# uzh-rpg/rpg_ramnet

Hardware: AMD Instinct MI355X
Metric: depth samples/sec (346x260 cropped to 256x344, 5-bin grids, K=5 grids + 1 frame per sample; training step) (higher is better)
Workload: dtype f32; 1 GPU; EventScape-shaped 346x260 -> 256x344 crop, 5 event bins, K=5, batch 8/GPU, seq-len 8, 1xMI355X-per-rank train, state=convgru, SI loss on [image,events4], Adam, backward-weights co-scheduled on a side stream, decoders on a second stream; global_batch=8, seq_len=8, parallelism=dp1

## Files before the change

include/ramnet_hip.h:

```cpp
#ifndef RAMNET_HIP_H
#define RAMNET_HIP_H
#include <stddef.h>
#include <stdint.h>

#ifdef __cplusplus
extern "C" {
#endif

#define RAMNET_ABI_VERSION 27
#define RAMNET_E_BADARG 10001
#define RAMNET_E_UNSUPPORTED 10002

enum ramnet_in_mode {
    RAMNET_IN_PLAIN = 0,
    RAMNET_IN_CAT = 1,
    RAMNET_IN_CAT_MUL = 2,
    RAMNET_IN_UP2X = 3,
    RAMNET_IN_UP2X_SKIP = 4,
    RAMNET_IN_RELUMASK = 5,
    RAMNET_IN_S2D = 6,
    RAMNET_IN_PARITY4 = 7
};

enum ramnet_algo { RAMNET_ALGO_DIRECT = 0, RAMNET_ALGO_WINOGRAD = 1, RAMNET_ALGO_HEAD = 2, RAMNET_ALGO_WINOGRAD24 = 3, RAMNET_ALGO_WINOGRAD_2X4 = 4,
                   RAMNET_ALGO_WINOGRAD_2X4_SPLIT = 5, RAMNET_ALGO_DIRECT_SPLIT = 6, RAMNET_ALGO_WINOGRAD24_2X3 = 7 };

enum ramnet_epilogue {
    RAMNET_EPI_LINEAR = 0,
    RAMNET_EPI_RELU = 1,
    RAMNET_EPI_SIGMOID = 2,
    RAMNET_EPI_RES_RELU = 3,
    RAMNET_EPI_GRU_BLEND = 4,
    RAMNET_EPI_LSTM = 5,
    RAMNET_EPI_GRU_BWD = 6,
    RAMNET_EPI_SIGMOID_HR = 7
};

typedef struct ramnet_conv_desc {
    const float *x0, *x1, *xm;
    int ld0, ld1, ldm;
    int C0, C1;
    int in_mode;
    int B, Hin, Win;
    int ntaps, stride;
    int8_t dy[25], dx[25];
    uint8_t wtap[25];
    const float *w;
    const float *bias;
    int Cout;
    int Ho, Wo;
    int HoF, WoF;
    int osy, osx, ooy, oox;
    int epi;
    float beta;
    const float *e0, *e1;
    int lde0, lde1;
    float *out, *o1, *o2;
    int ldo, ldo1, ldo2;
    int algo;
    int frame;
    int out_s2d;
    int head_cin;
    int s2d_5x5;
    float *splitk_ws;
    size_t splitk_floats;
    const int *active;
} ramnet_conv_desc;

#define RAMNET_WGRAD_MAX_SEGMENTS 48
typedef struct ramnet_wgrad_seg {
    const float *x0, *x1, *xm, *dout, *gmask;
} ramnet_wgrad_seg;

typedef struct ramnet_wgrad_desc {
    const float *x0, *x1, *xm;
    int ld0, ld1, ldm, C0, C1, in_mode;
    int B, Hin, Win;
    int ntaps, stride;
    int8_t dy[25], dx[25];
    const float *dout, *gmask;
    int ldg, ldgm;
    int Cout, Ho, Wo;
    float *dw;
    float *dbias;
    int algo;
    int gsy, gsx, goy, gox;
    int HoG, WoG;
    int head_cin;
    int dw_slabs;
    int nseg;
    const ramnet_wgrad_seg *segs;
} ramnet_wgrad_desc;

int ramnet_set_option(const char *name, int value);
int ramnet_get_option(const char *name);
const char *ramnet_last_error(void);
int ramnet_abi_version(void);
const char *ramnet_last_kernel(void);
int ramnet_stream_fork(void *from, void *to);

int ramnet_gemm(const float *A, const float *B, float *C, int M, int N, int K, int lda, int ldb, int ldc, int trans_a,
                int accumulate, int batch, long stride_a, long stride_b, long stride_c, void *stream);
int ramnet_gemm2(const float *A, const float *B, float *C, int M, long stride_a, long stride_b, long stride_c, int batch, const float *A2,
                 const float *B2, float *C2, int M2, long stride_a2, long stride_b2, long stride_c2, int batch2, int N, int K, int K2, int lda,
                 int ldb, int ldc, int trans_a, int accumulate, void *stream);

int ramnet_nchw_to_nhwc_pad(const float *src, float *dst, int B, int C, int H, int W, int Cpad, void *stream);
int ramnet_reflect_pad(const float *src, float *dst, int B, int C, int H, int W, int Cpad, int top, int left, int Hc, int Wc, int nhwc,
                       void *stream);
int ramnet_wgrad_wino_slabs(int Cin, int Cout);
int ramnet_wgrad_wino2x4_slabs(int Cin, int Cout);
int ramnet_wgrad_dsplit_slabs(int Cin, int Cout);
size_t ramnet_wgrad_dsplit_ws_floats(int Cin, int Cout);
int ramnet_unpack_wgrad_dsplit(const float *ws, float *grad, int Cout, int Cin, int CinWs, int CoutWs, int n_off, void *stream);
size_t ramnet_wgrad_wino2x4_ws_floats(int Cin, int Cout);
int ramnet_reduce_slabs(float *ws, int slabs, size_t n, void *stream);
size_t ramnet_packed_weight_elems(int Cout, int Cin, int KH, int KW, int transposed, int gates);
size_t ramnet_packed_weight_elems_wino(int Cout, int Cin, int transposed, int gates);
int ramnet_pack_weight_wino(const float *w_oihw, float *wp, int Cout, int Cin, int transposed, int gates, void *stream);
size_t ramnet_packed_weight_elems_wino2x4(int Cout, int Cin, int transposed);
int ramnet_pack_weight_wino2x4(const float *w_oihw, float *wp, int Cout, int Cin, int transposed, void *stream);
size_t ramnet_packed_weight_elems_wino2x4_gates(int Cout, int Cin, int transposed, int gates);
int ramnet_pack_weight_wino2x4_gates(const float *w_oihw, float *wp, int Cout, int Cin, int transposed, int gates, void *stream);
int ramnet_conv_wino_variant(const ramnet_conv_desc *d, int force);
int ramnet_conv_wino_split_ok(const ramnet_conv_desc *d, int force);
size_t ramnet_packed_weight_elems_wino2x4_split(int Cout, int Cin, int transposed);
int ramnet_pack_weight_wino2x4_split(const float *w_oihw, float *wp, int Cout, int Cin, int transposed, void *stream);
size_t ramnet_conv_splitk_floats(const ramnet_conv_desc *d);
int ramnet_wino2x4_config(int min_wgs);
int ramnet_fold_wino_supported(int Cout, int Cin);
size_t ramnet_packed_weight_elems_fold_wino(int Cout, int Cin);
int ramnet_pack_weight_fold_wino(const float *w_oihw, float *wp, int Cout, int Cin, void *stream);
int ramnet_pack_weight_fold_wino_dgrad(const float *w_oihw, float *wp, int Cout, int Cin, void *stream);
int ramnet_pack_border_weights(const float *w_oihw, float *rows, float *cols, float *rows_t, float *cols_t, int Cout, int Cin, void *stream);
int ramnet_fold_wino_variant(const ramnet_conv_desc *d, int force);
size_t ramnet_packed_weight_elems_fold_wino2x3(int Cout, int Cin);
int ramnet_pack_weight_fold_wino2x3(const float *w_oihw, float *wp, int Cout, int Cin, void *stream);
int ramnet_pack_weight_fold_wino2x3_dgrad(const float *w_oihw, float *wp, int Cout, int Cin, void *stream);
int ramnet_fold_unpack_wgrad(float *w4, float *dU, float *wr, float *wc, float *grad, int Cout, int Cin, int CinWs, void *stream);
size_t ramnet_packed_weight_elems_head(int Cin);
int ramnet_head_supported(int Cin, int Cout);
int ramnet_pack_weight_head(const float *w_oihw, float *wp, int Cout, int Cin, void *stream);
int ramnet_pack_weight(const float *w_oihw, float *wp, int Cout, int Cin, int KH, int KW,
                       int transposed, int gates, void *stream);
int ramnet_unpack_wgrad(const float *ws, float *grad_oihw, int Cout, int Cin, int CinWs, int CoutWs, int n_off,
                        int KH, int KW, void *stream);

int ramnet_unpack_wgrad_wino(const float *ws, float *grad_oihw, int Cout, int Cin, int CinWs, int CoutWs, int n_off,
                             void *stream);
int ramnet_unpack_wgrad_wino2x4(const float *ws, float *grad_oihw, int Cout, int Cin, int CinWs, int CoutWs, int n_off,
                                void *stream);

int ramnet_conv_launch(const ramnet_conv_desc *d, void *stream);
int ramnet_conv_launch_multi(const ramnet_conv_desc *descs, int n, void *stream);
int ramnet_wgrad_launch(const ramnet_wgrad_desc *d, void *stream);

int ramnet_pred_sigmoid_fwd(const float *x, int ldx, int C, const float *w, const float *b, float *y,
                            size_t npix, void *stream);
int ramnet_pred_sigmoid_bwd(const float *x, int ldx, int C, const float *w, const float *y, const float *dy,
                            float *dx, int lddx, float *dw, float *db, size_t npix, void *stream);
#define RAMNET_PRED_SI_MAX_SEGMENTS 8
size_t ramnet_pred_si_scratch_doubles(size_t seg_pix, int nseg);
int ramnet_pred_sigmoid_si_fwd(const float *x, int ldx, int C, const float *w, const float *b, float *y, size_t seg_pix, int nseg,
                               const float *const *targets, float weight, float lambda, double *scratch, double *stats, float *loss,
                               void *stream);
int ramnet_pred_sigmoid_si_bwd(const float *x, int ldx, int C, const float *w, const float *y, const float *dy, size_t seg_pix, int nseg,
                               const float *const *targets, const double *stats, const float *gscale, float weight, float lambda,
                               float *dx, int lddx, float *dw, float *db, double *scratch, int mask_x, void *stream);
int ramnet_pred_linear_fwd(const float *x, int ldx, int C, const float *w, const float *b, float *z, size_t npix, void *stream);
int ramnet_pred_linear_bwd(const float *x, int ldx, int C, const float *w, const float *dz, float *dx, int lddx, float *dw, float *db,
                           size_t npix, void *stream);
int ramnet_relu_bwd(const float *dy, const float *y, float *dx, size_t n, void *stream);
int ramnet_pad2_sum(const float *x, const float *skip, float *out, int B, int H, int W, int C, void *stream);
int ramnet_up2x_border_im2col(const float *x, const float *skip, float *rows, float *cols, int B, int H, int W, int C, void *stream);
int ramnet_pad2_sum_im2col(const float *x, const float *skip, float *out, float *rows, float *cols, int B, int H, int W, int C, void *stream);
int ramnet_unpad2_fold(const float *dxpad, float *dx, int B, int H, int W, int C, void *stream);
int ramnet_up2x_border_col2im(const float *rows, const float *cols, float *dx, int B, int H, int W, int C, void *stream);
int ramnet_frame_gather(const float *dy, const float *mask, float *rows, float *cols, int B, int H2, int W2, int C, void *stream);
int ramnet_space_to_depth2(const float *x, float *out, int B, int H, int W, int C, int inverse, void *stream);
int ramnet_upsample2x_bwd(const float *dup, float *dx, int B, int H, int W, int C, void *stream);
int ramnet_gru_bwd_a(const float *dhn, const float *ur, const float *o, const float *h, float *dpo,
                     float *dpur, float *dh, size_t npix, int C, int ld_dhn ,
                     void *stream);
int ramnet_gru_bwd_a2(const float *dhn, const float *ur, const float *o, const float *h, float *dpo,
                      float *dpur, float *dh, size_t npix, int C, int ld_dhn, int ld_dh ,
                      void *stream);
int ramnet_gru_bwd_b(const float *dxhr, const float *ur, const float *h, float *dpur, float *dh,
                     size_t npix, int C, void *stream);
int ramnet_lstm_bwd(const float *gates, const float *cprev, const float *cnew, const float *dhn,
                    const float *dcn, float *dpre, float *dcprev, size_t npix, int C, void *stream);
int ramnet_lstm_bwd_masked(const float *gates, const float *cprev, const float *cnew, const float *dhn, const float *dcn,
                           const int *active, float *dpre, float *dcprev, float *dxh, size_t npix, int hw, int C, void *stream);
int ramnet_bias_grad(const float *dy, const float *mask, float *db, size_t npix, int C, void *stream);
int ramnet_norm_slabs(int groups, long npix, int C);
int ramnet_norm_partial(const float *a, int lda, const float *y, int ldy, int act, const float *b, int ldb, int groups, long npix,
                        int C, int nslab, double *part, void *stream);
int ramnet_norm_finalize(const double *part, int groups, int nslab, int C, long npix, double eps, const float *gamma, const float *beta,
                         float *running_mean, float *running_var, double momentum, int update_running, int use_running,
                         long long *num_batches_tracked, double *mean, double *rstd, float *scale, float *shift, void *stream);
int ramnet_norm_finalize_bwd(const double *part, int groups, int nslab, int C, long npix, const double *mean, const double *rstd,
                             const float *gamma, int batch_stats, float *c1, float *c2, float *c3, float *dgamma, float *dbeta, void *stream);
int ramnet_norm_apply(const float *x, int ldx, const float *scale, const float *shift, const float *res, int ldr, int act, float *out,
                      int ldo, int groups, long npix, int C, void *stream);
int ramnet_norm_bwd(const float *dy, int lddy, const float *y, int ldy, int act, const float *x, int ldx, const float *c1, const float *c2,
                    const float *c3, float *dx, int lddx, float *dres, int lddres, int groups, long npix, int C, void *stream);
int ramnet_add(const float *a, const float *b, float *y, size_t n, void *stream);
int ramnet_concat2(const float *a, int lda, int Ca, const float *b, int ldb, int Cb, float *y, size_t npix, void *stream);
int ramnet_cat_batch_add(const float *const *parts, int n, size_t npix, int C, int ld, const float *base, float *out, void *stream);
int ramnet_cat_batch_add_masked(const float *const *parts, int n, size_t npix, int C, int ld, const float *base, const float *mask, float *out,
                                void *stream);
int ramnet_split2(const float *y, int ldy, int Ca, int Cb, float *a, float *b, size_t npix, void *stream);

int ramnet_si_loss_fwd(const float *pred, const float *target, size_t n, float weight, float lambda,
                       double *stats, float *loss, void *stream);
int ramnet_si_loss_from_stats(const double *stats, float weight, float lambda, float *loss, void *stream);
int ramnet_si_loss_bwd(const float *pred, const float *target, size_t n, float weight, float lambda,
                       const double *stats, const float *gscale, float *dpred, void *stream);

int ramnet_si_log_loss_fwd(const float *pred, const float *target, size_t n, float lambda, double *stats, float *loss, void *stream);
int ramnet_si_log_loss_bwd(const float *pred, const float *target, size_t n, float lambda, const double *stats, const float *gscale,
                           float *dpred, void *stream);
int ramnet_mse_loss_fwd(const float *pred, const float *target, int B, int H, int W, int half, double *stats, float *loss, void *stream);
int ramnet_mse_loss_bwd(const float *pred, const float *target, int B, int H, int W, int half, const double *stats, const float *gscale,
                        float *dpred, void *stream);

int ramnet_depth_metrics(const float *pred, const float *target, size_t n, float clip_distance, float reg_factor,
                         float cutoff, double *out11, void *stream);

size_t ramnet_msg_workspace_elems(int B, int H, int W, int num_scales);
int ramnet_msg_loss_fwd(const float *pred, const float *target, int B, int H, int W, int num_scales, float *ws,
                        double *stats, float *loss, void *stream);
int ramnet_msg_loss_bwd(const float *ws, const double *stats, const float *gscale, int B, int H, int W, int num_scales,
                        float *dws, float *dpred, void *stream);

int ramnet_voxelize(const double *events, size_t n_events, int bins, int W, int H, float *grid, void *stream);
int ramnet_voxel_indices(const double *events, size_t n_events, int bins, int W, int H,
                         long long *idx_left, long long *idx_right, void *stream);
int ramnet_normalize_nonzero(float *grid, size_t n, double *scratch, void *stream);
int ramnet_voxelize_batch(const double *events, const long long *offsets, int n_grids, size_t max_events, int bins, int W, int H,
                          float *grids, void *stream);
int ramnet_normalize_nonzero_batch(float *grids, int n_grids, size_t n, double *scratch, void *stream);
int ramnet_nonzero_stats_batch(const float *grids, int n_grids, size_t n, double *stats, void *stream);

int ramnet_augment_batch(const float *const *src, float *const *dst, const int *pidx, const float *theta, const int *win,
                         const int *win_host, const double *stats, const float *bx, const float *by, int G, int n_params, int C,
                         int H, int W, int th, int tw, int Cpad, int nhwc, void *stream);

#define RAMNET_BATCH_METRICS_TICKET_BYTES 262144
size_t ramnet_batch_metrics_workspace(int G, int N, size_t npix);
int ramnet_batch_metrics(const float *const *pred, const float *const *target, int G, int N, size_t npix, void *workspace,
                         double *out, void *stream);

int ramnet_fill_pointer_table(const void **table, const void *const *host_ptrs, int n, void *stream);
size_t ramnet_grad_loss_workspace(int G, int B, int H, int W);
int ramnet_grad_loss_stats(const float *const *pred, const float *const *target, int G, int B, int H, int W, int num_scales,
                           void *workspace, double *stats, const float *weights, float *loss, float *wsum, void *stream);
int ramnet_grad_loss_from_stats(const double *stats, int G, int num_scales, double Bg, const double *Bg_dev, const float *weights,
                                float *loss, float *wsum, void *stream);
int ramnet_grad_loss_bwd(const float *const *pred, const float *const *target, int G, int B, int H, int W, int num_scales,
                         const double *stats, double Bg, const double *Bg_dev, double gain, const float *weights, const float *up,
                         const float *up_sum, float *dpred, void *stream);

#ifdef __cplusplus
}
#endif
#endif
```

rpg_ramnet_amd/_hip.py:

```python
import ctypes as C
import os

_PKG = os.path.dirname(os.path.abspath(__file__))
LIB_PATH = os.environ.get("RAMNET_HIP_LIB") or os.path.join(_PKG, "librpg_ramnet_hip.so")

IN_PLAIN, IN_CAT, IN_CAT_MUL, IN_UP2X, IN_UP2X_SKIP, IN_RELUMASK, IN_S2D, IN_PARITY4 = range(8)
ALGO_DIRECT, ALGO_WINOGRAD, ALGO_HEAD, ALGO_WINOGRAD24, ALGO_WINOGRAD_2X4, ALGO_WINOGRAD_2X4_SPLIT, ALGO_DIRECT_SPLIT = 0, 1, 2, 3, 4, 5, 6
ALGO_WINOGRAD24_2X3 = 7
EPI_LINEAR, EPI_RELU, EPI_SIGMOID, EPI_RES_RELU, EPI_GRU_BLEND, EPI_LSTM, EPI_GRU_BWD, EPI_SIGMOID_HR = range(8)

_fp = C.c_void_p


class ConvDesc(C.Structure):
    _fields_ = [
        ("x0", _fp), ("x1", _fp), ("xm", _fp),
        ("ld0", C.c_int), ("ld1", C.c_int), ("ldm", C.c_int),
        ("C0", C.c_int), ("C1", C.c_int), ("in_mode", C.c_int),
        ("B", C.c_int), ("Hin", C.c_int), ("Win", C.c_int),
        ("ntaps", C.c_int), ("stride", C.c_int),
        ("dy", C.c_int8 * 25), ("dx", C.c_int8 * 25), ("wtap", C.c_uint8 * 25),
        ("w", _fp), ("bias", _fp),
        ("Cout", C.c_int), ("Ho", C.c_int), ("Wo", C.c_int), ("HoF", C.c_int), ("WoF", C.c_int),
        ("osy", C.c_int), ("osx", C.c_int), ("ooy", C.c_int), ("oox", C.c_int),
        ("epi", C.c_int), ("beta", C.c_float),
        ("e0", _fp), ("e1", _fp), ("lde0", C.c_int), ("lde1", C.c_int),
        ("out", _fp), ("o1", _fp), ("o2", _fp),
        ("ldo", C.c_int), ("ldo1", C.c_int), ("ldo2", C.c_int),
        ("algo", C.c_int),
        ("frame", C.c_int),
        ("out_s2d", C.c_int),
        ("head_cin", C.c_int),
        ("s2d_5x5", C.c_int),
        ("splitk_ws", C.c_void_p), ("splitk_floats", C.c_size_t),
        ("active", _fp),
    ]


class WgradSeg(C.Structure):
    _fields_ = [("x0", _fp), ("x1", _fp), ("xm", _fp), ("dout", _fp), ("gmask", _fp)]


WGRAD_MAX_SEGMENTS = 48


class WgradDesc(C.Structure):
    _fields_ = [
        ("x0", _fp), ("x1", _fp), ("xm", _fp),
        ("ld0", C.c_int), ("ld1", C.c_int), ("ldm", C.c_int),
        ("C0", C.c_int), ("C1", C.c_int), ("in_mode", C.c_int),
        ("B", C.c_int), ("Hin", C.c_int), ("Win", C.c_int),
        ("ntaps", C.c_int), ("stride", C.c_int),
        ("dy", C.c_int8 * 25), ("dx", C.c_int8 * 25),
        ("dout", _fp), ("gmask", _fp), ("ldg", C.c_int), ("ldgm", C.c_int),
        ("Cout", C.c_int), ("Ho", C.c_int), ("Wo", C.c_int),
        ("dw", _fp), ("dbias", _fp),
        ("algo", C.c_int),
        ("gsy", C.c_int), ("gsx", C.c_int), ("goy", C.c_int), ("gox", C.c_int), ("HoG", C.c_int), ("WoG", C.c_int),
        ("head_cin", C.c_int),
        ("dw_slabs", C.c_int),
        ("nseg", C.c_int), ("segs", C.POINTER(WgradSeg)),
    ]


_SIGS = {
    "ramnet_abi_version": (C.c_int, []),
    "ramnet_last_error": (C.c_char_p, []),
    "ramnet_set_option": (C.c_int, [C.c_char_p, C.c_int]),
    "ramnet_get_option": (C.c_int, [C.c_char_p]),
    "ramnet_last_kernel": (C.c_char_p, []),
    "ramnet_stream_fork": (C.c_int, [_fp, _fp]),
    "ramnet_gemm": (C.c_int, [_fp, _fp, _fp] + [C.c_int] * 9 + [C.c_long] * 3 + [_fp]),
    "ramnet_gemm2": (C.c_int, [_fp, _fp, _fp, C.c_int, C.c_long, C.c_long, C.c_long, C.c_int, _fp, _fp, _fp, C.c_int, C.c_long, C.c_long, C.c_long,
                               C.c_int, C.c_int, C.c_int, C.c_int, C.c_int, C.c_int, C.c_int, C.c_int, C.c_int, _fp]),
    "ramnet_nchw_to_nhwc_pad": (C.c_int, [_fp, _fp, C.c_int, C.c_int, C.c_int, C.c_int, C.c_int, _fp]),
    "ramnet_reflect_pad": (C.c_int, [_fp, _fp] + [C.c_int] * 10 + [_fp]),
    "ramnet_wgrad_wino_slabs": (C.c_int, [C.c_int, C.c_int]),
    "ramnet_wgrad_wino2x4_slabs": (C.c_int, [C.c_int, C.c_int]),
    "ramnet_wgrad_dsplit_slabs": (C.c_int, [C.c_int, C.c_int]),
    "ramnet_wgrad_dsplit_ws_floats": (C.c_size_t, [C.c_int, C.c_int]),
    "ramnet_unpack_wgrad_dsplit": (C.c_int, [_fp, _fp, C.c_int, C.c_int, C.c_int, C.c_int, C.c_int, _fp]),
    "ramnet_wgrad_wino2x4_ws_floats": (C.c_size_t, [C.c_int, C.c_int]),
    "ramnet_reduce_slabs": (C.c_int, [_fp, C.c_int, C.c_size_t, _fp]),
    "ramnet_packed_weight_elems": (C.c_size_t, [C.c_int] * 6),
    "ramnet_pack_weight": (C.c_int, [_fp, _fp, C.c_int, C.c_int, C.c_int, C.c_int, C.c_int, C.c_int, _fp]),
    "ramnet_packed_weight_elems_wino": (C.c_size_t, [C.c_int] * 4),
    "ramnet_pack_weight_wino": (C.c_int, [_fp, _fp, C.c_int, C.c_int, C.c_int, C.c_int, _fp]),
    "ramnet_packed_weight_elems_wino2x4": (C.c_size_t, [C.c_int] * 3),
    "ramnet_pack_weight_wino2x4": (C.c_int, [_fp, _fp, C.c_int, C.c_int, C.c_int, _fp]),
    "ramnet_packed_weight_elems_wino2x4_gates": (C.c_size_t, [C.c_int] * 4),
    "ramnet_pack_weight_wino2x4_gates": (C.c_int, [_fp, _fp, C.c_int, C.c_int, C.c_int, C.c_int, _fp]),
    "ramnet_wino2x4_config": (C.c_int, [C.c_int]),
    "ramnet_conv_wino_variant": (C.c_int, [C.POINTER(ConvDesc), C.c_int]),
    "ramnet_conv_wino_split_ok": (C.c_int, [C.POINTER(ConvDesc), C.c_int]),
    "ramnet_packed_weight_elems_wino2x4_split": (C.c_size_t, [C.c_int] * 3),
    "ramnet_pack_weight_wino2x4_split": (C.c_int, [_fp, _fp, C.c_int, C.c_int, C.c_int, _fp]),
    "ramnet_conv_splitk_floats": (C.c_size_t, [C.POINTER(ConvDesc)]),
    "ramnet_packed_weight_elems_head": (C.c_size_t, [C.c_int]),
    "ramnet_head_supported": (C.c_int, [C.c_int, C.c_int]),
    "ramnet_pack_weight_head": (C.c_int, [_fp, _fp, C.c_int, C.c_int, _fp]),
    "ramnet_fold_wino_supported": (C.c_int, [C.c_int, C.c_int]),
    "ramnet_packed_weight_elems_fold_wino": (C.c_size_t, [C.c_int, C.c_int]),
    "ramnet_pack_weight_fold_wino": (C.c_int, [_fp, _fp, C.c_int, C.c_int, _fp]),
    "ramnet_pack_weight_fold_wino_dgrad": (C.c_int, [_fp, _fp, C.c_int, C.c_int, _fp]),
    "ramnet_fold_wino_variant": (C.c_int, [C.POINTER(ConvDesc), C.c_int]),
    "ramnet_packed_weight_elems_fold_wino2x3": (C.c_size_t, [C.c_int, C.c_int]),
    "ramnet_pack_weight_fold_wino2x3": (C.c_int, [_fp, _fp, C.c_int, C.c_int, _fp]),
    "ramnet_pack_weight_fold_wino2x3_dgrad": (C.c_int, [_fp, _fp, C.c_int, C.c_int, _fp]),
    "ramnet_pack_border_weights": (C.c_int, [_fp] * 5 + [C.c_int, C.c_int, _fp]),
    "ramnet_fold_unpack_wgrad": (C.c_int, [_fp] * 5 + [C.c_int, C.c_int, C.c_int, _fp]),
    "ramnet_unpad2_fold": (C.c_int, [_fp, _fp, C.c_int, C.c_int, C.c_int, C.c_int, _fp]),
    "ramnet_up2x_border_col2im": (C.c_int, [_fp, _fp, _fp, C.c_int, C.c_int, C.c_int, C.c_int, _fp]),
    "ramnet_pad2_sum": (C.c_int, [_fp, _fp, _fp, C.c_int, C.c_int, C.c_int, C.c_int, _fp]),
    "ramnet_up2x_border_im2col": (C.c_int, [_fp, _fp, _fp, _fp, C.c_int, C.c_int, C.c_int, C.c_int, _fp]),
    "ramnet_pad2_sum_im2col": (C.c_int, [_fp, _fp, _fp, _fp, _fp, C.c_int, C.c_int, C.c_int, C.c_int, _fp]),
    "ramnet_space_to_depth2": (C.c_int, [_fp, _fp, C.c_int, C.c_int, C.c_int, C.c_int, C.c_int, _fp]),
    "ramnet_frame_gather": (C.c_int, [_fp, _fp, _fp, _fp, C.c_int, C.c_int, C.c_int, C.c_int, _fp]),
    "ramnet_unpack_wgrad": (C.c_int, [_fp, _fp] + [C.c_int] * 7 + [_fp]),
    "ramnet_unpack_wgrad_wino": (C.c_int, [_fp, _fp] + [C.c_int] * 5 + [_fp]),
    "ramnet_unpack_wgrad_wino2x4": (C.c_int, [_fp, _fp] + [C.c_int] * 5 + [_fp]),
    "ramnet_conv_launch": (C.c_int, [C.POINTER(ConvDesc), _fp]),
    "ramnet_conv_launch_multi": (C.c_int, [C.POINTER(ConvDesc), C.c_int, _fp]),
    "ramnet_wgrad_launch": (C.c_int, [C.POINTER(WgradDesc), _fp]),
    "ramnet_pred_sigmoid_fwd": (C.c_int, [_fp, C.c_int, C.c_int, _fp, _fp, _fp, C.c_size_t, _fp]),
    "ramnet_pred_sigmoid_bwd": (C.c_int, [_fp, C.c_int, C.c_int, _fp, _fp, _fp, _fp, C.c_int, _fp, _fp, C.c_size_t, _fp]),
    "ramnet_pred_si_scratch_doubles": (C.c_size_t, [C.c_size_t, C.c_int]),
    "ramnet_pred_sigmoid_si_fwd": (C.c_int, [_fp, C.c_int, C.c_int, _fp, _fp, _fp, C.c_size_t, C.c_int, C.POINTER(C.c_void_p), C.c_float, C.c_float,
                                             _fp, _fp, _fp, _fp]),
    "ramnet_pred_sigmoid_si_bwd": (C.c_int, [_fp, C.c_int, C.c_int, _fp, _fp, _fp, C.c_size_t, C.c_int, C.POINTER(C.c_void_p), _fp, _fp, C.c_float,
                                             C.c_float, _fp, C.c_int, _fp, _fp, _fp, C.c_int, _fp]),
    "ramnet_pred_linear_fwd": (C.c_int, [_fp, C.c_int, C.c_int, _fp, _fp, _fp, C.c_size_t, _fp]),
    "ramnet_pred_linear_bwd": (C.c_int, [_fp, C.c_int, C.c_int, _fp, _fp, _fp, C.c_int, _fp, _fp, C.c_size_t, _fp]),
    "ramnet_cat_batch_add": (C.c_int, [_fp, C.c_int, C.c_size_t, C.c_int, C.c_int, _fp, _fp, _fp]),
    "ramnet_cat_batch_add_masked": (C.c_int, [_fp, C.c_int, C.c_size_t, C.c_int, C.c_int, _fp, _fp, _fp, _fp]),
    "ramnet_relu_bwd": (C.c_int, [_fp, _fp, _fp, C.c_size_t, _fp]),
    "ramnet_upsample2x_bwd": (C.c_int, [_fp, _fp, C.c_int, C.c_int, C.c_int, C.c_int, _fp]),
    "ramnet_gru_bwd_a": (C.c_int, [_fp] * 7 + [C.c_size_t, C.c_int, C.c_int, _fp]),
    "ramnet_gru_bwd_a2": (C.c_int, [_fp] * 7 + [C.c_size_t, C.c_int, C.c_int, C.c_int, _fp]),
    "ramnet_gru_bwd_b": (C.c_int, [_fp] * 5 + [C.c_size_t, C.c_int, _fp]),
    "ramnet_lstm_bwd": (C.c_int, [_fp] * 7 + [C.c_size_t, C.c_int, _fp]),
    "ramnet_lstm_bwd_masked": (C.c_int, [_fp, _fp, _fp, _fp, _fp, _fp, _fp, _fp, _fp, C.c_size_t, C.c_int, C.c_int, _fp]),
    "ramnet_norm_slabs": (C.c_int, [C.c_int, C.c_long, C.c_int]),
    "ramnet_norm_partial": (C.c_int, [_fp, C.c_int, _fp, C.c_int, C.c_int, _fp, C.c_int, C.c_int, C.c_long, C.c_int, C.c_int, _fp, _fp]),
    "ramnet_norm_finalize": (C.c_int, [_fp, C.c_int, C.c_int, C.c_int, C.c_long, C.c_double, _fp, _fp, _fp, _fp, C.c_double, C.c_int, C.c_int,
                                       _fp, _fp, _fp, _fp, _fp, _fp]),
    "ramnet_norm_finalize_bwd": (C.c_int, [_fp, C.c_int, C.c_int, C.c_int, C.c_long, _fp, _fp, _fp, C.c_int, _fp, _fp, _fp, _fp, _fp, _fp]),
    "ramnet_norm_apply": (C.c_int, [_fp, C.c_int, _fp, _fp, _fp, C.c_int, C.c_int, _fp, C.c_int, C.c_int, C.c_long, C.c_int, _fp]),
    "ramnet_norm_bwd": (C.c_int, [_fp, C.c_int, _fp, C.c_int, C.c_int, _fp, C.c_int, _fp, _fp, _fp, _fp, C.c_int, _fp, C.c_int,
                                  C.c_int, C.c_long, C.c_int, _fp]),
    "ramnet_add": (C.c_int, [_fp, _fp, _fp, C.c_size_t, _fp]),
    "ramnet_split2": (C.c_int, [_fp, C.c_int, C.c_int, C.c_int, _fp, _fp, C.c_size_t, _fp]),
    "ramnet_concat2": (C.c_int, [_fp, C.c_int, C.c_int, _fp, C.c_int, C.c_int, _fp, C.c_size_t, _fp]),
    "ramnet_bias_grad": (C.c_int, [_fp, _fp, _fp, C.c_size_t, C.c_int, _fp]),
    "ramnet_si_loss_fwd": (C.c_int, [_fp, _fp, C.c_size_t, C.c_float, C.c_float, _fp, _fp, _fp]),
    "ramnet_si_loss_from_stats": (C.c_int, [_fp, C.c_float, C.c_float, _fp, _fp]),
    "ramnet_si_loss_bwd": (C.c_int, [_fp, _fp, C.c_size_t, C.c_float, C.c_float, _fp, _fp, _fp, _fp]),
    "ramnet_si_log_loss_fwd": (C.c_int, [_fp, _fp, C.c_size_t, C.c_float, _fp, _fp, _fp]),
    "ramnet_si_log_loss_bwd": (C.c_int, [_fp, _fp, C.c_size_t, C.c_float, _fp, _fp, _fp, _fp]),
    "ramnet_mse_loss_fwd": (C.c_int, [_fp, _fp, C.c_int, C.c_int, C.c_int, C.c_int, _fp, _fp, _fp]),
    "ramnet_mse_loss_bwd": (C.c_int, [_fp, _fp, C.c_int, C.c_int, C.c_int, C.c_int, _fp, _fp, _fp, _fp]),
    "ramnet_depth_metrics": (C.c_int, [_fp, _fp, C.c_size_t, C.c_float, C.c_float, C.c_float, _fp, _fp]),
    "ramnet_msg_workspace_elems": (C.c_size_t, [C.c_int] * 4),
    "ramnet_msg_loss_fwd": (C.c_int, [_fp, _fp, C.c_int, C.c_int, C.c_int, C.c_int, _fp, _fp, _fp, _fp]),
    "ramnet_msg_loss_bwd": (C.c_int, [_fp, _fp, _fp, C.c_int, C.c_int, C.c_int, C.c_int, _fp, _fp, _fp]),
    "ramnet_voxelize": (C.c_int, [_fp, C.c_size_t, C.c_int, C.c_int, C.c_int, _fp, _fp]),
    "ramnet_voxel_indices": (C.c_int, [_fp, C.c_size_t, C.c_int, C.c_int, C.c_int, _fp, _fp, _fp]),
    "ramnet_normalize_nonzero": (C.c_int, [_fp, C.c_size_t, _fp, _fp]),
    "ramnet_voxelize_batch": (C.c_int, [_fp, _fp, C.c_int, C.c_size_t, C.c_int, C.c_int, C.c_int, _fp, _fp]),
    "ramnet_normalize_nonzero_batch": (C.c_int, [_fp, C.c_int, C.c_size_t, _fp, _fp]),
    "ramnet_nonzero_stats_batch": (C.c_int, [_fp, C.c_int, C.c_size_t, _fp, _fp]),
    "ramnet_augment_batch": (C.c_int, [_fp] * 9 + [C.c_int] * 9 + [_fp]),
    "ramnet_batch_metrics_workspace": (C.c_size_t, [C.c_int, C.c_int, C.c_size_t]),
    "ramnet_batch_metrics": (C.c_int, [_fp, _fp, C.c_int, C.c_int, C.c_size_t, _fp, _fp, _fp]),
    "ramnet_fill_pointer_table": (C.c_int, [_fp, C.POINTER(C.c_void_p), C.c_int, _fp]),
    "ramnet_grad_loss_workspace": (C.c_size_t, [C.c_int] * 4),
    "ramnet_grad_loss_stats": (C.c_int, [_fp, _fp] + [C.c_int] * 5 + [_fp] * 6),
    "ramnet_grad_loss_from_stats": (C.c_int, [_fp, C.c_int, C.c_int, C.c_double, _fp, _fp, _fp, _fp, _fp]),
    "ramnet_grad_loss_bwd": (C.c_int, [_fp, _fp] + [C.c_int] * 5 + [_fp, C.c_double, _fp, C.c_double, _fp, _fp, _fp, _fp, _fp]),
}
EXPORTS = tuple(_SIGS)

_lib = None
_tracer = None


class _Traced:
    def __init__(self, l):
        self._l = l

    def __getattr__(self, name):
        fn = getattr(self._l, name)
        tr = _tracer
        if tr is None:
            return fn
        return lambda *a: tr(name, fn, a)


def set_tracer(fn):
    global _tracer
    _tracer = fn


class HipLibraryMissing(RuntimeError):
    pass


def lib():
    global _lib
    if _lib is None:
        if not os.path.exists(LIB_PATH):
            raise HipLibraryMissing(
                "%s not found: build it with `python -c 'import __graft_entry__ as g; g.build()'` "
                "(hipcc --offload-arch=gfx950). rpg_ramnet_amd has no CPU fallback." % LIB_PATH)
        import torch
        rt = os.path.join(os.path.dirname(torch.__file__), "lib", "libamdhip64.so")
        if os.path.exists(rt):
            C.CDLL(rt, mode=C.RTLD_GLOBAL)
        l = C.CDLL(LIB_PATH)
        for name, (res, args) in _SIGS.items():
            fn = getattr(l, name)
            fn.restype, fn.argtypes = res, args
        if l.ramnet_abi_version() != 27:
            raise RuntimeError("ABI version mismatch in %s" % LIB_PATH)
        _lib = l
    return _lib if _tracer is None else _Traced(_lib)


def check(code, what):
    if code != 0:
        msg = lib().ramnet_last_error()
        raise RuntimeError("%s failed (code %d): %s" % (what, code, msg.decode() if msg else "?"))
```

rpg_ramnet_amd/csrc/common.hpp:

```cpp
#pragma once
#include <hip/hip_runtime.h>
#include <stdint.h>
#include <stdio.h>
#include "../../include/ramnet_hip.h"

typedef float f32x16 __attribute__((ext_vector_type(16)));

namespace ramnet {

constexpr int CK = 16;
constexpr int LDP = CK + 4;
constexpr int TWID = 16;
constexpr int WCK = 32;

extern int g_opt_voxel_sorted, g_opt_fold_pair, g_opt_wgrad_blocks, g_opt_wgrad_wino_blocks, g_opt_wino_ksplit, g_opt_wgrad_wino_nf, g_opt_pred_si_cap, g_opt_pred_si_bwd_cap;
void set_error(const char *fmt, ...);
void note_kernel(const char *fmt, ...);
int launch_wino(const ramnet_conv_desc &d, hipStream_t st);
size_t wino24_splitk_floats(const ramnet_conv_desc &d);
int launch_wino6(const ramnet_conv_desc &d, hipStream_t st);
int launch_wino6s(const ramnet_conv_desc &d, hipStream_t st);
int launch_head(const ramnet_conv_desc &d, hipStream_t st);
int launch_wino24(const ramnet_conv_desc &d, hipStream_t st);
int launch_wgrad_wino24(const ramnet_wgrad_desc &d, hipStream_t st);
int launch_head_wgrad(const ramnet_wgrad_desc &d, hipStream_t st);
int launch_wgrad_wino(const ramnet_wgrad_desc &d, hipStream_t st);
int launch_wgrad_wino6(const ramnet_wgrad_desc &d, hipStream_t st);
int launch_wgrad_dsplit(const ramnet_wgrad_desc &d, hipStream_t st);

#define RAMNET_CHECK_ARG(cond)                                                        \
    do {                                                                              \
        if (!(cond)) {                                                                \
            ramnet::set_error("%s:%d: bad argument: %s", __FILE__, __LINE__, #cond);  \
            return RAMNET_E_BADARG;                                                   \
        }                                                                             \
    } while (0)

#define RAMNET_HIP(call)                                                                        \
    do {                                                                                        \
        hipError_t e_ = (call);                                                                 \
        if (e_ != hipSuccess) {                                                                 \
            ramnet::set_error("%s:%d: %s -> %s", __FILE__, __LINE__, #call, hipGetErrorString(e_)); \
            return (int)e_;                                                                     \
        }                                                                                       \
    } while (0)

#define RAMNET_LAUNCH_CHECK() RAMNET_HIP(hipGetLastError())

hipError_t allow_full_lds(const void *kernel);
#define RAMNET_FULL_LDS(kern) RAMNET_HIP(ramnet::allow_full_lds(reinterpret_cast<const void *>(kern)))

__device__ __forceinline__ float4 ld4(const float *p) { return *reinterpret_cast<const float4 *>(p); }
__device__ __forceinline__ void st4(float *p, float4 v) { *reinterpret_cast<float4 *>(p) = v; }
__device__ __forceinline__ float4 f4zero() { return make_float4(0.f, 0.f, 0.f, 0.f); }
__device__ __forceinline__ float4 f4add(float4 a, float4 b) { return make_float4(a.x + b.x, a.y + b.y, a.z + b.z, a.w + b.w); }
__device__ __forceinline__ float4 f4mul(float4 a, float4 b) { return make_float4(a.x * b.x, a.y * b.y, a.z * b.z, a.w * b.w); }
__device__ __forceinline__ float4 f4scale(float4 a, float s) { return make_float4(a.x * s, a.y * s, a.z * s, a.w * s); }
__device__ __forceinline__ float sigmoidf_(float x) { return __builtin_amdgcn_rcpf(1.0f + __expf(-x)); }
__device__ __forceinline__ float tanhf_(float x) { return 1.0f - 2.0f * __builtin_amdgcn_rcpf(1.0f + __expf(2.0f * x)); }

__device__ __forceinline__ auto wino_rsrc(const void *p, unsigned bytes) {
    const unsigned long long a = (unsigned long long)p;
    const unsigned lo = __builtin_amdgcn_readfirstlane((unsigned)a), hi = __builtin_amdgcn_readfirstlane((unsigned)(a >> 32));
    return __builtin_amdgcn_make_buffer_rsrc((void *)(((unsigned long long)hi << 32) | lo), (short)0, (int)bytes, 0x00020000);
}
constexpr unsigned WOOB = 0x7fffff00u;

struct InSrc {
    const float *x0, *x1, *xm;
    int ld0, ld1, ldm, C0, Cin, mode, Hin, Win;
};

__device__ __forceinline__ void up2x_coord(int d, int n_src, int &i0, int &i1, float &l1) {
    float s = fmaxf(0.5f * (float)d - 0.25f, 0.0f);
    i0 = (int)s;
    i1 = i0 + (i0 < n_src - 1 ? 1 : 0);
    l1 = s - (float)i0;
}

__device__ __forceinline__ float4 load_in4(const InSrc &s, int b, int iy, int ix, int c) {
    if ((unsigned)iy >= (unsigned)s.Hin || (unsigned)ix >= (unsigned)s.Win || c >= s.Cin) return f4zero();
    if (s.mode == RAMNET_IN_UP2X || s.mode == RAMNET_IN_UP2X_SKIP) {
        const int Hs = s.Hin >> 1, Ws = s.Win >> 1;
        int y0, y1, x0, x1;
        float ly, lx;
        up2x_coord(iy, Hs, y0, y1, ly);
        up2x_coord(ix, Ws, x0, x1, lx);
        const float hy = 1.0f - ly, hx = 1.0f - lx;
        const size_t r0 = ((size_t)b * Hs + y0) * Ws, r1 = ((size_t)b * Hs + y1) * Ws;
        float4 v00 = ld4(s.x0 + (r0 + x0) * s.ld0 + c), v01 = ld4(s.x0 + (r0 + x1) * s.ld0 + c);
        float4 v10 = ld4(s.x0 + (r1 + x0) * s.ld0 + c), v11 = ld4(s.x0 + (r1 + x1) * s.ld0 + c);
        if (s.mode == RAMNET_IN_UP2X_SKIP) {
            v00 = f4add(v00, ld4(s.x1 + (r0 + x0) * s.ld1 + c));
            v01 = f4add(v01, ld4(s.x1 + (r0 + x1) * s.ld1 + c));
            v10 = f4add(v10, ld4(s.x1 + (r1 + x0) * s.ld1 + c));
            v11 = f4add(v11, ld4(s.x1 + (r1 + x1) * s.ld1 + c));
        }
        float4 top = f4add(f4scale(v00, hx), f4scale(v01, lx));
        float4 bot = f4add(f4scale(v10, hx), f4scale(v11, lx));
        return f4add(f4scale(top, hy), f4scale(bot, ly));
    }
    const size_t pix = ((size_t)b * s.Hin + iy) * s.Win + ix;
    if (s.mode == RAMNET_IN_PLAIN) return ld4(s.x0 + pix * s.ld0 + c);
    if (s.mode == RAMNET_IN_RELUMASK) {
        float4 v = ld4(s.x0 + pix * s.ld0 + c), m = ld4(s.xm + pix * s.ldm + c);
        return make_float4(m.x > 0.f ? v.x : 0.f, m.y > 0.f ? v.y : 0.f, m.z > 0.f ? v.z : 0.f, m.w > 0.f ? v.w : 0.f);
    }
    if (c < s.C0) return ld4(s.x0 + pix * s.ld0 + c);
    float4 v = ld4(s.x1 + pix * s.ld1 + (c - s.C0));
    if (s.mode == RAMNET_IN_CAT_MUL) v = f4mul(v, ld4(s.xm + pix * s.ldm + (c - s.C0)));
    return v;
}

template <int QPP, int LDX, int NB, int NT>
__device__ __forceinline__ void stage_patch(float *__restrict__ patch, const InSrc &s, int b, int iy0, int ix0, int c0,
                                            int PH, int PW, int tid) {
    constexpr int PXS = LDX, QS = 4;
    const int nslots = PH * PW * QPP;
    if (s.mode == RAMNET_IN_UP2X || s.mode == RAMNET_IN_UP2X_SKIP) {
        for (int sl = tid; sl < nslots; sl += NT) {
            const int pix = sl / QPP, qd = sl - pix * QPP;
            const int py = pix / PW, px = pix - py * PW;
            st4(patch + pix * PXS + qd * QS, load_in4(s, b, iy0 + py, ix0 + px, c0 + qd * 4));
        }
        return;
    }
    const bool two = s.mode == RAMNET_IN_CAT_MUL || s.mode == RAMNET_IN_RELUMASK;
    for (int base = tid; base < nslots; base += NB * NT) {
        float4 v[NB], m[NB];
        int dst[NB];
        bool ok[NB], hasm[NB];
#pragma unroll
        for (int i = 0; i < NB; ++i) {
            const int sl = base + i * NT;
            const int pix = sl / QPP, qd = sl - pix * QPP;
            const int py = pix / PW, px = pix - py * PW;
            const int iy = iy0 + py, ix = ix0 + px, c = c0 + qd * 4;
            ok[i] = sl < nslots && (unsigned)iy < (unsigned)s.Hin && (unsigned)ix < (unsigned)s.Win && c < s.Cin;
            dst[i] = sl < nslots ? pix * PXS + qd * QS : -1;
            const size_t gp = ((size_t)b * s.Hin + iy) * s.Win + ix;
            const bool second = s.mode != RAMNET_IN_PLAIN && s.mode != RAMNET_IN_RELUMASK && c >= s.C0;
            const float *p0 = second ? s.x1 + gp * s.ld1 + (c - s.C0) : s.x0 + gp * s.ld0 + c;
            hasm[i] = two && (s.mode == RAMNET_IN_RELUMASK || second);
            const float *p1 = s.mode == RAMNET_IN_RELUMASK ? s.xm + gp * s.ldm + c : s.xm + gp * s.ldm + (c - s.C0);
            v[i] = ld4(ok[i] ? p0 : s.x0);
            if (two) m[i] = ld4(ok[i] && hasm[i] ? p1 : s.x0);
        }
#pragma unroll
        for (int i = 0; i < NB; ++i) {
            float4 r = v[i];
            if (two && hasm[i]) {
                if (s.mode == RAMNET_IN_RELUMASK)
                    r = make_float4(m[i].x > 0.f ? r.x : 0.f, m[i].y > 0.f ? r.y : 0.f, m[i].z > 0.f ? r.z : 0.f, m[i].w > 0.f ? r.w : 0.f);
                else
                    r = f4mul(r, m[i]);
            }
            if (!ok[i]) r = f4zero();
            if (dst[i] >= 0) st4(patch + dst[i], r);
        }
    }
}

template <int QPP, int NB, int NT>
struct PatchRegs {
    float4 v[NB], m[NB];
    unsigned okmask, mmask;

    __device__ __forceinline__ void load(const InSrc &s, int b, int iy0, int ix0, int c0, int PH, int PW, int tid) {
        const int nslots = PH * PW * QPP;
        const bool two = s.mode == RAMNET_IN_CAT_MUL || s.mode == RAMNET_IN_RELUMASK;
        okmask = 0, mmask = 0;
#pragma unroll
        for (int i = 0; i < NB; ++i) {
            const int sl = tid + i * NT;
            const int pix = sl / QPP, qd = sl - pix * QPP;
            const int py = pix / PW, px = pix - py * PW;
            const int iy = iy0 + py, ix = ix0 + px, c = c0 + qd * 4;
            const bool ok = sl < nslots && (unsigned)iy < (unsigned)s.Hin && (unsigned)ix < (unsigned)s.Win && c < s.Cin;
            const size_t gp = ((size_t)b * s.Hin + iy) * s.Win + ix;
            const bool second = s.mode != RAMNET_IN_PLAIN && s.mode != RAMNET_IN_RELUMASK && c >= s.C0;
            const float *p0 = second ? s.x1 + gp * s.ld1 + (c - s.C0) : s.x0 + gp * s.ld0 + c;
            const bool hm = two && (s.mode == RAMNET_IN_RELUMASK || second);
            const float *p1 = s.mode == RAMNET_IN_RELUMASK ? s.xm + gp * s.ldm + c : s.xm + gp * s.ldm + (c - s.C0);
            v[i] = ld4(ok ? p0 : s.x0);
            m[i] = two ? ld4(ok && hm ? p1 : s.x0) : f4zero();
            okmask |= (ok ? 1u : 0u) << i;
            mmask |= (hm ? 1u : 0u) << i;
        }
    }

    __device__ __forceinline__ float4 value(const InSrc &s, int i) const {
        float4 r = v[i];
        if ((mmask >> i) & 1u) {
            if (s.mode == RAMNET_IN_RELUMASK)
                r = make_float4(m[i].x > 0.f ? r.x : 0.f, m[i].y > 0.f ? r.y : 0.f, m[i].z > 0.f ? r.z : 0.f, m[i].w > 0.f ? r.w : 0.f);
            else
                r = f4mul(r, m[i]);
        }
        if (!((okmask >> i) & 1u)) r = f4zero();
        return r;
    }

    template <int ROWF, int PS>
    __device__ __forceinline__ void store_planes(float *__restrict__ patch, const InSrc &s, int PH, int PW, int tid) const {
        const int nslots = PH * PW * QPP;
#pragma unroll
        for (int i = 0; i < NB; ++i) {
            const int sl = tid + i * NT;
            const float4 r = value(s, i);
            const int pix = sl / QPP, qd = sl - pix * QPP;
            const int py = pix / PW, px = pix - py * PW;
            if (sl < nslots) {
                float *d = patch + (2 * qd) * PS + py * ROWF + px * 2;
                *reinterpret_cast<float2 *>(d) = make_float2(r.x, r.y);
                *reinterpret_cast<float2 *>(d + PS) = make_float2(r.z, r.w);
            }
        }
    }

    template <int LDX>
    __device__ __forceinline__ void store(float *__restrict__ patch, const InSrc &s, int PH, int PW, int tid) const {
        const int nslots = PH * PW * QPP;
#pragma unroll
        for (int i = 0; i < NB; ++i) {
            const int sl = tid + i * NT;
            float4 r = v[i];
            if ((mmask >> i) & 1u) {
                if (s.mode == RAMNET_IN_RELUMASK)
                    r = make_float4(m[i].x > 0.f ? r.x : 0.f, m[i].y > 0.f ? r.y : 0.f, m[i].z > 0.f ? r.z : 0.f, m[i].w > 0.f ? r.w : 0.f);
                else
                    r = f4mul(r, m[i]);
            }
            if (!((okmask >> i) & 1u)) r = f4zero();
            if (sl < nslots) st4(patch + (sl / QPP) * LDX + (sl % QPP) * 4, r);
        }
    }
};

inline int cdiv(int a, int b) { return (a + b - 1) / b; }
inline int roundup(int a, int b) { return cdiv(a, b) * b; }

}
```

rpg_ramnet_amd/csrc/conv_igemm.hip:

```cpp
#include <stdlib.h>
#include "common.hpp"
#include "conv_epilogue.hpp"

namespace ramnet {

struct ConvCommon {
    InSrc src;
    int nchunks, CoutPad;
    int patch_floats;
    int nclass;
    int xcd_swizzle;
};

struct ConvClass {
    int ntaps, Ho, Wo, ooy, oox;
    int PH, PW, dymin, dxmin;
    int tiles_x, tiles_y;
    int toff[25];
    unsigned woff[25];
};
struct ConvClasses { ConvClass c[4]; };

template <int BM, int BN, int WM, int WN, bool MASK = false>
__global__ void __launch_bounds__(256) conv_igemm_kernel(const ramnet_conv_desc p, const ConvCommon qc, const ConvClasses qk) {
    int flat = blockIdx.x + gridDim.x * (blockIdx.y + gridDim.y * blockIdx.z);
    if (qc.xcd_swizzle) {
        const int nwg = gridDim.x * gridDim.y * gridDim.z, xcd = flat & 7, qq = nwg >> 3, rr = nwg & 7;
        flat = (xcd < rr ? xcd * (qq + 1) : rr * (qq + 1) + (xcd - rr) * qq) + (flat >> 3);
    }
    int bid = flat % gridDim.x;
    const int by = (flat / gridDim.x) % gridDim.y, bz = flat / (gridDim.x * gridDim.y);
    const ConvClass &q = qk.c[bz];
    constexpr int TM = BM / WM / 32, TN = BN / WN / 32;
    constexpr int TH = BM / TWID;
    constexpr int CKC = CK;
    static_assert(WM * WN == 4 && TM >= 1 && TN >= 1, "4 waves per workgroup");
    extern __shared__ __attribute__((aligned(16))) float smem[];
    float *patch = smem;
    float *wsm = smem + qc.patch_floats;

    const int tid = threadIdx.x, lane = tid & 63;
    const int wave = __builtin_amdgcn_readfirstlane(tid >> 6);
    const int wm = wave / WN, wn = wave % WN;
    const int l31 = lane & 31, kk = lane >> 5;

    if (bid >= q.tiles_x * q.tiles_y * p.B) return;
    const int tx_i = bid % q.tiles_x;
    bid /= q.tiles_x;
    const int ty_i = bid % q.tiles_y;
    const int b = bid / q.tiles_y;
    const int n0 = by * BN;
    const int oy0 = ty_i * TH, ox0 = tx_i * TWID;
    const int iy0 = oy0 * p.stride + q.dymin, ix0 = ox0 * p.stride + q.dxmin;

    int aBase[TM], bBase[TN];
#pragma unroll
    for (int ms = 0; ms < TM; ++ms) {
        const int m = (wm * TM + ms) * 32 + l31;
        aBase[ms] = (((m >> 4) * p.stride) * q.PW + (m & 15) * p.stride) * LDP + 4 * kk;
    }
#pragma unroll
    for (int ns = 0; ns < TN; ++ns) bBase[ns] = ((wn * TN + ns) * 32 + l31) * LDP + 4 * kk;

    f32x16 acc[TM][TN];
#pragma unroll
    for (int ms = 0; ms < TM; ++ms)
#pragma unroll
        for (int ns = 0; ns < TN; ++ns)
#pragma unroll
            for (int r = 0; r < 16; ++r) acc[ms][ns][r] = 0.f;

    constexpr int WF4 = BN * 4;
    constexpr int WPT = (WF4 + 255) / 256;
    float4 wreg[WPT];
    const int ntaps = q.ntaps;
    auto load_w = [&](int chunk, int t) {
        const float *src = p.w + ((size_t)q.woff[t] + ((size_t)chunk * qc.CoutPad + n0)) * 16;
#pragma unroll
        for (int i = 0; i < WPT; ++i) {
            const int f = tid + i * 256;
            if (WF4 % 256 == 0 || f < WF4) wreg[i] = ld4(src + (size_t)f * 4);
        }
    };
    auto store_w = [&](int buf) {
        float *dst = wsm + buf * (BN * LDP);
#pragma unroll
        for (int i = 0; i < WPT; ++i) {
            const int f = tid + i * 256;
            if (WF4 % 256 == 0 || f < WF4) st4(dst + (f >> 2) * LDP + (f & 3) * 4, wreg[i]);
        }
    };

    load_w(0, 0);
    int buf = 0;
    for (int chunk = 0; chunk < qc.nchunks; ++chunk) {
        __syncthreads();
        stage_patch<CKC / 4, LDP, 4, 256>(patch, qc.src, b, iy0, ix0, chunk * CKC, q.PH, q.PW, tid);
        for (int t = 0; t < ntaps; ++t) {
            store_w(buf);
            __syncthreads();
            if (t + 1 < ntaps) load_w(chunk, t + 1);
            else if (chunk + 1 < qc.nchunks) load_w(chunk + 1, 0);
            const float *pa = patch + q.toff[t];
            const float *wb = wsm + buf * (BN * LDP);
#pragma unroll
            for (int k8 = 0; k8 < 2; ++k8) {
                float4 a[TM], bb[TN];
#pragma unroll
                for (int ms = 0; ms < TM; ++ms) a[ms] = ld4(pa + aBase[ms] + k8 * 8);
#pragma unroll
                for (int ns = 0; ns < TN; ++ns) bb[ns] = ld4(wb + bBase[ns] + k8 * 8);
#pragma unroll
                for (int ms = 0; ms < TM; ++ms)
#pragma unroll
                    for (int ns = 0; ns < TN; ++ns) {
                        acc[ms][ns] = __builtin_amdgcn_mfma_f32_32x32x2f32(a[ms].x, bb[ns].x, acc[ms][ns], 0, 0, 0);
                        acc[ms][ns] = __builtin_amdgcn_mfma_f32_32x32x2f32(a[ms].y, bb[ns].y, acc[ms][ns], 0, 0, 0);
                        acc[ms][ns] = __builtin_amdgcn_mfma_f32_32x32x2f32(a[ms].z, bb[ns].z, acc[ms][ns], 0, 0, 0);
                        acc[ms][ns] = __builtin_amdgcn_mfma_f32_32x32x2f32(a[ms].w, bb[ns].w, acc[ms][ns], 0, 0, 0);
                    }
            }
            buf ^= 1;
        }
    }

    const int epi = p.epi;
    const bool act = !MASK || sample_active(p, b);
#pragma unroll
    for (int ms = 0; ms < TM; ++ms) {
#pragma unroll
        for (int r = 0; r < 16; ++r) {
            const int m = (wm * TM + ms) * 32 + (r & 3) + 8 * (r >> 2) + 4 * kk;
            const int oy = oy0 + (m >> 4), ox = ox0 + (m & 15);
            if (oy >= q.Ho || ox >= q.Wo) continue;
            const size_t pix = ((size_t)b * p.HoF + (oy * p.osy + q.ooy)) * p.WoF + (ox * p.osx + q.oox);
            const bool addold = epilogue_addold(p, oy * p.osy + q.ooy, ox * p.osx + q.oox);
            if (epi == RAMNET_EPI_LSTM) {
                if constexpr (TN == 4) {
                    const int C = p.Cout, ch = by * 32 + l31;
                    if (MASK && !act) {
                        if (ch < C) epilogue_inactive(p, epi, pix, ch);
                    } else if (ch < C) {
                        const float gi = sigmoidf_(acc[ms][0][r] + p.bias[ch]);
                        const float gf = sigmoidf_(acc[ms][1][r] + p.bias[C + ch]);
                        const float go = sigmoidf_(acc[ms][2][r] + p.bias[2 * C + ch]);
                        const float gc = tanhf_(acc[ms][3][r] + p.bias[3 * C + ch]);
                        const float cp = p.e1 ? p.e1[pix * p.lde1 + ch] : 0.f;
                        const float cn = gf * cp + gi * gc;
                        p.out[pix * p.ldo + ch] = go * tanhf_(cn);
                        p.o1[pix * p.ldo1 + ch] = cn;
                        if (p.o2) {
                            float *g = p.o2 + pix * p.ldo2 + ch;
                            g[0] = gi, g[C] = gf, g[2 * C] = go, g[3 * C] = gc;
                        }
                    }
                }
                continue;
            }
#pragma unroll
            for (int ns = 0; ns < TN; ++ns) {
                const int n = n0 + (wn * TN + ns) * 32 + l31;
                if (n >= p.Cout) continue;
                if (MASK && !act) {
                    epilogue_inactive(p, epi, pix, n);
                    continue;
                }
                epilogue_store(p, epi, pix, n, acc[ms][ns][r] + epilogue_side(p, epi, b, oy * p.osy + q.ooy, ox * p.osx + q.oox, n), addold);
            }
        }
    }
}

template <int BM, int BN, int WM, int WN>
static int launch_cfg(const ramnet_conv_desc &d, const ConvCommon &qc, const ConvClasses &qk, int max_tiles, hipStream_t st) {
    auto kern = d.active ? conv_igemm_kernel<BM, BN, WM, WN, true> : conv_igemm_kernel<BM, BN, WM, WN>;
    const size_t lds = ((size_t)qc.patch_floats + 2 * BN * LDP) * sizeof(float);
    static size_t lds_set[2] = {0, 0};
    if (lds > lds_set[d.active != nullptr]) {
        RAMNET_FULL_LDS((kern));
        lds_set[d.active != nullptr] = 160 * 1024;
    }
    if (lds > 160 * 1024) {
        set_error("conv patch does not fit LDS (%zu bytes)", lds);
        return RAMNET_E_UNSUPPORTED;
    }
    dim3 grid(max_tiles * d.B, qc.CoutPad / BN, qc.nclass);
    note_kernel(d.active ? "conv_igemm_kernel<%d,%d,%d,%d,masked>" : "conv_igemm_kernel<%d,%d,%d,%d>", BM, BN, WM, WN);
    hipLaunchKernelGGL(kern, grid, dim3(256), lds, st, d, qc, qk);
    RAMNET_LAUNCH_CHECK();
    return 0;
}

static int check_desc(const ramnet_conv_desc &d) {
    RAMNET_CHECK_ARG(d.x0 && d.w && d.out);
    RAMNET_CHECK_ARG(d.ntaps >= 1 && d.ntaps <= 25 && (d.stride == 1 || d.stride == 2));
    RAMNET_CHECK_ARG(d.B > 0 && d.Ho > 0 && d.Wo > 0 && d.Hin > 0 && d.Win > 0 && d.Cout > 0);
    RAMNET_CHECK_ARG(d.C0 > 0 && d.C0 % 4 == 0 && d.ld0 % 4 == 0 && d.ldo > 0);
    RAMNET_CHECK_ARG(d.osy >= 1 && d.osx >= 1);
    const bool cat = d.in_mode == RAMNET_IN_CAT || d.in_mode == RAMNET_IN_CAT_MUL;
    if (cat) RAMNET_CHECK_ARG(d.x1 && d.C1 > 0 && d.C1 % 4 == 0 && d.ld1 % 4 == 0);
    if (d.in_mode == RAMNET_IN_CAT_MUL || d.in_mode == RAMNET_IN_RELUMASK) RAMNET_CHECK_ARG(d.xm && d.ldm % 4 == 0);
    if (d.in_mode == RAMNET_IN_UP2X_SKIP) RAMNET_CHECK_ARG(d.x1 && d.ld1 % 4 == 0);
    if (d.in_mode == RAMNET_IN_UP2X || d.in_mode == RAMNET_IN_UP2X_SKIP) RAMNET_CHECK_ARG(d.Hin % 2 == 0 && d.Win % 2 == 0);
    if (d.epi == RAMNET_EPI_RES_RELU) RAMNET_CHECK_ARG(d.e0);
    if (d.epi == RAMNET_EPI_GRU_BLEND) RAMNET_CHECK_ARG(d.e0);
    if (d.epi == RAMNET_EPI_LSTM) RAMNET_CHECK_ARG(d.o1 && d.bias);
    if (d.epi == RAMNET_EPI_GRU_BWD) RAMNET_CHECK_ARG(d.e0 && d.o1 && d.Cout % 8 == 0 && !d.bias && d.beta == 0.f && d.frame == 0 && d.out_s2d == 0);
    if (d.epi == RAMNET_EPI_SIGMOID_HR) RAMNET_CHECK_ARG(d.e1 && d.o1 && d.Cout % 8 == 0 && d.beta == 0.f && d.frame == 0 && d.out_s2d == 0 &&
                                                         d.algo != RAMNET_ALGO_WINOGRAD24 && d.algo != RAMNET_ALGO_WINOGRAD24_2X3 && d.algo != RAMNET_ALGO_HEAD);
    {
        unsigned long long ld = (unsigned long long)d.ld0;
        if (cat || d.in_mode == RAMNET_IN_UP2X_SKIP) ld = ld > (unsigned long long)d.ld1 ? ld : (unsigned long long)d.ld1;
        if (d.xm) ld = ld > (unsigned long long)d.ldm ? ld : (unsigned long long)d.ldm;
        const unsigned long long px = (unsigned long long)d.B * d.Hin * d.Win * (d.in_mode == RAMNET_IN_S2D ? 4 : 1);
        RAMNET_CHECK_ARG(px * ld < (1ull << 32));
    }
    RAMNET_CHECK_ARG(d.frame >= 0);
    if (d.active) RAMNET_CHECK_ARG((d.epi == RAMNET_EPI_SIGMOID || d.epi == RAMNET_EPI_SIGMOID_HR || d.epi == RAMNET_EPI_GRU_BLEND ||
                                    (d.epi == RAMNET_EPI_LSTM && d.e0)) && d.frame == 0 && d.out_s2d == 0 &&
                                   (d.algo == RAMNET_ALGO_DIRECT || d.algo == RAMNET_ALGO_WINOGRAD || d.algo == RAMNET_ALGO_WINOGRAD_2X4 ||
                                    d.algo == RAMNET_ALGO_WINOGRAD_2X4_SPLIT));
    if (d.frame > 0) RAMNET_CHECK_ARG(d.e0 && d.e1 && (d.epi == RAMNET_EPI_RELU || d.epi == RAMNET_EPI_LINEAR));
    return 0;
}

static int launch_classes(const ramnet_conv_desc *ds, int n, hipStream_t st) {
    const ramnet_conv_desc &d = ds[0];
    for (int i = 0; i < n; ++i) {
        const int rc = check_desc(ds[i]);
        if (rc) return rc;
        RAMNET_CHECK_ARG(ds[i].x0 == d.x0 && ds[i].w == d.w && ds[i].out == d.out && ds[i].stride == d.stride &&
                         ds[i].Cout == d.Cout && ds[i].epi == d.epi && ds[i].osy == d.osy && ds[i].osx == d.osx &&
                         ds[i].B == d.B && ds[i].in_mode == d.in_mode && ds[i].active == d.active);
    }
    const bool cat = d.in_mode == RAMNET_IN_CAT || d.in_mode == RAMNET_IN_CAT_MUL;
    ConvCommon qc;
    ConvClasses qk;
    qc.src.x0 = d.x0, qc.src.x1 = d.x1, qc.src.xm = d.xm;
    qc.src.ld0 = d.ld0, qc.src.ld1 = d.ld1, qc.src.ldm = d.ldm;
    qc.src.C0 = d.C0, qc.src.Cin = d.C0 + (cat ? d.C1 : 0);
    qc.src.mode = d.in_mode, qc.src.Hin = d.Hin, qc.src.Win = d.Win;
    qc.nchunks = cdiv(qc.src.Cin, CK);
    qc.CoutPad = d.epi == RAMNET_EPI_LSTM ? 4 * roundup(d.Cout, 32) : roundup(d.Cout, 32);
    qc.nclass = n;
    qc.xcd_swizzle = 0;
    const int lstm = d.epi == RAMNET_EPI_LSTM;
    int BM = 128, BN = lstm ? 128 : (qc.CoutPad % 128 == 0 ? 128 : qc.CoutPad % 64 == 0 ? 64 : 32);
    auto blocks = [&](int bm, int bn) {
        long t = 0;
        for (int i = 0; i < n; ++i) t += (long)cdiv(ds[i].Wo, TWID) * cdiv(ds[i].Ho, bm / TWID);
        return t * d.B * (qc.CoutPad / bn);
    };
    if (!lstm && BN >= 64) {
        const long want = 768;
        if (blocks(BM, BN) < want) BM = 64;
        if (blocks(BM, BN) < want && BN == 128) BN = 64;
    }
    if (!lstm && BN == 32 && blocks(256, 32) >= 1024)
        BM = 256;
    const int TH = BM / TWID;
    int max_tiles = 0;
    qc.patch_floats = 0;
    for (int i = 0; i < n; ++i) {
        const ramnet_conv_desc &e = ds[i];
        ConvClass &q = qk.c[i];
        int dymin = 127, dymax = -127, dxmin = 127, dxmax = -127;
        for (int t = 0; t < e.ntaps; ++t) {
            dymin = e.dy[t] < dymin ? e.dy[t] : dymin, dymax = e.dy[t] > dymax ? e.dy[t] : dymax;
            dxmin = e.dx[t] < dxmin ? e.dx[t] : dxmin, dxmax = e.dx[t] > dxmax ? e.dx[t] : dxmax;
        }
        q.ntaps = e.ntaps, q.Ho = e.Ho, q.Wo = e.Wo, q.ooy = e.ooy, q.oox = e.oox;
        q.dymin = dymin, q.dxmin = dxmin;
        q.PH = (TH - 1) * e.stride + (dymax - dymin) + 1;
        q.PW = (TWID - 1) * e.stride + (dxmax - dxmin) + 1;
        q.tiles_x = cdiv(e.Wo, TWID), q.tiles_y = cdiv(e.Ho, TH);
        for (int t = 0; t < e.ntaps; ++t) {
            q.toff[t] = ((e.dy[t] - dymin) * q.PW + (e.dx[t] - dxmin)) * LDP;
            q.woff[t] = (unsigned)e.wtap[t] * (unsigned)qc.nchunks * (unsigned)qc.CoutPad;
        }
        if (q.PH * q.PW * LDP > qc.patch_floats) qc.patch_floats = q.PH * q.PW * LDP;
        if (q.tiles_x * q.tiles_y > max_tiles) max_tiles = q.tiles_x * q.tiles_y;
    }
    if (lstm) return launch_cfg<128, 128, 4, 1>(d, qc, qk, max_tiles, st);
    if (BM == 128 && BN == 128) return launch_cfg<128, 128, 2, 2>(d, qc, qk, max_tiles, st);
    if (BM == 128 && BN == 64) return launch_cfg<128, 64, 2, 2>(d, qc, qk, max_tiles, st);
    if (BM == 64 && BN == 128) return launch_cfg<64, 128, 2, 2>(d, qc, qk, max_tiles, st);
    if (BM == 64 && BN == 64) return launch_cfg<64, 64, 2, 2>(d, qc, qk, max_tiles, st);
    if (BM == 256) return launch_cfg<256, 32, 4, 1>(d, qc, qk, max_tiles, st);
    return launch_cfg<128, 32, 4, 1>(d, qc, qk, max_tiles, st);
}

}

using namespace ramnet;

extern "C" int ramnet_conv_launch(const ramnet_conv_desc *dp, void *stream) {
    RAMNET_CHECK_ARG(dp != nullptr);
    if (dp->algo == RAMNET_ALGO_WINOGRAD) {
        const int rc = check_desc(*dp);
        return rc ? rc : launch_wino(*dp, (hipStream_t)stream);
    }
    if (dp->algo == RAMNET_ALGO_WINOGRAD_2X4) {
        const int rc = check_desc(*dp);
        return rc ? rc : launch_wino6(*dp, (hipStream_t)stream);
    }
    if (dp->algo == RAMNET_ALGO_WINOGRAD_2X4_SPLIT) {
        const int rc = check_desc(*dp);
        return rc ? rc : launch_wino6s(*dp, (hipStream_t)stream);
    }
    if (dp->algo == RAMNET_ALGO_WINOGRAD24 || dp->algo == RAMNET_ALGO_WINOGRAD24_2X3) {
        const int rc = check_desc(*dp);
        return rc ? rc : launch_wino24(*dp, (hipStream_t)stream);
    }
    if (dp->algo == RAMNET_ALGO_HEAD) {
        const int rc = check_desc(*dp);
        return rc ? rc : launch_head(*dp, (hipStream_t)stream);
    }
    RAMNET_CHECK_ARG(dp->algo == RAMNET_ALGO_DIRECT && dp->in_mode != RAMNET_IN_S2D && dp->out_s2d == 0);
    return launch_classes(dp, 1, (hipStream_t)stream);
}

extern "C" int ramnet_conv_launch_multi(const ramnet_conv_desc *descs, int n, void *stream) {
    RAMNET_CHECK_ARG(descs != nullptr && n >= 1 && n <= 4);
    for (int i = 0; i < n; ++i) RAMNET_CHECK_ARG(descs[i].in_mode != RAMNET_IN_S2D && descs[i].out_s2d == 0);
    return launch_classes(descs, n, (hipStream_t)stream);
}
```

rpg_ramnet_amd/csrc/conv_plan.hpp:

```cpp
#pragma once
#include "conv_wino_common.hpp"

namespace ramnet {

#define RAMNET_PLAN_CHECK(cond)                                                                       \
    do {                                                                                              \
        if (!(cond)) {                                                                                \
            if (!quiet) ramnet::set_error("%s:%d: bad argument: %s", __FILE__, __LINE__, #cond);      \
            return RAMNET_E_BADARG;                                                                   \
        }                                                                                             \
    } while (0)

constexpr int WKS = 16;
constexpr int W6_BN = 64;
constexpr int W6_U_FLOATS = 24 * W6_BN * WK;
constexpr int W6S_POS_BYTES = 2 * 3 * 1024;
constexpr int W6S_BLK_BYTES = 4 * 6 * W6S_POS_BYTES;

inline int log2_exact(int v) {
    int sh = 0;
    while ((1 << sh) < v) ++sh;
    return (1 << sh) == v ? sh : -1;
}

inline bool al16(const void *ptr) { return ptr == nullptr || ((uintptr_t)ptr & 15) == 0; }

template <class Desc>
inline void fill_in_src(const Desc &d, InSrc &s) {
    const bool cat = d.in_mode == RAMNET_IN_CAT || d.in_mode == RAMNET_IN_CAT_MUL;
    s.x0 = d.x0, s.x1 = d.x1, s.xm = d.xm;
    s.ld0 = d.ld0, s.ld1 = d.ld1, s.ldm = d.ldm;
    s.C0 = d.C0, s.Cin = d.C0 + (cat ? d.C1 : 0);
    s.mode = d.in_mode, s.Hin = d.Hin, s.Win = d.Win;
    if (d.in_mode == RAMNET_IN_S2D) s.Cin = 4 * d.C0, s.ld1 = log2_exact(d.C0);
}

inline bool taps_3x3(const int8_t *dy, const int8_t *dx, bool forward_order, int &dy0, int &dx0) {
    dy0 = 127, dx0 = 127;
    for (int t = 0; t < 9; ++t) {
        dy0 = dy[t] < dy0 ? dy[t] : dy0;
        dx0 = dx[t] < dx0 ? dx[t] : dx0;
    }
    unsigned seen = 0;
    for (int t = 0; t < 9; ++t) {
        const int a = dy[t] - dy0, c = dx[t] - dx0;
        if (a < 0 || a >= 3 || c < 0 || c >= 3 || (forward_order && a * 3 + c != t)) return false;
        seen |= 1u << (a * 3 + c);
    }
    return seen == 0x1ffu;
}

inline bool conv_vec4(const ramnet_conv_desc &d, bool with_o2) {
    return d.Cout % 4 == 0 && d.ldo % 4 == 0 && al16(d.out) && al16(d.bias) && (!d.o1 || (d.ldo1 % 4 == 0 && al16(d.o1))) &&
           (!d.e0 || (d.lde0 % 4 == 0 && al16(d.e0))) && (!d.e1 || (d.lde1 % 4 == 0 && al16(d.e1))) &&
           (!with_o2 || !d.o2 || (d.ldo2 % 4 == 0 && al16(d.o2)));
}

inline bool out_s2d_ok(const ramnet_conv_desc &d) {
    return d.out_s2d >= 8 && log2_exact(d.out_s2d) > 0 && d.Cout == 4 * d.out_s2d && d.epi == RAMNET_EPI_LINEAR && !d.bias && d.beta == 0.f &&
           d.HoF == 2 * d.Ho && d.WoF == 2 * d.Wo;
}

inline int xcd_groups(size_t wbytes, int nblk) {
    int xg = wbytes > (12u << 20) ? 2 : wbytes > (3u << 20) ? 1 : 0;
    while (xg > 0 && (nblk % (1 << xg)) != 0) --xg;
    return xg;
}

inline int check_offsets32(const ramnet_conv_desc &d, bool with_o2, bool quiet) {
    const unsigned long long px = (unsigned long long)d.Hin * d.Win * (d.in_mode == RAMNET_IN_S2D ? 4 : 1);
    int ldmax = d.ld0 > d.ld1 ? d.ld0 : d.ld1;
    ldmax = ldmax > d.ldm ? ldmax : d.ldm;
    RAMNET_PLAN_CHECK(px * ldmax * 4ull < (unsigned long long)WOOB);
    int lo = d.ldo > d.ldo1 ? d.ldo : d.ldo1;
    lo = lo > d.lde0 ? lo : d.lde0;
    lo = lo > d.lde1 ? lo : d.lde1;
    if (with_o2) lo = lo > d.ldo2 ? lo : d.ldo2;
    RAMNET_PLAN_CHECK((unsigned long long)d.HoF * d.WoF * lo * 4ull < (unsigned long long)WOOB);
    return 0;
}

inline long wino6_tile(int Ho, int Wo, int &txg) {
    const int shapes[3] = {4, 2, 8};
    long best = -1;
    for (int s = 0; s < 3; ++s) {
        const int t = shapes[s], th = 2 * (32 / t), tw = 4 * t;
        const long a = (long)cdiv(Ho, th) * th * cdiv(Wo, tw) * tw;
        if (best < 0 || a < best) best = a, txg = t;
    }
    return best;
}

inline bool wino6_lstm_ok(const ramnet_conv_desc &d) {
    return d.in_mode == RAMNET_IN_CAT && d.C0 % WK == 0 && d.Cout > 0 && d.Cout % 16 == 0 && d.o1 && d.bias && !d.out_s2d && !d.frame &&
           d.osy == 1 && d.osx == 1 && d.ooy == 0 && d.oox == 0 &&
           (!d.o2 || (d.ldo2 % 4 == 0 && d.ldo2 >= 4 * d.Cout && ((uintptr_t)d.o2 & 15) == 0));
}

struct Wino6Plan {
    WinoParams q;
    int txg;
    unsigned grid;
    size_t exchange;
};

inline int wino6_plan(const ramnet_conv_desc &d, int chunk, Wino6Plan &out, bool quiet = false) {
    const bool split = chunk == WKS;
    RAMNET_PLAN_CHECK(d.ntaps == 9 && d.stride == 1 && !d.frame);
    const bool lstm = d.epi == RAMNET_EPI_LSTM;
    if (lstm) RAMNET_PLAN_CHECK(!split && wino6_lstm_ok(d) && (!d.active || d.e0));
    const int ncol = lstm ? 4 * d.Cout : d.Cout;
    RAMNET_PLAN_CHECK(ncol % W6_BN == 0);
    RAMNET_PLAN_CHECK(d.in_mode == RAMNET_IN_PLAIN || d.in_mode == RAMNET_IN_CAT || d.in_mode == RAMNET_IN_CAT_MUL || d.in_mode == RAMNET_IN_RELUMASK ||
                      d.in_mode == RAMNET_IN_S2D);
    if (d.in_mode == RAMNET_IN_S2D) RAMNET_PLAN_CHECK(d.C0 >= chunk && log2_exact(d.C0) > 0);
    if (d.in_mode == RAMNET_IN_CAT || d.in_mode == RAMNET_IN_CAT_MUL) RAMNET_PLAN_CHECK(d.C0 % chunk == 0);
    RAMNET_PLAN_CHECK(conv_vec4(d, false) && d.osy == 1 && d.osx == 1 && d.ooy == 0 && d.oox == 0);
    if (d.out_s2d) RAMNET_PLAN_CHECK(out_s2d_ok(d));
    if (d.epi == RAMNET_EPI_GRU_BWD) RAMNET_PLAN_CHECK(d.Cout % 128 == 0);
    int dy0, dx0;
    RAMNET_PLAN_CHECK(taps_3x3(d.dy, d.dx, false, dy0, dx0));
    if (int rc = check_offsets32(d, lstm && d.o2, quiet)) return rc;
    WinoParams &q = out.q;
    q = WinoParams{};
    fill_in_src(d, q.src);
    q.nchunks = cdiv(q.src.Cin, chunk), q.nblk = cdiv(ncol, W6_BN);
    wino6_tile(d.Ho, d.Wo, out.txg);
    q.tiles_x = cdiv(d.Wo, 4 * out.txg), q.tiles_y = cdiv(d.Ho, 2 * (32 / out.txg));
    q.dy0 = dy0, q.dx0 = dx0;
    q.vec4 = 1, q.s2d_shift = d.out_s2d ? log2_exact(d.out_s2d) : 0, q.ksplit = 1;
    q.xg = xcd_groups((size_t)q.nchunks * q.nblk * (split ? (size_t)W6S_BLK_BYTES : W6_U_FLOATS * sizeof(float)), q.nblk);
    const int wgcols = split ? 64 : 32;
    const int nbl = (q.nblk * (W6_BN / wgcols)) >> q.xg;
    q.inv_nbl = 1.0f / (float)nbl, q.inv_tx = 1.0f / (float)q.tiles_x, q.inv_ty = 1.0f / (float)q.tiles_y;
    out.grid = (unsigned)(cdiv(q.tiles_x * q.tiles_y * d.B, 8 >> q.xg) * 8 * nbl);
    out.exchange = (size_t)4 * 4 * 32 * (wgcols + 4) * sizeof(float);
    return 0;
}

#undef RAMNET_PLAN_CHECK

template <int BLOCK = 256, class K, class... A>
inline int launch_1d(K kernel, size_t total, void *stream, A... args) {
    size_t blocks = (total + BLOCK - 1) / BLOCK;
    if (blocks > 65535) blocks = 65535;
    hipLaunchKernelGGL(kernel, dim3((unsigned)blocks), dim3(BLOCK), 0, (hipStream_t)stream, args...);
    RAMNET_LAUNCH_CHECK();
    return 0;
}

}
```

rpg_ramnet_amd/csrc/conv_wino6.hip:

```cpp
#include <stdlib.h>
#include <type_traits>
#include "common.hpp"
#include "conv_epilogue.hpp"
#include "conv_plan.hpp"

typedef float f32x4 __attribute__((ext_vector_type(4)));
typedef unsigned u32x4 __attribute__((ext_vector_type(4)));

namespace ramnet {

#ifdef RAMNET_PROBE
__device__ unsigned long long g_probe6[16384 * 16];
#define RAMNET_STAMP(k) do { if (threadIdx.x == 0 && blockIdx.x < 16384) g_probe6[blockIdx.x * 16 + (k)] = __builtin_readcyclecounter(); } while (0)
#else
#define RAMNET_STAMP(k) do { } while (0)
#endif

template <int TXG> struct R6Geom {
    static constexpr int TYG = 32 / TXG, TH = 2 * TYG, TW = 4 * TXG, PH = TH + 2, PW = TW + 2, PWS = PW + 3;
    static constexpr int PSLOTS = PH * PWS + ((4 - (PH * PWS) % 8) + 8) % 8;
    static constexpr int PLANE = PSLOTS * 4;
    static constexpr int PFLOATS = 2 * PLANE;
    static_assert(PH * PW * 2 <= 768, "three patch slots per thread");
};

template <int TXG, int MODE, bool MASK = false, bool LSTM = false>
__global__ void __launch_bounds__(256, 2) conv_wino_r6_kernel(const ramnet_conv_desc p, const WinoParams q) {
    constexpr int NF = 1;
    constexpr int RO_LD = NF * 32 + 4;
    using G = R6Geom<TXG>;
    constexpr int RP_PLANE = G::PLANE, RP_FLOATS = G::PFLOATS, RPW = G::PWS, RTW = G::TW;
    extern __shared__ __attribute__((aligned(16))) float smem[];
    float *patch = smem;

    const int tid = threadIdx.x, lane = tid & 63;
    const int wave = __builtin_amdgcn_readfirstlane(tid >> 6);
    const int l31 = lane & 31, hq = lane >> 5;
    RAMNET_STAMP(0);
#ifdef RAMNET_PROBE
    if (threadIdx.x == 0 && blockIdx.x < 16384) {
        g_probe6[blockIdx.x * 16 + 7] = __builtin_amdgcn_s_memrealtime();
        g_probe6[blockIdx.x * 16 + 8] = __builtin_amdgcn_s_getreg((31 << 11) | 4);
        g_probe6[blockIdx.x * 16 + 9] = __builtin_amdgcn_s_getreg((31 << 11) | 20);
    }
#endif

    auto fdiv = [](int n, int d, float inv) {
        int qv = (int)((float)n * inv);
        const int r = n - qv * d;
        qv += (r >= d ? 1 : 0) - (r < 0 ? 1 : 0);
        return qv;
    };
    const int xslot = blockIdx.x >> 3, xcd = blockIdx.x & 7;
    const int nbl = (q.nblk * (2 / NF)) >> q.xg;
    const int xq = fdiv(xslot, nbl, q.inv_nbl);
    const int nblk_v = ((xslot - xq * nbl) << q.xg) + (xcd & ((1 << q.xg) - 1));
    const int nblk_i = NF == 1 ? nblk_v >> 1 : nblk_v, fh = NF == 1 ? nblk_v & 1 : 0;
    int bid = xq * (8 >> q.xg) + (xcd >> q.xg);
    if (bid >= q.tiles_x * q.tiles_y * p.B) return;
    const int bq = fdiv(bid, q.tiles_x, q.inv_tx);
    const int tx_i = bid - bq * q.tiles_x;
    const int b = fdiv(bq, q.tiles_y, q.inv_ty);
    const int ty_i = bq - b * q.tiles_y;
    const int n0 = nblk_i * W6_BN + fh * 32;
    const int oy0 = ty_i * G::TH, ox0 = tx_i * G::TW;
    const int iy0 = oy0 + q.dy0, ix0 = ox0 + q.dx0;

    const int tty = l31 / TXG, ttx = l31 % TXG;
    const int ra = wave == 0 ? 0 : (wave == 2 ? 2 : 1);
    const int rb = wave == 0 ? 2 : (wave == 1 ? 2 : (wave == 2 ? 1 : 3));
    const float sb = wave == 1 ? 1.f : -1.f;
    const int pra = hq * RP_PLANE + ((2 * tty + ra) * RPW + 4 * ttx + (((2 * tty + ra) >> 1) & 3)) * 4;
    const int prb = hq * RP_PLANE + ((2 * tty + rb) * RPW + 4 * ttx + (((2 * tty + rb) >> 1) & 3)) * 4;

    f32x16 acc[6][NF];
#pragma unroll
    for (int i = 0; i < 6; ++i)
#pragma unroll
        for (int f = 0; f < NF; ++f)
#pragma unroll
            for (int r = 0; r < 16; ++r) acc[i][f][r] = 0.f;

    const int nch = q.nchunks;
    const int clast = (nch - 1) * WK;
    WinoPatch<MODE, 3> pr;
    pr.template init<G::PH, G::PW, G::PWS, G::PLANE, true>(q.src, b, iy0, ix0, tid, clast, 2 * RP_FLOATS);
    const auto wrs = wino_rsrc(p.w, (unsigned)((size_t)nch * q.nblk * W6_U_FLOATS * sizeof(float)));
    const unsigned wvo = (unsigned)((wave * 3072 + fh * 256 + lane * 4) * 4);
    const int wblk = nblk_i * W6_U_FLOATS * 4, wchunk = q.nblk * W6_U_FLOATS * 4;
    auto wload = [&](int chunk, int i) {
        return __builtin_bit_cast(float4, __builtin_amdgcn_raw_buffer_load_b128(wrs, (int)wvo, chunk * wchunk + wblk + i * 1024, 0));
    };
    float4 breg[6][NF];
    float tA[6][4], tB[6][4];
    constexpr int LD = 2;
    float vb[4][4];
    float4 qa[6], qb[6];
    float sa[4], sd[4];
    auto colop = [&](int qp, int vi, int i, const float (&t)[6][4]) {
        float(&v)[4] = vb[vi];
        if (qp == 0) {
            if (i < 4) v[i] = fmaf(-5.f, t[2][i], t[4][i]);
            else v[i - 4] = fmaf(4.f, t[0][i - 4], v[i - 4]);
        } else if (qp == 1) {
            if (i < 2) sa[2 * i] = fmaf(-4.f, t[2][2 * i], t[4][2 * i]), sa[2 * i + 1] = fmaf(-4.f, t[2][2 * i + 1], t[4][2 * i + 1]);
            else if (i < 4) sd[2 * i - 4] = fmaf(-4.f, t[1][2 * i - 4], t[3][2 * i - 4]), sd[2 * i - 3] = fmaf(-4.f, t[1][2 * i - 3], t[3][2 * i - 3]);
            else v[i - 4] = sa[i - 4] + sd[i - 4];
        } else if (qp == 2) {
            if (i >= 4) v[i - 4] = sa[i - 4] - sd[i - 4];
        } else if (qp == 3) {
            if (i < 2) sa[2 * i] = t[4][2 * i] - t[2][2 * i], sa[2 * i + 1] = t[4][2 * i + 1] - t[2][2 * i + 1];
            else if (i < 4) sd[2 * i - 4] = t[3][2 * i - 4] - t[1][2 * i - 4], sd[2 * i - 3] = t[3][2 * i - 3] - t[1][2 * i - 3];
            else v[i - 4] = fmaf(2.f, sd[i - 4], sa[i - 4]);
        } else if (qp == 4) {
            if (i >= 4) v[i - 4] = fmaf(-2.f, sd[i - 4], sa[i - 4]);
        } else {
            if (i < 4) v[i] = fmaf(-5.f, t[3][i], t[5][i]);
            else v[i - 4] = fmaf(4.f, t[1][i - 4], v[i - 4]);
        }
    };

    RAMNET_STAMP(1);
    pr.load(q.src, 0, clast);
#pragma unroll
    for (int i = 0; i < 12; ++i)
        if (!(i & 1)) breg[i >> 1][0] = wload(0, i);
    pr.store(patch, q.src, 0);
    pr.load(q.src, min(WK, clast), clast);
    __syncthreads();
    RAMNET_STAMP(2);
#pragma unroll
    for (int c = 0; c < 6; ++c) {
        const float4 x = ld4(patch + pra + c * 4), y = ld4(patch + prb + c * 4);
        tA[c][0] = x.x + sb * y.x, tA[c][1] = x.y + sb * y.y, tA[c][2] = x.z + sb * y.z, tA[c][3] = x.w + sb * y.w;
    }
#pragma unroll
    for (int qp = 0; qp < LD; ++qp)
#pragma unroll
        for (int i = 0; i < 8; ++i) colop(qp, qp, i, tA);
    pr.store(patch + RP_FLOATS, q.src, min(WK, clast));
    pr.load(q.src, min(2 * WK, clast), clast);
    __syncthreads();
    RAMNET_STAMP(3);
    auto body = [&](auto par, int chunk, const float (&tc)[6][4], float (&tn)[6][4]) {
        constexpr int PAR = decltype(par)::value;
        const float *pnext = patch + ((chunk + 1) & 1) * RP_FLOATS;
        float *pfree = patch + (chunk & 1) * RP_FLOATS;
        const int cw = min(chunk + 1, nch - 1);
        const int c2 = min((chunk + 2) * WK, clast), c3 = min((chunk + 3) * WK, clast);
        auto slot = [&](int s) {
            const int g = s >> 3, i = s & 7;
            if (s < 12) {
                if (!(s & 1)) qa[s >> 1] = ld4(pnext + pra + (s >> 1) * 4);
                else qb[s >> 1] = ld4(pnext + prb + (s >> 1) * 4);
            }
            if (s >= 4 && s < 28) {
                const int j = (s - 4) >> 2, c = (s - 4) & 3;
                const float x = c == 0 ? qa[j].x : c == 1 ? qa[j].y : c == 2 ? qa[j].z : qa[j].w;
                const float y = c == 0 ? qb[j].x : c == 1 ? qb[j].y : c == 2 ? qb[j].z : qb[j].w;
                tn[j][c] = fmaf(sb, y, x);
                asm volatile("" : "+v"(tn[j][c]));
            }
            if (g + LD < 6) colop(g + LD, (g + LD + 2 * PAR) & 3, i, tc);
            else colop(g + LD - 6, (g + LD - 6 + 2 * (PAR ^ 1)) & 3, i, tn);
            if (s >= 28 && s < 31) pr.store_slot(pfree, q.src, c2, s - 28);
            if (s == 33 || s == 35 || s == 37) pr.load_slot(q.src, c3, (s - 33) >> 1, clast);
            if ((s & 15) == 15) breg[g - 1][0] = wload(cw, (g - 1) * 2), breg[g][0] = wload(cw, g * 2);
        };
#pragma unroll
        for (int gp = 0; gp < 3; ++gp) {
            const int p0 = 2 * gp, p1 = 2 * gp + 1;
            const float b0[4] = {breg[p0][0].x, breg[p0][0].y, breg[p0][0].z, breg[p0][0].w};
            const float b1[4] = {breg[p1][0].x, breg[p1][0].y, breg[p1][0].z, breg[p1][0].w};
#pragma unroll
            for (int j = 0; j < 4; ++j) {
                __builtin_amdgcn_sched_barrier(0);
                acc[p0][0] = __builtin_amdgcn_mfma_f32_32x32x2f32(b0[j], vb[(p0 + 2 * PAR) & 3][j], acc[p0][0], 0, 0, 0);
                __builtin_amdgcn_sched_barrier(0);
                slot(gp * 16 + j * 4), slot(gp * 16 + j * 4 + 1);
                __builtin_amdgcn_sched_barrier(0);
                acc[p1][0] = __builtin_amdgcn_mfma_f32_32x32x2f32(b1[j], vb[(p1 + 2 * PAR) & 3][j], acc[p1][0], 0, 0, 0);
                __builtin_amdgcn_sched_barrier(0);
                slot(gp * 16 + j * 4 + 2), slot(gp * 16 + j * 4 + 3);
            }
        }
        __builtin_amdgcn_sched_barrier(0);
        __syncthreads();
    };
    int chunk = 0;
    do {
        body(std::integral_constant<int, 0>{}, chunk, tA, tB);
        if (chunk + 1 < nch) body(std::integral_constant<int, 1>{}, chunk + 1, tB, tA);
        chunk += 2;
    } while (chunk < nch);
    RAMNET_STAMP(4);

    const int qd = tid & 7, nq = n0 + qd * 4;
    const bool nok = nq < p.Cout;
    const float4 bias4 = p.bias ? ld4(p.bias + (nok ? nq : 0)) : f4zero();
    const int lchn = nblk_i * 16 + fh * 8 + (tid & 1) * 4;
    float4 lbias[4];
    if constexpr (LSTM) {
#pragma unroll
        for (int g = 0; g < 4; ++g) lbias[g] = ld4(p.bias + g * p.Cout + lchn);
    }
    float *P = smem;
#pragma unroll
    for (int f = 0; f < NF; ++f)
#pragma unroll
        for (int g = 0; g < 4; ++g) {
            float c0[4], c1[4], c2[4], c3[4];
#pragma unroll
            for (int e = 0; e < 4; ++e) {
                const int r = 4 * g + e;
                const float m0 = acc[0][f][r], m1 = acc[1][f][r], m2 = acc[2][f][r], m3 = acc[3][f][r], m4 = acc[4][f][r], m5 = acc[5][f][r];
                const float a12 = m1 + m2, d12 = m1 - m2, a34 = m3 + m4, d34 = m3 - m4;
                c0[e] = m0 + a12 + a34, c1[e] = d12 + 2.f * d34, c2[e] = a12 + 4.f * a34, c3[e] = d12 + 8.f * d34 + m5;
            }
            float *dst = P + ((wave * 4) * 32 + l31) * RO_LD + f * 32 + 8 * g + 4 * hq;
            st4(dst + 0 * 32 * RO_LD, make_float4(c0[0], c0[1], c0[2], c0[3]));
            st4(dst + 1 * 32 * RO_LD, make_float4(c1[0], c1[1], c1[2], c1[3]));
            st4(dst + 2 * 32 * RO_LD, make_float4(c2[0], c2[1], c2[2], c2[3]));
            st4(dst + 3 * 32 * RO_LD, make_float4(c3[0], c3[1], c3[2], c3[3]));
        }
    __syncthreads();
    RAMNET_STAMP(5);
    const int epi = p.epi;
    const bool act = !MASK || sample_active(p, b);
    constexpr int NI = 4, RSTEP = 32 / RTW;
    const int px0 = (tid >> 3) % RTW, py0 = (tid >> 3) / RTW;
    const bool colok = nok && ox0 + px0 < p.Wo;
    const unsigned pix0 = (unsigned)((oy0 + py0) * p.WoF + ox0 + px0);
    const size_t img = (size_t)b * p.HoF * p.WoF;
    const float *lbase = P + ((px0 & 3) * 32 + (px0 >> 2)) * RO_LD + qd * 4;
    auto rsrc_of = [&](const float *ptr, int ld) { return wino_rsrc(ptr ? ptr + img * ld : nullptr, WOOB); };
    auto bld = [](decltype(wino_rsrc(nullptr, 0u)) r, unsigned off) { return __builtin_bit_cast(float4, __builtin_amdgcn_raw_buffer_load_b128(r, (int)off, 0, 0)); };
    auto bst = [](decltype(wino_rsrc(nullptr, 0u)) r, unsigned off, float4 v) { __builtin_amdgcn_raw_buffer_store_b128(__builtin_bit_cast(u32x4, v), r, (int)off, 0, 0); };
    unsigned bad[2 * NI];
#pragma unroll
    for (int j = 0; j < 2 * NI; ++j) bad[j] = (colok && oy0 + py0 + j * RSTEP < p.Ho) ? 0u : WOOB;
    auto off0_of = [&](int ld, bool have, int dn = 0) { return have ? (pix0 * (unsigned)ld + (unsigned)(nq + dn)) * 4u : WOOB; };
    auto step_of = [&](int ld) { return (unsigned)(RSTEP * p.WoF * ld * 4); };
    const auto r_out = rsrc_of(p.out, p.ldo);
    if constexpr (LSTM) {
        constexpr int LSTEP = 128 / RTW;
        const int C = p.Cout, lpx = (tid >> 1) % RTW, lpy = (tid >> 1) / RTW;
        const unsigned lpix = (unsigned)((oy0 + lpy) * p.WoF + ox0 + lpx);
        const float *lb0 = P + ((lpx & 3) * 32 + (lpx >> 2)) * RO_LD + (tid & 1) * 4;
        const auto r_c = rsrc_of(p.e1, p.lde1), r_h = MASK ? rsrc_of(p.e0, p.lde0) : r_out;
        const auto r_cn = rsrc_of(p.o1, p.ldo1), r_g = rsrc_of(p.o2, p.ldo2);
        const bool lact = !MASK || sample_active(p, b);
        auto lsel = [&](float4 v, float4 w) { return make_float4(lact ? v.x : w.x, lact ? v.y : w.y, lact ? v.z : w.z, lact ? v.w : w.w); };
        unsigned lbad[2];
#pragma unroll
        for (int i = 0; i < 2; ++i) lbad[i] = (ox0 + lpx < p.Wo && oy0 + lpy + i * LSTEP < p.Ho) ? 0u : WOOB;
        auto loff = [&](int ld, bool have, int i) {
            return have ? ((lpix * (unsigned)ld + (unsigned)lchn) * 4u + (unsigned)(i * LSTEP * p.WoF * ld * 4)) | lbad[i] : WOOB;
        };
        float4 cp[2], hp[2];
#pragma unroll
        for (int i = 0; i < 2; ++i) {
            cp[i] = bld(r_c, loff(p.lde1, p.e1 != nullptr, i));
            if (MASK) hp[i] = bld(r_h, loff(p.lde0, true, i));
        }
#pragma unroll
        for (int i = 0; i < 2; ++i) {
            const int py = lpy + i * LSTEP;
            const float *bb = lb0 + ((py >> 1) * TXG + (py & 1) * 128) * RO_LD;
            const float sg = (py & 1) ? -1.f : 1.f;
            float4 t0[4], t1[4], t2[4], a[4];
#pragma unroll
            for (int g = 0; g < 4; ++g) t0[g] = ld4(bb + 8 * g), t1[g] = ld4(bb + 128 * RO_LD + 8 * g), t2[g] = ld4(bb + 256 * RO_LD + 8 * g);
#pragma unroll
            for (int g = 0; g < 4; ++g)
                a[g] = f4add(make_float4(fmaf(sg, t2[g].x, fmaf(sg, t1[g].x, t0[g].x)), fmaf(sg, t2[g].y, fmaf(sg, t1[g].y, t0[g].y)),
                                         fmaf(sg, t2[g].z, fmaf(sg, t1[g].z, t0[g].z)), fmaf(sg, t2[g].w, fmaf(sg, t1[g].w, t0[g].w))), lbias[g]);
            float4 gi = make_float4(sigmoidf_(a[0].x), sigmoidf_(a[0].y), sigmoidf_(a[0].z), sigmoidf_(a[0].w));
            float4 gf = make_float4(sigmoidf_(a[1].x), sigmoidf_(a[1].y), sigmoidf_(a[1].z), sigmoidf_(a[1].w));
            float4 go = make_float4(sigmoidf_(a[2].x), sigmoidf_(a[2].y), sigmoidf_(a[2].z), sigmoidf_(a[2].w));
            float4 gc = make_float4(tanhf_(a[3].x), tanhf_(a[3].y), tanhf_(a[3].z), tanhf_(a[3].w));
            const float4 c = cp[i];
            float4 cn = make_float4(gf.x * c.x + gi.x * gc.x, gf.y * c.y + gi.y * gc.y, gf.z * c.z + gi.z * gc.z, gf.w * c.w + gi.w * gc.w);
            float4 hn = make_float4(go.x * tanhf_(cn.x), go.y * tanhf_(cn.y), go.z * tanhf_(cn.z), go.w * tanhf_(cn.w));
            if (MASK) hn = lsel(hn, hp[i]), cn = lsel(cn, c), gi = lsel(gi, f4zero()), gf = lsel(gf, f4zero()), go = lsel(go, f4zero()), gc = lsel(gc, f4zero());
            bst(r_out, loff(p.ldo, true, i), hn);
            bst(r_cn, loff(p.ldo1, true, i), cn);
            const unsigned og = loff(p.ldo2, p.o2 != nullptr, i);
            bst(r_g, og, gi), bst(r_g, og + (unsigned)C * 4u, gf), bst(r_g, og + (unsigned)C * 8u, go), bst(r_g, og + (unsigned)C * 12u, gc);
        }
        return;
    }
    auto run = [&](auto kind) {
        constexpr int K = decltype(kind)::value;
        const bool addold = K == 0 && p.beta != 0.f && (epi == RAMNET_EPI_RELU || epi == RAMNET_EPI_LINEAR);
        const bool relu = epi == RAMNET_EPI_RELU;
        const auto r_e0 = (K >= 1 && K <= 3) ? rsrc_of(p.e0, p.lde0) : r_out;
        const auto r_e1 = (K == 2 || K == 3 || K == 5) ? rsrc_of(p.e1, p.lde1) : r_out;
        const auto r_o1 = (K == 2 || K == 3 || K == 5) ? rsrc_of(p.o1, p.ldo1) : r_out;
        const unsigned o_out = off0_of(p.ldo, true), s_out = step_of(p.ldo);
        const unsigned o_e0 = off0_of(p.lde0, K >= 1 && K <= 3), s_e0 = step_of(p.lde0);
        const unsigned o_e1 = off0_of(p.lde1, ((K == 2 || K == 3) && p.e1 != nullptr) || (K == 5 && nq >= p.Cout / 2), (K == 3 || K == 5) ? -(p.Cout / 2) : 0), s_e1 = step_of(p.lde1);
        const unsigned o_o1 = off0_of(p.ldo1, ((K == 2 || K == 3) && p.o1 != nullptr) || (K == 5 && nq >= p.Cout / 2), K == 5 ? -(p.Cout / 2) : 0), s_o1 = step_of(p.ldo1);
#pragma unroll
        for (int half = 0; half < 2; ++half) {
            unsigned oo[NI];
            float4 ea[NI], eb[NI], ec[NI], t0[NI], t1[NI], t2[NI];
#pragma unroll
            for (int i = 0; i < NI; ++i) {
                const int j = half * NI + i;
                oo[i] = (o_out + j * s_out) | bad[j];
                if (K == 0) ea[i] = addold ? bld(r_out, oo[i]) : f4zero();
                if (K >= 1 && K <= 3) ea[i] = bld(r_e0, (o_e0 + j * s_e0) | bad[j]);
                if (K == 2 || K == 3 || K == 5) eb[i] = bld(r_e1, (o_e1 + j * s_e1) | bad[j]);
                if (K == 3) ec[i] = bld(r_out, oo[i]);
            }
            RAMNET_STAMP(11 + 2 * half);
#pragma unroll
            for (int i = 0; i < NI; ++i) {
                const int py = py0 + (half * NI + i) * RSTEP;
                const float *bb = lbase + ((py >> 1) * TXG + (py & 1) * 128) * RO_LD;
                t0[i] = ld4(bb), t1[i] = ld4(bb + 128 * RO_LD), t2[i] = ld4(bb + 256 * RO_LD);
            }
#pragma unroll
            for (int i = 0; i < NI; ++i) {
                const float sg = ((py0 + (half * NI + i) * RSTEP) & 1) ? -1.f : 1.f;
                float4 v = make_float4(fmaf(sg, t2[i].x, fmaf(sg, t1[i].x, t0[i].x)), fmaf(sg, t2[i].y, fmaf(sg, t1[i].y, t0[i].y)),
                                       fmaf(sg, t2[i].z, fmaf(sg, t1[i].z, t0[i].z)), fmaf(sg, t2[i].w, fmaf(sg, t1[i].w, t0[i].w)));
                v = f4add(v, bias4);
                if (K == 0) {
                    if (addold) v = make_float4(v.x + p.beta * ea[i].x, v.y + p.beta * ea[i].y, v.z + p.beta * ea[i].z, v.w + p.beta * ea[i].w);
                    if (relu) v = make_float4(fmaxf(v.x, 0.f), fmaxf(v.y, 0.f), fmaxf(v.z, 0.f), fmaxf(v.w, 0.f));
                } else if (K == 4) {
                    v = make_float4(sigmoidf_(v.x), sigmoidf_(v.y), sigmoidf_(v.z), sigmoidf_(v.w));
                    if (MASK && !act) v = f4zero();
                } else if (K == 5) {
                    v = make_float4(sigmoidf_(v.x), sigmoidf_(v.y), sigmoidf_(v.z), sigmoidf_(v.w));
                    if (MASK && !act) v = f4zero();
                    const float4 h = (MASK && !act) ? f4zero() : eb[i];
                    bst(r_o1, (o_o1 + (half * NI + i) * s_o1) | bad[half * NI + i], make_float4(h.x * v.x, h.y * v.y, h.z * v.z, h.w * v.w));
                } else if (K == 1) {
                    v = make_float4(fmaxf(v.x + ea[i].x, 0.f), fmaxf(v.y + ea[i].y, 0.f), fmaxf(v.z + ea[i].z, 0.f), fmaxf(v.w + ea[i].w, 0.f));
                } else if (K == 3) {
                    const float4 g = v, r = ea[i], h = eb[i], old = ec[i];
                    bst(r_o1, (o_o1 + (half * NI + i) * s_o1) | bad[half * NI + i], make_float4(g.x * h.x * r.x * (1.0f - r.x), g.y * h.y * r.y * (1.0f - r.y),
                                                                                g.z * h.z * r.z * (1.0f - r.z), g.w * h.w * r.w * (1.0f - r.w)));
                    v = make_float4(old.x + g.x * r.x, old.y + g.y * r.y, old.z + g.z * r.z, old.w + g.w * r.w);
                } else {
                    const float4 o = make_float4(tanhf_(v.x), tanhf_(v.y), tanhf_(v.z), tanhf_(v.w)), u = ea[i], h = eb[i];
                    if (MASK && !act) {
                        bst(r_o1, (o_o1 + (half * NI + i) * s_o1) | bad[half * NI + i], f4zero());
                        v = h;
                    } else {
                        bst(r_o1, (o_o1 + (half * NI + i) * s_o1) | bad[half * NI + i], o);
                        v = make_float4(h.x * (1.0f - u.x) + o.x * u.x, h.y * (1.0f - u.y) + o.y * u.y, h.z * (1.0f - u.z) + o.z * u.z,
                                        h.w * (1.0f - u.w) + o.w * u.w);
                    }
                }
                bst(r_out, oo[i], v);
            }
            RAMNET_STAMP(12 + 2 * half);
        }
    };
    if (q.s2d_shift) {
        const int g = nq >> q.s2d_shift;
        const unsigned fp0 = (unsigned)((2 * (oy0 + py0) + (g >> 1)) * p.WoF + 2 * (ox0 + px0) + (g & 1));
#pragma unroll
        for (int half = 0; half < 2; ++half) {
            float4 t0[NI], t1[NI], t2[NI];
#pragma unroll
            for (int i = 0; i < NI; ++i) {
                const int py = py0 + (half * NI + i) * RSTEP;
                const float *bb = lbase + ((py >> 1) * TXG + (py & 1) * 128) * RO_LD;
                t0[i] = ld4(bb), t1[i] = ld4(bb + 128 * RO_LD), t2[i] = ld4(bb + 256 * RO_LD);
            }
#pragma unroll
            for (int i = 0; i < NI; ++i) {
                const int j = half * NI + i;
                const float sg = ((py0 + j * RSTEP) & 1) ? -1.f : 1.f;
                const unsigned off = ((fp0 * (unsigned)p.ldo + (unsigned)(nq - (g << q.s2d_shift))) * 4u + j * 2 * step_of(p.ldo)) | bad[j];
                bst(r_out, off, make_float4(fmaf(sg, t2[i].x, fmaf(sg, t1[i].x, t0[i].x)), fmaf(sg, t2[i].y, fmaf(sg, t1[i].y, t0[i].y)),
                                            fmaf(sg, t2[i].z, fmaf(sg, t1[i].z, t0[i].z)), fmaf(sg, t2[i].w, fmaf(sg, t1[i].w, t0[i].w))));
            }
        }
        return;
    }
    if (epi == RAMNET_EPI_GRU_BLEND) run(std::integral_constant<int, 2>{});
    else if (epi == RAMNET_EPI_RES_RELU) run(std::integral_constant<int, 1>{});
    else if (epi == RAMNET_EPI_GRU_BWD && n0 >= p.Cout / 2) run(std::integral_constant<int, 3>{});
    else if (epi == RAMNET_EPI_SIGMOID) run(std::integral_constant<int, 4>{});
    else if (epi == RAMNET_EPI_SIGMOID_HR) run(std::integral_constant<int, 5>{});
    else run(std::integral_constant<int, 0>{});
#ifdef RAMNET_PROBE
    __builtin_amdgcn_s_waitcnt(0);
    RAMNET_STAMP(6);
    if (threadIdx.x == 0 && blockIdx.x < 16384) g_probe6[blockIdx.x * 16 + 10] = __builtin_amdgcn_s_memrealtime();
#endif
}

__global__ void pack_weight_wino_r6_kernel(const float *__restrict__ w, float *__restrict__ wp, int Cout, int Cin, int transposed,
                                           int gates, int R, int N, int nchunks, int nblk, size_t total) {
    for (size_t i = blockIdx.x * (size_t)blockDim.x + threadIdx.x; i < total; i += (size_t)gridDim.x * blockDim.x) {
        const int j = (int)(i & 3), lane = (int)((i >> 2) & 63), f = (int)((i >> 8) & 1);
        size_t jj = i >> 9;
        const int pl = (int)(jj % 6);
        jj /= 6;
        const int wv = (int)(jj & 3);
        jj >>= 2;
        const int nb = (int)(jj % nblk), chunk = (int)(jj / nblk);
        const int n = f * 32 + (lane & 31);
        const int r = chunk * WK + 4 * (lane >> 5) + j;
        int no = nb * W6_BN + n;
        if (gates > 1) no = ((lane & 31) >> 3) * (N / gates) + nb * 16 + f * 8 + (lane & 7);
        float v = 0.f;
        if (r < R && no < N) {
            double g[3][3];
            for (int a = 0; a < 3; ++a)
                for (int bb = 0; bb < 3; ++bb)
                    g[a][bb] = transposed ? (double)w[((size_t)r * Cin + no) * 9 + (2 - a) * 3 + (2 - bb)]
                                          : (double)w[((size_t)no * Cin + r) * 9 + a * 3 + bb];
            const double G2[4][3] = {{1, 0, 0}, {0.5, 0.5, 0.5}, {0.5, -0.5, 0.5}, {0, 0, 1}};
            const double G4[6][3] = {{1.0 / 4, 0, 0},           {-1.0 / 6, -1.0 / 6, -1.0 / 6}, {-1.0 / 6, 1.0 / 6, -1.0 / 6},
                                     {1.0 / 24, 1.0 / 12, 1.0 / 6}, {1.0 / 24, -1.0 / 12, 1.0 / 6}, {0, 0, 1}};
            double s = 0;
            for (int a = 0; a < 3; ++a)
                for (int bb = 0; bb < 3; ++bb) s += G2[wv][a] * g[a][bb] * G4[pl][bb];
            v = (float)s;
        }
        wp[i] = v;
    }
}

static void wino6_geometry(int Cout, int Cin, int transposed, int &R, int &N, int &nchunks, int &nblk) {
    R = transposed ? Cout : Cin;
    N = transposed ? Cin : Cout;
    nchunks = cdiv(R, WK);
    nblk = cdiv(N, W6_BN);
}

static int g_w6_min_wgs = 150;

int wino6_eligible(const ramnet_conv_desc &d, int chunk, int force) {
    Wino6Plan pl;
    if (wino6_plan(d, chunk, pl, true) != 0) return 0;
    if (d.out_s2d && d.in_mode != RAMNET_IN_PLAIN && d.in_mode != RAMNET_IN_RELUMASK) return 0;
    if (force) return 1;
    int txg;
    const long a6 = wino6_tile(d.Ho, d.Wo, txg);
    const long a4t = (long)cdiv(d.Wo, 4) * 4 * cdiv(d.Ho, 32) * 32, a4w = (long)cdiv(d.Wo, 16) * 16 * cdiv(d.Ho, 8) * 8;
    const long a4 = a4t < a4w ? a4t : a4w;
    if (3 * a6 > 4 * a4 * 0.9) return 0;
    const long wgs = a6 / 256 * d.B * pl.q.nblk;
    return wgs >= g_w6_min_wgs ? 1 : 0;
}

int launch_wino6(const ramnet_conv_desc &d, hipStream_t st) {
    Wino6Plan pl;
    if (int rc = wino6_plan(d, WK, pl)) return rc;
    const bool lstm = d.epi == RAMNET_EPI_LSTM;
    if (lstm) note_kernel(d.active ? "conv_wino_r6_kernel<%d,%d,masked,lstm>" : "conv_wino_r6_kernel<%d,%d,lstm>", pl.txg, d.in_mode);
    else note_kernel(d.active ? "conv_wino_r6_kernel<%d,%d,masked>" : "conv_wino_r6_kernel<%d,%d>", pl.txg, d.in_mode);
    size_t probe_pad = 0;
#ifdef RAMNET_PROBE
    if (const char *e = getenv("RAMNET_PROBE_LDS_KB")) probe_pad = (size_t)atoi(e) * 1024;
#endif
#define RAMNET_GO6K(KEYv, TXv, ...)                                                                                 \
    case (KEYv) + (TXv) * 100: {                                                                                    \
        const size_t pf = (size_t)(2 * R6Geom<TXv>::PFLOATS + 256 * 4) * sizeof(float);                             \
        RAMNET_FULL_LDS((conv_wino_r6_kernel<TXv, __VA_ARGS__>));                                                   \
        hipLaunchKernelGGL((conv_wino_r6_kernel<TXv, __VA_ARGS__>), dim3(pl.grid), dim3(256), (pl.exchange > pf ? pl.exchange : pf) + probe_pad, st, d, pl.q); \
    } break;
#define RAMNET_GO6(TXv, MDv) RAMNET_GO6K(MDv, TXv, MDv)
#define RAMNET_GO6M(TXv, MDv) RAMNET_GO6K(100000 + (MDv), TXv, MDv, true)
#define RAMNET_GO6L(TXv, MSKv) RAMNET_GO6K(200000 + (MSKv) * 100000 + RAMNET_IN_CAT, TXv, RAMNET_IN_CAT, MSKv, true)
#define RAMNET_GO6_TX(TXv)                                                                                          \
    RAMNET_GO6L(TXv, false) RAMNET_GO6L(TXv, true)                                                                  \
    RAMNET_GO6M(TXv, RAMNET_IN_CAT) RAMNET_GO6M(TXv, RAMNET_IN_CAT_MUL)                                             \
    RAMNET_GO6(TXv, RAMNET_IN_PLAIN) RAMNET_GO6(TXv, RAMNET_IN_CAT) RAMNET_GO6(TXv, RAMNET_IN_CAT_MUL) RAMNET_GO6(TXv, RAMNET_IN_RELUMASK) \
    RAMNET_GO6(TXv, RAMNET_IN_S2D)
    switch (pl.txg * 100 + d.in_mode + (d.active ? 100000 : 0) + (lstm ? 200000 : 0)) {
        RAMNET_GO6_TX(4)
        RAMNET_GO6_TX(2)
        RAMNET_GO6_TX(8)
    default:
        RAMNET_CHECK_ARG(!"conv_wino_r6: unsupported (tile, input mode) combination");
    }
#undef RAMNET_GO6_TX
#undef RAMNET_GO6L
#undef RAMNET_GO6M
#undef RAMNET_GO6
#undef RAMNET_GO6K
    RAMNET_LAUNCH_CHECK();
    return 0;
}

}

using namespace ramnet;

#ifdef RAMNET_PROBE
extern "C" int ramnet_probe6_read(unsigned long long *dst, size_t n) {
    return hipMemcpyFromSymbol(dst, HIP_SYMBOL(ramnet::g_probe6), n * sizeof(unsigned long long)) == hipSuccess ? 0 : 1;
}
#endif

extern "C" int ramnet_wino2x4_config(int min_wgs) {
    if (min_wgs >= 0) g_w6_min_wgs = min_wgs;
    return 0;
}

extern "C" int ramnet_conv_wino_variant(const ramnet_conv_desc *d, int force) { return d ? wino6_eligible(*d, WK, force) : 0; }

extern "C" size_t ramnet_packed_weight_elems_wino2x4_gates(int Cout, int Cin, int transposed, int gates) {
    int R, N, nchunks, nblk;
    (void)gates;
    wino6_geometry(Cout, Cin, transposed, R, N, nchunks, nblk);
    return (size_t)nchunks * nblk * W6_U_FLOATS;
}

extern "C" size_t ramnet_packed_weight_elems_wino2x4(int Cout, int Cin, int transposed) {
    return ramnet_packed_weight_elems_wino2x4_gates(Cout, Cin, transposed, 1);
}

extern "C" int ramnet_pack_weight_wino2x4_gates(const float *w, float *wp, int Cout, int Cin, int transposed, int gates, void *stream) {
    RAMNET_CHECK_ARG(w && wp && Cout > 0 && Cin > 0);
    RAMNET_CHECK_ARG(gates == 1 || (gates == 4 && !transposed && Cout % 64 == 0));
    int R, N, nchunks, nblk;
    wino6_geometry(Cout, Cin, transposed, R, N, nchunks, nblk);
    const size_t total = (size_t)nchunks * nblk * W6_U_FLOATS;
    return launch_1d(pack_weight_wino_r6_kernel, total, stream, w, wp, Cout, Cin, transposed, gates, R, N, nchunks, nblk, total);
}

extern "C" int ramnet_pack_weight_wino2x4(const float *w, float *wp, int Cout, int Cin, int transposed, void *stream) {
    return ramnet_pack_weight_wino2x4_gates(w, wp, Cout, Cin, transposed, 1, stream);
}
```

rpg_ramnet_amd/csrc/conv_wino_common.hpp:

```cpp
#pragma once
#include "common.hpp"

namespace ramnet {

constexpr int WK = 8;

struct WinoParams {
    InSrc src;
    int nchunks, nblk;
    int tiles_x, tiles_y;
    int dy0, dx0;
    int vec4;
    int s2d_shift;
    int xg;
    int sparse;
    int ksplit;
    float *ws;
    int *cnt;
    float inv_nbl, inv_tx, inv_ty;
};

template <int MODE, int NS = 2, int QPP = 2>
struct WinoPatch {
    static_assert(QPP == 2 || QPP == 4, "quads per pixel");
    static constexpr bool CAT = MODE == RAMNET_IN_CAT || MODE == RAMNET_IN_CAT_MUL;
    float4 v[NS], m[NS];
    unsigned vo0[NS], vo1[NS], vom[NS];
    unsigned bad[NS];
    int ldst[NS];
    decltype(wino_rsrc(nullptr, 0u)) r0, r1, rm;

    template <int PH, int PW, int PWS = PW, int PLANE = PH * PW * 4, bool SKEW = false>
    __device__ __forceinline__ void init(const InSrc &s, int b, int iy0, int ix0, int tid, int clast, int scratch) {
        const bool s2d = MODE == RAMNET_IN_S2D;
        const size_t img = (size_t)(s2d ? 4 : 1) * s.Hin * s.Win;
        r0 = wino_rsrc(s.x0 + (size_t)b * img * s.ld0, (unsigned)(img * s.ld0 * 4));
        r1 = r0, rm = r0;
        if (CAT) r1 = wino_rsrc(s.x1 + (size_t)b * img * s.ld1, (unsigned)(img * s.ld1 * 4));
        if (MODE == RAMNET_IN_CAT_MUL || MODE == RAMNET_IN_RELUMASK) rm = wino_rsrc(s.xm + (size_t)b * img * s.ldm, (unsigned)(img * s.ldm * 4));
#pragma unroll
        for (int i = 0; i < NS; ++i) {
            const int sl = tid + i * 256;
            const int pix = sl / QPP, qd = sl % QPP;
            const int py = pix / PW, px = pix - py * PW;
            const int iy = iy0 + py, ix = ix0 + px;
            const bool slot = sl < PH * PW * QPP;
            const bool in = slot && (unsigned)iy < (unsigned)s.Hin && (unsigned)ix < (unsigned)s.Win;
            const unsigned gp = s2d ? (unsigned)((2 * iy) * 2 * s.Win + 2 * ix) : (unsigned)(iy * s.Win + ix);
            vo0[i] = in ? (gp * s.ld0 + qd * 4) * 4u : WOOB;
            vo1[i] = in ? (gp * s.ld1 + qd * 4) * 4u : WOOB;
            vom[i] = in ? (gp * s.ldm + qd * 4) * 4u : WOOB;
            bad[i] = clast + qd * 4 < s.Cin ? 0u : WOOB;
            ldst[i] = slot ? qd * PLANE + (py * PWS + px + (SKEW ? ((py >> 1) & 3) : 0)) * 4 : scratch + tid * 4;
        }
    }
    static __device__ __forceinline__ float4 bload(decltype(wino_rsrc(nullptr, 0u)) r, unsigned vo, int so) {
        return __builtin_bit_cast(float4, __builtin_amdgcn_raw_buffer_load_b128(r, (int)vo, so, 0));
    }
    __device__ __forceinline__ void load_slot_to(float4 &vo, float4 &mo, const InSrc &s, int c0, int i, int clast) {
        const unsigned last = c0 == clast ? 0xffffffffu : 0u;
        if (MODE == RAMNET_IN_S2D) {
            const int g = c0 >> s.ld1;
            vo = bload(r0, vo0[i] | (bad[i] & last), (((g >> 1) * 2 * s.Win + (g & 1)) * s.ld0 + (c0 - (g << s.ld1))) * 4);
        } else if (CAT) {
            const bool second = c0 >= s.C0;
            vo = bload(second ? r1 : r0, second ? (vo1[i] | (bad[i] & last)) : vo0[i], (second ? c0 - s.C0 : c0) * 4);
            if (MODE == RAMNET_IN_CAT_MUL) mo = bload(rm, second ? (vom[i] | (bad[i] & last)) : WOOB, (second ? c0 - s.C0 : 0) * 4);
        } else {
            vo = bload(r0, vo0[i] | (bad[i] & last), c0 * 4);
            if (MODE == RAMNET_IN_RELUMASK) mo = bload(rm, vom[i] | (bad[i] & last), c0 * 4);
        }
    }
    __device__ __forceinline__ void load_slot(const InSrc &s, int c0, int i, int clast) { load_slot_to(v[i], m[i], s, c0, i, clast); }
    __device__ __forceinline__ void load(const InSrc &s, int c0, int clast) {
#pragma unroll
        for (int i = 0; i < NS; ++i) load_slot(s, c0, i, clast);
    }
    __device__ __forceinline__ void store_regs(float *__restrict__ patch, const InSrc &s, int c0, int i, float4 r, float4 mk) const {
        if (MODE == RAMNET_IN_RELUMASK)
            r = make_float4(mk.x > 0.f ? r.x : 0.f, mk.y > 0.f ? r.y : 0.f, mk.z > 0.f ? r.z : 0.f, mk.w > 0.f ? r.w : 0.f);
        if (MODE == RAMNET_IN_CAT_MUL) {
            const float one = c0 >= s.C0 ? 0.f : 1.f;
            r = make_float4(r.x * (mk.x + one), r.y * (mk.y + one), r.z * (mk.z + one), r.w * (mk.w + one));
        }
        st4(patch + ldst[i], r);
    }
    __device__ __forceinline__ void store_slot(float *__restrict__ patch, const InSrc &s, int c0, int i) const { store_regs(patch, s, c0, i, v[i], m[i]); }
    __device__ __forceinline__ void store(float *__restrict__ patch, const InSrc &s, int c0) const {
#pragma unroll
        for (int i = 0; i < NS; ++i) store_slot(patch, s, c0, i);
    }
};

}
```

rpg_ramnet_amd/ops.py:

```python
import contextlib
import ctypes as C
import os as _os

import torch
from torch.autograd import Function

from . import _hip as H

_NULL = None
_ABL_SKIP_WGRAD = _os.environ.get("RAMNET_ABL_SKIP_WGRAD") == "1"
if _ABL_SKIP_WGRAD:
    import warnings as _warnings
    _warnings.warn("RAMNET_ABL_SKIP_WGRAD=1: backward-weights launches are SKIPPED — every weight gradient of this process is zero "
                   "(tuning runs only; unset the variable for anything else)", RuntimeWarning)

_WINOGRAD = True
_WINO_MIN_CIN = 32


def set_winograd(on):
    global _WINOGRAD
    _WINOGRAD = bool(on)


_WINO_2X4 = "auto"
_WGRAD_SLABS = True
_WGRAD_2X4 = "auto"


def set_wgrad_slabs(on):
    global _WGRAD_SLABS
    _WGRAD_SLABS = bool(on)



def set_winograd_2x4(mode, min_wgs=None):
    global _WINO_2X4
    assert mode in ("auto", "off", "force")
    _WINO_2X4 = mode
    if min_wgs is not None:
        H.check(H.lib().ramnet_wino2x4_config(int(min_wgs)), "wino2x4_config")
        invalidate_descs()


def get_winograd():
    return _WINOGRAD


_FOLD_UP = True


_FOLD_WINO = True
_FOLD_WINO_MIN_COUT = 32
_FOLD_WINO_WGRAD = True
_SAVE_XPAD = False


def set_fold_winograd_wgrad(on):
    global _FOLD_WINO_WGRAD
    _FOLD_WINO_WGRAD = bool(on)


def set_fold_pair(on):
    H.check(H.lib().ramnet_set_option(b"fold_pair", int(bool(on))), "set_option")
    invalidate_packs()
    invalidate_descs()


_GRU_BWD_FUSED = True


def set_gru_bwd_fused(on):
    global _GRU_BWD_FUSED
    _GRU_BWD_FUSED = bool(on)


_GRU_HR = _os.environ.get("RAMNET_GRU_HR", "1") != "0"


def set_gru_materialize_hr(on):
    global _GRU_HR
    _GRU_HR = bool(on)


_SPLIT_OPERANDS = False


def set_split_operands(on):
    global _SPLIT_OPERANDS
    _SPLIT_OPERANDS = bool(on)
    invalidate_descs()


def get_split_operands():
    return _SPLIT_OPERANDS


_SPLIT_WGRAD = _os.environ.get("RAMNET_SPLIT_WGRAD", "0") == "1"


def set_split_wgrad(on):
    global _SPLIT_WGRAD
    _SPLIT_WGRAD = bool(on)


def get_split_wgrad():
    return _SPLIT_WGRAD


def set_wgrad_winograd_2x4(mode):
    global _WGRAD_2X4
    assert mode in ("auto", "off", "force")
    _WGRAD_2X4 = mode


def set_winograd_split(on):
    H.check(H.lib().ramnet_set_option(b"wino_ksplit", int(on)), "set_option")
    invalidate_descs()


def _fold_pair(Cout, Cin):
    return Cout == 32 and Cin % 32 == 0 and bool(H.lib().ramnet_get_option(b"fold_pair"))


def _fold_wino_ok(Cin, Cout):
    kc = 16 if ((Cout % 64 == 0 and Cin % 16 == 0) or _fold_pair(Cout, Cin)) else 8
    return Cout % 32 == 0 and Cout >= _FOLD_WINO_MIN_COUT and Cin % (2 * kc) == 0


def set_fold_winograd(on):
    global _FOLD_WINO
    _FOLD_WINO = bool(on)


_FOLD_2X3 = "auto"


def set_fold_winograd_2x3(mode):
    global _FOLD_2X3
    assert mode in ("auto", "off", "force")
    _FOLD_2X3 = mode


def set_fold_upsample(on):
    global _FOLD_UP
    _FOLD_UP = bool(on)


def get_fold_upsample():
    return _FOLD_UP


_RAW_STREAM = getattr(torch._C, "_cuda_getCurrentRawStream", None)
_RAW_DEVICE = getattr(torch._C, "_cuda_getDevice", None)


def _st():
    if _RAW_STREAM is not None and _RAW_DEVICE is not None:
        return C.c_void_p(_RAW_STREAM(_RAW_DEVICE()))
    return C.c_void_p(torch.cuda.current_stream().cuda_stream)


def _p(t, off=0):
    return None if t is None else C.c_void_p(t.data_ptr() + 4 * off)


def dense(t):
    if t is None:
        return None
    B, Hh, W, Cc = t.shape
    s = t.stride()
    ok = (s[3] == 1 or Cc == 1) and s[2] % 4 == 0 and s[1] == W * s[2] and s[0] == Hh * s[1] and t.data_ptr() % 16 == 0
    if ok and t.dtype == torch.float32:
        return t
    return t.contiguous().float()


def ld(t):
    return t.stride(2)


class Taps:
    _cache = {}

    def __init__(self, triples):
        self.n = len(triples)
        assert 1 <= self.n <= 25
        self.dy = (C.c_int8 * 25)(*[t[0] for t in triples])
        self.dx = (C.c_int8 * 25)(*[t[1] for t in triples])
        self.wt = (C.c_uint8 * 25)(*[t[2] for t in triples])
        self.wino = False
        self.head = False
        self.flop_taps = self.n

    @classmethod
    def get(cls, kind, k, pad, py=0, px=0):
        key = (kind, k, pad, py, px)
        if key not in cls._cache:
            if kind in ("conv", "conv_s2d"):
                tr = [(kh - pad, kw - pad, kh * k + kw) for kh in range(k) for kw in range(k)]
            elif kind in ("dgrad1", "dgrad1_s2d"):
                tr = [(pad - kh, pad - kw, kh * k + kw) for kh in range(k) for kw in range(k)]
            elif kind == "dgrad2":
                tr = [((py + pad - kh) // 2, (px + pad - kw) // 2, kh * k + kw)
                      for kh in range(k) for kw in range(k)
                      if (py + pad - kh) % 2 == 0 and (px + pad - kw) % 2 == 0]
            elif kind == "fold":
                tr = [(py + ty, px + tx, (py * 2 + px) * 16 + ty * 4 + tx) for ty in range(4) for tx in range(4)]
            else:
                raise KeyError(kind)
            cls._cache[key] = cls(tr)
            cls._cache[key].wino = kind in ("conv", "dgrad1", "conv_s2d", "dgrad1_s2d") and k == 3 and pad == 1
            cls._cache[key].head = kind == "conv" and k == 5 and pad == 2
            if kind.endswith("_s2d"):
                cls._cache[key].flop_taps = 25.0 / 4.0
            if kind == "fold":
                cls._cache[key].flop_taps = 25
        return cls._cache[key]


def conv_launch(x0, taps, w, out, Cout, active=None, **kw):
    d = _conv_desc(x0, taps, w, out, Cout, **kw)
    if active is not None:
        d.active = _p(active)
    H.check(H.lib().ramnet_conv_launch(C.byref(d), _st()), "ramnet_conv_launch")


def conv_launch_multi(x0, w, out, Cout, classes, **kw):
    arr = (H.ConvDesc * len(classes))()
    if isinstance(w, PackRef):
        w = w.cp.pack(w.transposed, False)
    for i, (taps, Ho, Wo, os_) in enumerate(classes):
        arr[i] = _conv_desc(x0, taps, w, out, Cout, Ho=Ho, Wo=Wo, os=os_, **kw)
    H.check(H.lib().ramnet_conv_launch_multi(arr, len(classes), _st()), "ramnet_conv_launch_multi")


def uses_winograd(taps, w, stride, epi, in_mode, C0, C1):
    return bool(isinstance(w, PackRef) and _WINOGRAD and taps.wino and stride == 1
                and (w.cp.gates == 1 or w.transposed or (epi == H.EPI_LSTM and w.cp.Cout % 16 == 0))
                and (epi != H.EPI_LSTM or w.cp.gates == 4) and in_mode not in (H.IN_UP2X, H.IN_UP2X_SKIP)
                and C0 + C1 >= _WINO_MIN_CIN and (C1 == 0 or C0 % 8 == 0))


_HEAD = True


def set_head_kernel(on):
    global _HEAD
    _HEAD = bool(on)


def get_head_kernel():
    return _HEAD


def uses_head(taps, w, stride, epi, in_mode):
    return bool(isinstance(w, PackRef) and _HEAD and taps.head and stride == 1 and not w.transposed
                and w.cp.gates == 1 and len(w.cp.weights) == 1 and in_mode == H.IN_PLAIN and epi in (H.EPI_LINEAR, H.EPI_RELU)
                and H.lib().ramnet_head_supported(w.cp.Cin, w.cp.Cout))


_DESC_CACHE = {}
_DESC_EPOCH = 0
_DESC_CACHE_ON = _os.environ.get("RAMNET_DESC_CACHE", "1") != "0"


def invalidate_descs():
    global _DESC_EPOCH
    _DESC_EPOCH += 1
    _DESC_CACHE.clear()
    _WDESC_CACHE.clear()


def _sd(t):
    return -1 if t is None else t.stride(2)


def _conv_desc(x0, taps, w, out, Cout, *, stride=1, x1=None, xm=None, xm_off=0, in_mode=H.IN_PLAIN,
               C0=None, C1=0, Hin=None, Win=None, bias=None, epi=H.EPI_LINEAR, beta=0.0, e0=None, e1=None,
               o1=None, o2=None, Ho=None, Wo=None, os=(1, 1, 0, 0), out_off=0, frame=0, out_s2d=0, wino24=False, ws_owner=None):
    is_ref = isinstance(w, PackRef)
    al = out.data_ptr() | (4 * out_off)
    for t in (e0, e1, o1, o2, bias):
        if t is not None:
            al |= t.data_ptr()
    key = (id(taps), id(w.cp) if is_ref else 0, w.transposed if is_ref else -1, id(ws_owner), Cout, stride, in_mode, C0, C1, Hin, Win, epi, beta, Ho,
           Wo, os, out_off, frame, out_s2d, wino24, xm_off, tuple(x0.shape), x0.stride(2), _sd(x1), _sd(xm), out.shape[1], out.shape[2],
           out.stride(2), _sd(e0), _sd(e1), _sd(o1), _sd(o2), bias is None, al & 15, _WINOGRAD, _WINO_2X4, _SPLIT_OPERANDS, _HEAD, _S2D_SPARSE, _S2D_2X4,
           _FOLD_2X3, _DESC_EPOCH, x0.device.index)
    hit = _DESC_CACHE.get(key) if _DESC_CACHE_ON else None
    if hit is not None and (not is_ref or hit[3]() is w.cp) and (ws_owner is None or hit[4]() is ws_owner):
        tmpl, kind, nsplit = hit[0], hit[1], hit[2]
        d = H.ConvDesc.from_buffer_copy(tmpl)
        d.x0, d.x1, d.xm = _p(x0), _p(x1), _p(xm, xm_off)
        d.bias, d.e0, d.e1 = _p(bias), _p(e0), _p(e1)
        d.out, d.o1, d.o2 = _p(out, out_off), _p(o1), _p(o2)
        if kind in ("f23", "f23d"):
            d.w = _p(ws_owner.pack_fold_wino2x3_dgrad() if kind == "f23d" else ws_owner.pack_fold_wino2x3())
        else:
            d.w = _p(w) if kind is None else _p(w.cp.pack(0, "head") if kind == "head" else w.cp.pack(w.transposed, kind))
        if nsplit:
            d.splitk_ws = _p((w.cp if is_ref else ws_owner).splitk_ws(nsplit, x0.device))
        return d
    meta = []
    d = _conv_desc_build(x0, taps, w, out, Cout, meta, stride=stride, x1=x1, xm=xm, xm_off=xm_off, in_mode=in_mode, C0=C0, C1=C1, Hin=Hin, Win=Win,
                         bias=bias, epi=epi, beta=beta, e0=e0, e1=e1, o1=o1, o2=o2, Ho=Ho, Wo=Wo, os=os, out_off=out_off, frame=frame,
                         out_s2d=out_s2d, wino24=wino24, ws_owner=ws_owner)
    import weakref
    if len(_DESC_CACHE) > 4096:
        _DESC_CACHE.clear()
    _DESC_CACHE[key] = (H.ConvDesc.from_buffer_copy(d), meta[0], meta[1], weakref.ref(w.cp) if is_ref else None,
                        weakref.ref(ws_owner) if ws_owner is not None else None)
    return d


def _conv_desc_build(x0, taps, w, out, Cout, meta, *, stride=1, x1=None, xm=None, xm_off=0, in_mode=H.IN_PLAIN,
                     C0=None, C1=0, Hin=None, Win=None, bias=None, epi=H.EPI_LINEAR, beta=0.0, e0=None, e1=None,
                     o1=None, o2=None, Ho=None, Wo=None, os=(1, 1, 0, 0), out_off=0, frame=0, out_s2d=0, wino24=False, ws_owner=None):
    B = x0.shape[0]
    kind, nsplit = None, 0
    d = H.ConvDesc()
    d.x0, d.x1, d.xm = _p(x0), _p(x1), _p(xm, xm_off)
    d.ld0, d.ld1, d.ldm = ld(x0), (ld(x1) if x1 is not None else 0), (ld(xm) if xm is not None else 0)
    d.C0, d.C1, d.in_mode = (x0.shape[3] if C0 is None else C0), C1, in_mode
    d.algo = H.ALGO_DIRECT
    ref = None
    cp = w.cp if isinstance(w, PackRef) else ws_owner
    if isinstance(w, PackRef) and beta == 0.0 and frame == 0 and os == (1, 1, 0, 0) and uses_head(taps, w, stride, epi, in_mode):
        d.algo, d.head_cin = H.ALGO_HEAD, w.cp.Cin
        kind = "head"
        w = w.cp.pack(0, "head")
    elif isinstance(w, PackRef):
        wino = uses_winograd(taps, w, stride, epi, in_mode, d.C0, C1)
        d.algo = H.ALGO_WINOGRAD if wino else H.ALGO_DIRECT
        d.s2d_5x5 = int(wino and isinstance(w.cp, S2DConvParam) and _S2D_SPARSE and (in_mode == H.IN_S2D or out_s2d > 0))
        if (wino and (w.cp.gates == 1 or w.transposed or (epi == H.EPI_LSTM and w.cp.gates == 4)) and os == (1, 1, 0, 0)
                and (_S2D_2X4 or not isinstance(w.cp, S2DConvParam))):
            ref = w
        kind = bool(wino)
        w = w.cp.pack(w.transposed, wino)
    d.B, d.Hin, d.Win = B, (x0.shape[1] if Hin is None else Hin), (x0.shape[2] if Win is None else Win)
    d.ntaps, d.stride = taps.n, stride
    d.dy, d.dx, d.wtap = taps.dy, taps.dx, taps.wt
    d.w, d.bias = _p(w), _p(bias)
    d.Cout = Cout
    d.HoF, d.WoF = out.shape[1], out.shape[2]
    d.Ho, d.Wo = (d.HoF if Ho is None else Ho), (d.WoF if Wo is None else Wo)
    d.osy, d.osx, d.ooy, d.oox = os
    d.epi, d.beta, d.frame, d.out_s2d = epi, beta, frame, out_s2d
    d.e0, d.e1 = _p(e0), _p(e1)
    d.lde0, d.lde1 = (ld(e0) if e0 is not None else 0), (ld(e1) if e1 is not None else 0)
    d.out, d.o1, d.o2 = _p(out, out_off), _p(o1), _p(o2)
    d.ldo, d.ldo1, d.ldo2 = ld(out), (ld(o1) if o1 is not None else 0), (ld(o2) if o2 is not None else 0)
    if wino24:
        d.algo = H.ALGO_WINOGRAD24
    if ref is not None and _WINO_2X4 != "off" and H.lib().ramnet_conv_wino_variant(C.byref(d), int(_WINO_2X4 == "force")):
        d.algo, d.s2d_5x5 = H.ALGO_WINOGRAD_2X4, 0
        kind = "2x4g" if epi == H.EPI_LSTM else "2x4"
        if _SPLIT_OPERANDS and H.lib().ramnet_conv_wino_split_ok(C.byref(d), int(_WINO_2X4 == "force")):
            d.algo, kind = H.ALGO_WINOGRAD_2X4_SPLIT, "2x4s"
        d.w = _p(ref.cp.pack(ref.transposed, kind))
    if wino24 and cp is not None and _FOLD_2X3 != "off" and H.lib().ramnet_fold_wino_variant(C.byref(d), int(_FOLD_2X3 == "force")):
        kind = "f23d" if in_mode == H.IN_PARITY4 else "f23"
        d.algo = H.ALGO_WINOGRAD24_2X3
        d.w = _p(cp.pack_fold_wino2x3_dgrad() if kind == "f23d" else cp.pack_fold_wino2x3())
    if d.algo in (H.ALGO_WINOGRAD, H.ALGO_WINOGRAD24) and cp is not None:
        n = H.lib().ramnet_conv_splitk_floats(C.byref(d))
        if n:
            d.splitk_ws, d.splitk_floats = _p(cp.splitk_ws(n, x0.device)), n
            nsplit = n
    meta[:] = [kind, nsplit]
    return d


_WDESC_CACHE = {}


def _wgrad_desc_build(x0, taps, dout, dw, Cout, stride, x1, xm, xm_off, in_mode, C0, C1, Hin, Win, gmask, dbias, Ho, Wo, gview, dw_off, wino24):
    d = H.WgradDesc()
    d.x0, d.x1, d.xm = _p(x0), _p(x1), _p(xm, xm_off)
    d.ld0, d.ld1, d.ldm = ld(x0), (ld(x1) if x1 is not None else 0), (ld(xm) if xm is not None else 0)
    d.C0, d.C1, d.in_mode = (x0.shape[3] if C0 is None else C0), C1, in_mode
    d.B, d.Hin, d.Win = x0.shape[0], (x0.shape[1] if Hin is None else Hin), (x0.shape[2] if Win is None else Win)
    d.ntaps, d.stride = taps.n, stride
    d.dy, d.dx = taps.dy, taps.dx
    d.dout, d.gmask = _p(dout), _p(gmask)
    d.ldg, d.ldgm = ld(dout), (ld(gmask) if gmask is not None else 0)
    d.Cout, d.Ho, d.Wo = Cout, (dout.shape[1] if Ho is None else Ho), (dout.shape[2] if Wo is None else Wo)
    d.dw, d.dbias = _p(dw, dw_off), _p(dbias)
    if gview is not None:
        d.gsy, d.gsx, d.goy, d.gox, d.HoG, d.WoG = gview
    d.algo = H.ALGO_WINOGRAD if getattr(dw, "wino", False) else H.ALGO_DIRECT
    if getattr(dw, "wino6", False):
        d.algo = H.ALGO_WINOGRAD_2X4
    if getattr(dw, "wg_dsplit", False):
        d.algo = H.ALGO_DIRECT_SPLIT
    d.dw_slabs = getattr(dw, "slabs", 0) if (d.algo in (H.ALGO_WINOGRAD, H.ALGO_WINOGRAD_2X4, H.ALGO_DIRECT_SPLIT) and _WGRAD_SLABS) else 0
    if wino24:
        d.algo = H.ALGO_WINOGRAD24
    hc = getattr(dw, "head_cin", 0)
    if hc and _HEAD and taps.head and stride == 1 and in_mode == H.IN_PLAIN and gview is None and dw_off == 0:
        d.algo, d.head_cin = H.ALGO_HEAD, hc
    if d.algo in (H.ALGO_WINOGRAD, H.ALGO_WINOGRAD_2X4) and C1 and d.C0 % 32:
        raise RuntimeError("Winograd backward-weights needs the concatenation boundary at a multiple of 32 channels")
    return d


def wgrad_launch(x0, taps, dout, dw, Cout, *, stride=1, x1=None, xm=None, xm_off=0, in_mode=H.IN_PLAIN, C0=None,
                 C1=0, Hin=None, Win=None, gmask=None, dbias=None, Ho=None, Wo=None, gview=None, dw_off=0, wino24=False, segs=None, stream=None):
    key = (id(taps), id(dw), getattr(dw, "wino", False), getattr(dw, "wino6", False), getattr(dw, "wg_dsplit", False), getattr(dw, "slabs", 0), getattr(dw, "head_cin", 0), Cout, stride,
           in_mode, C0, C1, Hin, Win, Ho, Wo, gview, dw_off, wino24, xm_off, tuple(x0.shape), x0.stride(2), _sd(x1), _sd(xm), dout.shape[1],
           dout.shape[2], dout.stride(2), _sd(gmask), _WGRAD_SLABS, _HEAD, x0.device.index)
    tmpl = _WDESC_CACHE.get(key) if _DESC_CACHE_ON else None
    if tmpl is not None:
        d = H.WgradDesc.from_buffer_copy(tmpl)
        d.x0, d.x1, d.xm = _p(x0), _p(x1), _p(xm, xm_off)
        d.dout, d.gmask = _p(dout), _p(gmask)
        d.dw, d.dbias = _p(dw, dw_off), _p(dbias)
    else:
        d = _wgrad_desc_build(x0, taps, dout, dw, Cout, stride, x1, xm, xm_off, in_mode, C0, C1, Hin, Win, gmask, dbias, Ho, Wo, gview, dw_off, wino24)
        if len(_WDESC_CACHE) > 4096:
            _WDESC_CACHE.clear()
        _WDESC_CACHE[key] = H.WgradDesc.from_buffer_copy(d)
    if segs is not None:
        d.nseg, d.segs = len(segs), C.cast(segs, C.POINTER(H.WgradSeg))
    if _ABL_SKIP_WGRAD:
        return
    H.check(H.lib().ramnet_wgrad_launch(C.byref(d), _st() if stream is None else stream), "ramnet_wgrad_launch")


_SIDE = {}
_USE_SIDE = False


def set_wgrad_overlap(on):
    global _USE_SIDE
    _USE_SIDE = bool(on)
    H.check(H.lib().ramnet_set_option(b"wgrad_wino_nf", 2 if _USE_SIDE else 1), "set_option")


_DECODE = {}
_USE_DECODE = False
_DECODE_USED = set()


def set_decoder_overlap(on):
    global _USE_DECODE
    _USE_DECODE = bool(on)


def decoder_overlap():
    return _USE_DECODE


def decode_stream(dev):
    st = _DECODE.get(dev)
    if st is None:
        st = _DECODE[dev] = torch.cuda.Stream(device=dev)
    _DECODE_USED.add(dev)
    return st


_BRANCH = {}
_USE_BRANCH = False


def set_branch_overlap(on):
    global _USE_BRANCH
    _USE_BRANCH = bool(on)


def branch_overlap():
    return _USE_BRANCH


def branch_stream(dev, i):
    st = _BRANCH.get((dev, i))
    if st is None:
        st = _BRANCH[(dev, i)] = torch.cuda.Stream(device=dev)
    return st


def _side_stream(dev):
    st = _SIDE.get(dev)
    if st is None:
        st = _SIDE[dev] = torch.cuda.Stream(device=dev)
    return st


@contextlib.contextmanager
def side_work(tensors, dev):
    if not _USE_SIDE:
        yield
        return
    side = _side_stream(dev)
    side.wait_event(torch.cuda.current_stream().record_event())
    with torch.cuda.stream(side):
        yield
    for t in tensors:
        if t is not None:
            t.record_stream(side)
    _Engine.side_used = dev


def wgrad_side(tensors, *args, **kw):
    if not _USE_SIDE:
        return wgrad_launch(*args, **kw)
    dev = args[0].device
    side = _side_stream(dev)
    raw = C.c_void_p(side.cuda_stream)
    H.check(H.lib().ramnet_stream_fork(_st(), raw), "ramnet_stream_fork")
    wgrad_launch(*args, stream=raw, **kw)
    for t in tensors:
        if t is not None:
            t.record_stream(side)
    _Engine.side_used = dev


_WGRAD_DEFER = 0


def set_wgrad_defer(n):
    global _WGRAD_DEFER
    n = int(n)
    assert 0 <= n <= H.WGRAD_MAX_SEGMENTS
    _WGRAD_DEFER = n


def wgrad_defer():
    return _WGRAD_DEFER


def _wgrad_cell(cp, dw, tensors, x0, taps, dout, Cout, **kw):
    if _WGRAD_DEFER <= 1 or not getattr(dw, "wino6", False) or not _WGRAD_SLABS:
        return wgrad_side(tensors, x0, taps, dout, dw, Cout, **kw)
    x1, xm = kw.get("x1"), kw.get("xm")
    key = (id(dw), tuple(x0.shape), ld(x0), ld(x1) if x1 is not None else 0, ld(xm) if xm is not None else 0, ld(dout), Cout,
           kw.get("in_mode"), kw.get("C1"), kw.get("xm_off", 0), x0.device)
    q = cp._defer
    if q and q[0][0] != key:
        cp.flush_deferred()
    cp._defer.append((key, tensors, x0, taps, dout, dw, Cout, kw))
    if len(cp._defer) >= _WGRAD_DEFER:
        cp.flush_deferred()


_ZERO_BATCH = None


def _zero_later(t):
    if _ZERO_BATCH is None:
        t.zero_()
    else:
        _ZERO_BATCH.append(t)


class _Engine:
    dirty = []
    task = -1
    side_used = None

    @classmethod
    def enter(cls):
        tid = torch._C._current_graph_task_id()
        if tid != cls.task:
            if cls.dirty:
                cls.reset()
            cls.task = tid
            if tid != -1:
                torch.autograd.Variable._execution_engine.queue_callback(cls.flush)

    @classmethod
    def mark(cls, cp):
        cls.enter()
        if not cp._dirty:
            cp._dirty = True
            cls.dirty.append(cp)

    @classmethod
    def _join(cls):
        for dev in _DECODE_USED:
            torch.cuda.current_stream(dev).wait_stream(_DECODE[dev])
        if cls.side_used is not None:
            torch.cuda.current_stream().wait_event(_side_stream(cls.side_used).record_event())
            cls.side_used = None

    @classmethod
    def flush(cls):
        for cp in cls.dirty:
            cp.flush_deferred()
        cls._join()
        dirty, cls.dirty, cls.task = cls.dirty, [], -1
        hook = _FINALIZE_HOOK if (_FINALIZE_HOOK is not None and not (torch.cuda.is_available() and torch.cuda.is_current_stream_capturing())) else None
        if hook is not None:
            hook.begin(dirty)
        global _ZERO_BATCH
        _ZERO_BATCH = []
        try:
            for cp in dirty:
                cp.finalize()
                if hook is not None:
                    hook.finalized(cp)
        finally:
            zs, _ZERO_BATCH = _ZERO_BATCH, None
            zs = [z for z in zs if z.numel() > 0]
            if zs:
                torch._foreach_zero_(zs)
        if hook is not None and hasattr(hook, "end"):
            hook.end()

    @classmethod
    def reset(cls):
        for cp in cls.dirty:
            cp._defer = []
        cls._join()
        dirty, cls.dirty, cls.task = cls.dirty, [], -1
        for cp in dirty:
            cp.discard()


_FINALIZE_HOOK = None


def set_finalize_hook(hook):
    global _FINALIZE_HOOK
    _FINALIZE_HOOK = hook


def get_finalize_hook():
    return _FINALIZE_HOOK


def ensure_grad(p):
    if p.grad is None:
        p.grad = torch.zeros_like(p)
    return p.grad


FOLD_A = ([[.25, 0, 0, 0, 0], [.75, .75, .25, 0, 0], [0, .25, .75, .75, .25], [0, 0, 0, .25, .75]],
          [[.75, .25, 0, 0, 0], [.25, .75, .75, .25, 0], [0, 0, .25, .75, .75], [0, 0, 0, 0, .25]])


_CONSTS = {}


def _const(name, values, device, dtype):
    key = (name, str(device), dtype)
    t = _CONSTS.get(key)
    if t is None:
        t = _CONSTS[key] = torch.tensor(values, dtype=dtype, device=device)
    return t


def fold_weights(w):
    A = _const("FOLD_A", FOLD_A, w.device, torch.float64)
    return torch.einsum("ptk,qsl,oikl->oipqts", A, A, w.double())


S2D_TAP = [(-1, 0), (-1, 1), (0, 0), (0, 1), (1, 0)]


def s2d_weights(w):
    O, I = w.shape[0], w.shape[1]
    out = w.new_zeros(O, 4, I, 3, 3)
# ... 557 lines not shown
                    wgrad_launch(xpad, Taps.get("fold", 4, 0, py, px), dy, w4, cp.Cout, gmask=y, dbias=bws, Ho=Hh, Wo=W,
                                 gview=(2, 2, py, px, H2, W2), dw_off=(py * 2 + px) * 16 * cp.CinWs * cp.Cout)
        g_rows = torch.empty(2, B * W2, 2 * cp.Cout, device=dev)
        g_cols = torch.empty(2, B * H2, 2 * cp.Cout, device=dev)
        H.check(L.ramnet_frame_gather(_p(dy), _p(y), _p(g_rows), _p(g_cols), B, H2, W2, cp.Cout, _st()), "ramnet_frame_gather")
        gemm2(a_rows, g_rows, wr, a_cols, g_cols, wc, trans_a=True, accumulate=True)


_FOLD_DGRAD = True


def set_fold_dgrad(on):
    global _FOLD_DGRAD
    _FOLD_DGRAD = bool(on)


def _fold_dgrad_ok(B, H2, W2, cp):
    return bool(_FOLD_DGRAD and _FOLD_UP and cp.Cout % 16 == 0 and cp.Cin % 64 == 0
                and B * H2 * W2 * cp.Cout * 4 < 2 ** 30)


def _folded_upsample_dgrad(x, dy, y, cp):
    L = H.lib()
    B, Hh, W, Cc = x.shape
    H2, W2 = 2 * Hh, 2 * W
    dev = x.device
    g = dy
    if y is not None:
        g = torch.empty_like(dy)
        H.check(L.ramnet_relu_bwd(_p(dy), _p(y), _p(g), dy.numel(), _st()), "ramnet_relu_bwd")
    dxpad = torch.empty(B, Hh + 4, W + 4, Cc, device=dev)
    conv_launch(g, Taps.get("fold", 4, 0, 0, 0), cp.pack_fold_wino_dgrad(), dxpad, Cc, in_mode=H.IN_PARITY4, wino24=True, ws_owner=cp)
    dx = torch.empty(B, Hh, W, Cc, device=dev)
    H.check(L.ramnet_unpad2_fold(_p(dxpad), _p(dx), B, Hh, W, Cc, _st()), "ramnet_unpad2_fold")
    g_rows = torch.empty(2, B * W2, 2 * cp.Cout, device=dev)
    g_cols = torch.empty(2, B * H2, 2 * cp.Cout, device=dev)
    H.check(L.ramnet_frame_gather(_p(g), None, _p(g_rows), _p(g_cols), B, H2, W2, cp.Cout, _st()), "ramnet_frame_gather")
    wt_rows, wt_cols = cp.border_weights_t()
    d_rows = torch.empty(2, B * W2, 5 * Cc, device=dev)
    d_cols = torch.empty(2, B * H2, 5 * Cc, device=dev)
    gemm2(g_rows, wt_rows, d_rows, g_cols, wt_cols, d_cols)
    H.check(L.ramnet_up2x_border_col2im(_p(d_rows), _p(d_cols), _p(dx), B, Hh, W, Cc, _st()), "ramnet_up2x_border_col2im")
    return dx


class ConvAct(Function):

    @staticmethod
    def forward(ctx, x, skip, w, b, cp, stride, relu, up):
        x, skip = dense(x), dense(skip)
        if skip is not None and skip.shape != x.shape:
            raise RuntimeError("skip connection %s does not match the decoder feature map %s (NHWC)" % (tuple(skip.shape), tuple(x.shape)))
        if x.shape[3] != (cp.Cin + 3) // 4 * 4:
            raise RuntimeError("conv expects %d input channels, got %d" % (cp.Cin, x.shape[3]))
        B, Hh, W, _ = x.shape
        k, pad = cp.k, cp.k // 2
        Hin, Win = (2 * Hh, 2 * W) if up else (Hh, W)
        Ho, Wo = (Hin + 2 * pad - k) // stride + 1, (Win + 2 * pad - k) // stride + 1
        y = torch.empty(B, Ho, Wo, cp.Cout, device=x.device)
        mode = (H.IN_UP2X_SKIP if skip is not None else H.IN_UP2X) if up else H.IN_PLAIN
        epi = H.EPI_RELU if relu else H.EPI_LINEAR
        xpad = None
        ctx.s2d = _s2d_eligible(x, cp, k, stride, up)
        ctx.s2d_fused = ctx.s2d and _s2d_fused(x.shape[3])
        if ctx.s2d_fused:
            conv_launch(x, Taps.get("conv_s2d", 3, 1), cp.s2d().fwd(), y, cp.Cout, in_mode=H.IN_S2D, Hin=Hh // 2, Win=W // 2,
                        bias=cp.bias(), epi=epi)
        elif ctx.s2d:
            x = _space_to_depth(x)
            conv_launch(x, Taps.get("conv_s2d", 3, 1), cp.s2d().fwd(), y, cp.Cout, bias=cp.bias(), epi=epi)
        elif _fold_eligible(x, cp, k, stride, up):
            xpad = _folded_upsample_conv(x, skip, cp, y, epi)
        else:
            conv_launch(x, Taps.get("conv", k, pad), cp.fwd(), y, cp.Cout, stride=stride, x1=skip, in_mode=mode,
                        Hin=Hin, Win=Win, bias=cp.bias(), epi=epi)
        ctx.cp, ctx.stride, ctx.relu, ctx.up, ctx.mode = cp, stride, relu, up, mode
        ctx.premask_ok, ctx.premasked = bool(relu), False
        ctx.save_for_backward(x, skip, y, xpad if _SAVE_XPAD else None)
        return y

    @staticmethod
    def backward(ctx, dy):
        x, skip, y, xpad = ctx.saved_tensors
        cp, stride, relu, up, mode = ctx.cp, ctx.stride, ctx.relu, ctx.up, ctx.mode
        relu = relu and not ctx.premasked
        dy = dense(dy)
        if ctx.s2d_fused:
            sp = cp.s2d()
            ws, bws = sp.grad_ws(wino_ok=True)
            Hl, Wl = x.shape[1] // 2, x.shape[2] // 2
            wgrad_side([x, dy, y], x, Taps.get("conv_s2d", 3, 1), dy, ws, cp.Cout, in_mode=H.IN_S2D, Hin=Hl, Win=Wl,
                       gmask=y if relu else None, dbias=bws)
            dx = None
            if ctx.needs_input_grad[0]:
                dx = torch.empty_like(x)
                conv_launch(dy, Taps.get("dgrad1_s2d", 3, 1), sp.bwd(), dx, sp.Cin, xm=y if relu else None,
                            in_mode=H.IN_RELUMASK if relu else H.IN_PLAIN, Ho=Hl, Wo=Wl, out_s2d=x.shape[3])
            return dx, None, None, None, None, None, None, None
        if ctx.s2d:
            sp = cp.s2d()
            ws, bws = sp.grad_ws(wino_ok=True)
            wgrad_side([x, dy, y], x, Taps.get("conv_s2d", 3, 1), dy, ws, cp.Cout, gmask=y if relu else None, dbias=bws)
            dx = None
            if ctx.needs_input_grad[0]:
                gs = torch.empty_like(x)
                conv_launch(dy, Taps.get("dgrad1_s2d", 3, 1), sp.bwd(), gs, sp.Cin, xm=y if relu else None,
                            in_mode=H.IN_RELUMASK if relu else H.IN_PLAIN)
                dx = _space_to_depth(gs, inverse=True)
            return dx, None, None, None, None, None, None, None
        B, Hh, W, _ = x.shape
        k, pad = cp.k, cp.k // 2
        Hin, Win = (2 * Hh, 2 * W) if up else (Hh, W)
        if _fold_eligible(x, cp, k, stride, up):
            dy = dy.contiguous()
            _folded_upsample_wgrad(x, skip, dy, y if relu else None, cp, xpad)
        else:
            ws, bws = cp.grad_ws(wino_ok=(stride == 1 and k == 3 and pad == 1 and mode == H.IN_PLAIN))
            wgrad_side([x, skip, dy, y], x, Taps.get("conv", k, pad), dy, ws, cp.Cout, stride=stride, x1=skip, in_mode=mode,
                       Hin=Hin, Win=Win, gmask=y if relu else None, dbias=bws)
        dx = dskip = None
        if (ctx.needs_input_grad[0] or (skip is not None and ctx.needs_input_grad[1])) and _fold_eligible(x, cp, k, stride, up) \
                and _fold_dgrad_ok(B, Hin, Win, cp):
            dx = _folded_upsample_dgrad(x, dy, y if relu else None, cp)
            return dx, (dx if skip is not None else None), None, None, None, None, None, None
        if ctx.needs_input_grad[0] or (skip is not None and ctx.needs_input_grad[1]):
            gin = torch.empty(B, Hin, Win, cp.Cin, device=x.device)
            gmode = H.IN_RELUMASK if relu else H.IN_PLAIN
            if stride == 1:
                conv_launch(dy, Taps.get("dgrad1", k, pad), cp.bwd(), gin, cp.Cin, xm=y if relu else None, in_mode=gmode)
            else:
                conv_launch_multi(dy, cp.bwd(), gin, cp.Cin,
                                  [(Taps.get("dgrad2", k, pad, py, px), (Hin - py + 1) // 2, (Win - px + 1) // 2, (2, 2, py, px))
                                   for py in range(2) for px in range(2)], xm=y if relu else None, in_mode=gmode)
            if up:
                dx = torch.empty(B, Hh, W, cp.Cin, device=x.device)
                H.check(H.lib().ramnet_upsample2x_bwd(_p(gin), _p(dx), B, Hh, W, cp.Cin, _st()), "ramnet_upsample2x_bwd")
            else:
                dx = gin
            dskip = dx if skip is not None else None
        return dx, dskip, None, None, None, None, None, None


class TConvAct(Function):

    @staticmethod
    def forward(ctx, x, w, b, cp, relu=True):
        x = dense(x)
        B, Hh, W, _ = x.shape
        Ct = cp.Cin
        y = torch.empty(B, 2 * Hh, 2 * W, Ct, device=x.device)
        conv_launch_multi(x, cp.bwd(), y, Ct, [(Taps.get("dgrad2", 5, 2, py, px), Hh, W, (2, 2, py, px))
                                               for py in range(2) for px in range(2)], bias=cp.bias(),
                          epi=H.EPI_RELU if relu else H.EPI_LINEAR)
        ctx.cp, ctx.relu = cp, relu
        ctx.save_for_backward(x, y)
        return y

    @staticmethod
    def backward(ctx, dy):
        x, y = ctx.saved_tensors
        cp = ctx.cp
        dy = dense(dy)
        B, Hh, W, Cx = x.shape
        taps = Taps.get("conv", 5, 2)
        ws, _ = cp.grad_ws()
        mask, mode = (y, H.IN_RELUMASK) if ctx.relu else (None, H.IN_PLAIN)
        wgrad_launch(dy, taps, x, ws, Cx, stride=2, xm=mask, in_mode=mode)
        if cp.biases[0] is not None:
            dyc = dy.contiguous()
            H.check(H.lib().ramnet_bias_grad(_p(dyc), _p(mask), _p(ensure_grad(cp.biases[0])), B * 4 * Hh * W, cp.Cin, _st()), "bias_grad")
        dx = None
        if ctx.needs_input_grad[0]:
            dx = torch.empty(B, Hh, W, Cx, device=x.device)
            conv_launch(dy, taps, cp.fwd(), dx, Cx, stride=2, xm=mask, in_mode=mode)
        return dx, None, None, None, None


class ResConv(Function):

    @staticmethod
    def forward(ctx, t, res, w, b, cp):
        t, res = dense(t), dense(res)
        assert t.shape == res.shape
        y = torch.empty_like(res, memory_format=torch.contiguous_format)
        conv_launch(t, Taps.get("conv", 3, 1), cp.fwd(), y, cp.Cout, bias=cp.bias(), epi=H.EPI_RES_RELU, e0=res)
        ctx.cp = cp
        ctx.save_for_backward(t, y)
        return y

    @staticmethod
    def backward(ctx, dy):
        t, y = ctx.saved_tensors
        cp = ctx.cp
        dy = dense(dy).contiguous()
        dpre = torch.empty_like(y)
        H.check(H.lib().ramnet_relu_bwd(_p(dy), _p(y), _p(dpre), y.numel(), _st()), "ramnet_relu_bwd")
        ws, bws = cp.grad_ws(wino_ok=True)
        wgrad_side([t, dpre], t, Taps.get("conv", 3, 1), dpre, ws, cp.Cout, dbias=bws)
        dt = torch.empty_like(t, memory_format=torch.contiguous_format)
        conv_launch(dpre, Taps.get("dgrad1", 3, 1), cp.bwd(), dt, cp.Cin)
        dres = dpre
        if _USE_SIDE:
            dres = torch.empty_like(y)
            H.check(H.lib().ramnet_relu_bwd(_p(dy), _p(y), _p(dres), y.numel(), _st()), "ramnet_relu_bwd")
        return dt, dres, None, None, None


def _norm_partial(a, y, act, b, groups):
    B, Hh, W, Cc = b.shape
    npix = B * Hh * W // groups
    L = H.lib()
    nslab = L.ramnet_norm_slabs(groups, npix, Cc)
    part = torch.empty(groups, nslab, Cc, 2, device=b.device, dtype=torch.float64)
    H.check(L.ramnet_norm_partial(_p(a), Cc, _p(y), Cc, act, _p(b), Cc, groups, npix, Cc, nslab, _p(part), _st()), "ramnet_norm_partial")
    return part, nslab, npix


def norm_stats(x, groups):
    part, _, npix = _norm_partial(x, None, 0, x, groups)
    s = part.sum(1)
    mean = s[..., 0] / npix
    return mean, (s[..., 1] / npix - mean * mean).clamp_(min=0.0)


class NormAct(Function):

    @staticmethod
    def forward(ctx, x, gamma, beta, res, mean, rstd, scale, shift, batch_stats, act):
        x, res = dense(x).contiguous(), (dense(res).contiguous() if res is not None else None)
        B, Hh, W, Cc = x.shape
        groups = mean.shape[0]
        y = torch.empty_like(x)
        H.check(H.lib().ramnet_norm_apply(_p(x), Cc, _p(scale), _p(shift), _p(res), Cc, act, _p(y), Cc, groups, B * Hh * W // groups, Cc,
                                          _st()), "ramnet_norm_apply")
        ctx.batch_stats, ctx.act, ctx.has_res = batch_stats, act, res is not None
        ctx.save_for_backward(x, y, gamma, mean, rstd)
        return y

    @staticmethod
    def backward(ctx, dy):
        x, y, gamma, mean, rstd = ctx.saved_tensors
        dy = dense(dy).contiguous()
        Cc = x.shape[3]
        groups, act, L = mean.shape[0], ctx.act, H.lib()
        part, nslab, npix = _norm_partial(dy, y if act else None, act, x, groups)
        c = torch.empty(3, groups, Cc, device=x.device)
        dgb = torch.empty(2, Cc, device=x.device) if gamma is not None else None
        H.check(L.ramnet_norm_finalize_bwd(_p(part), groups, nslab, Cc, npix, _p(mean), _p(rstd), _p(gamma.detach()) if gamma is not None else None,
                                           int(ctx.batch_stats), _p(c[0]), _p(c[1]), _p(c[2]), _p(dgb[0]) if dgb is not None else None,
                                           _p(dgb[1]) if dgb is not None else None, _st()), "ramnet_norm_finalize_bwd")
        dx = torch.empty_like(x)
        dres = torch.empty_like(x) if ctx.has_res else None
        H.check(L.ramnet_norm_bwd(_p(dy), Cc, _p(y) if act else None, Cc, act, _p(x), Cc, _p(c[0]), _p(c[1]), _p(c[2]), _p(dx), Cc, _p(dres), Cc,
                                  groups, npix, Cc, _st()), "ramnet_norm_bwd")
        return dx, (dgb[0] if dgb is not None else None), (dgb[1] if dgb is not None else None), dres, None, None, None, None, None, None


_ACT_CODE = {None: 0, "relu": 1, "sigmoid": 2}


def norm_act(x, layer, act=None, res=None):
    x = dense(x).contiguous()
    B, Hh, W, Cc = x.shape
    inst = isinstance(layer, torch.nn.InstanceNorm2d)
    tracked = layer.running_mean is not None
    use_input = layer.training or not tracked
    groups = (B if inst else 1) if use_input else 1
    npix = B * Hh * W // groups
    update = bool(tracked and layer.training)
    if update and npix < 2:
        raise ValueError("Expected more than 1 value per channel when training, got input size %s" % ([B, Cc, Hh, W],))
    if update and layer.momentum is None:
        raise NotImplementedError("cumulative moving average (momentum=None): the reference builds its norm layers with momentum 0.1")
    dev = x.device
    mr = torch.empty(2, groups, Cc, device=dev, dtype=torch.float64)
    ss = torch.empty(2, groups, Cc, device=dev)
    part, nslab = None, 0
    if use_input:
        part, nslab, _ = _norm_partial(x, None, 0, x, groups)
    g, b = layer.weight, layer.bias
    H.check(H.lib().ramnet_norm_finalize(_p(part), groups, nslab, Cc, npix, float(layer.eps), _p(g.detach()) if g is not None else None,
                                         _p(b.detach()) if b is not None else None, _p(layer.running_mean), _p(layer.running_var),
                                         float(layer.momentum or 0.0), int(update), int(not use_input),
                                         _p(layer.num_batches_tracked) if (update and not inst) else None,
                                         _p(mr[0]), _p(mr[1]), _p(ss[0]), _p(ss[1]), _st()), "ramnet_norm_finalize")
    return NormAct.apply(x, g, b, res, mr[0], mr[1], ss[0], ss[1], use_input, _ACT_CODE[act])


def active_mask(active, B, device):
    if active is None:
        return None
    if not torch.is_tensor(active) or active.dim() != 1 or active.shape[0] != B:
        raise ValueError("active: a bool / integer tensor of shape [%d] expected, got %s" % (
            B, tuple(active.shape) if torch.is_tensor(active) else type(active).__name__))
    if active.dtype.is_floating_point or active.is_complex():
        raise ValueError("active: a bool / integer tensor expected, got %s" % active.dtype)
    if active.device.type == "cpu":
        return (active != 0).to(torch.int32).to(device)
    if active.device != device:
        raise ValueError("active: on %s, the cell runs on %s" % (active.device, device))
    return active if (active.dtype == torch.int32 and active.is_contiguous()) else (active != 0).to(torch.int32).contiguous()


class GRUCell(Function):

    @staticmethod
    def forward(ctx, x, h, wu, bu, wr, br, wo, bo, cp_ur, cp_o, out=None, active=None):
        x, h = dense(x), dense(h)
        act = active_mask(active, x.shape[0], x.device)
        if x.shape != h.shape:
            raise RuntimeError("Sizes of tensors must match except in dimension 1. Expected %s but got %s (input vs state; "
                               "NHWC)" % (tuple(x.shape), tuple(h.shape)))
        B, Hh, W, Cc = x.shape
        taps = Taps.get("conv", 3, 1)
        ur = torch.empty(B, Hh, W, 2 * Cc, device=x.device)
        hr = torch.empty(B, Hh, W, Cc, device=x.device) if (_GRU_HR and Cc % 4 == 0) else None
        if hr is not None:
            conv_launch(x, taps, cp_ur.fwd(), ur, 2 * Cc, x1=h, in_mode=H.IN_CAT, C1=Cc, bias=cp_ur.bias(), epi=H.EPI_SIGMOID_HR, e1=h, o1=hr,
                        active=act)
        else:
            conv_launch(x, taps, cp_ur.fwd(), ur, 2 * Cc, x1=h, in_mode=H.IN_CAT, C1=Cc, bias=cp_ur.bias(), epi=H.EPI_SIGMOID, active=act)
        hn = torch.empty(B, Hh, W, Cc, device=x.device) if out is None else out
        if out is not None:
            if tuple(out.shape) != (B, Hh, W, Cc) or not out.is_contiguous() or out.dtype != torch.float32:
                raise RuntimeError("GRUCell: `out` must be a contiguous fp32 NHWC buffer of the state's shape")
            ctx.mark_dirty(out)
        need = any(ctx.needs_input_grad)
        o = torch.empty_like(hn) if need else None
        if hr is not None:
            conv_launch(x, taps, cp_o.fwd(), hn, Cc, x1=hr, in_mode=H.IN_CAT, C1=Cc, bias=cp_o.bias(), epi=H.EPI_GRU_BLEND, e0=ur, e1=h, o1=o,
                        active=act)
        else:
            conv_launch(x, taps, cp_o.fwd(), hn, Cc, x1=h, xm=ur, xm_off=Cc, in_mode=H.IN_CAT_MUL, C1=Cc, bias=cp_o.bias(),
                        epi=H.EPI_GRU_BLEND, e0=ur, e1=h, o1=o, active=act)
        ctx.cps = (cp_ur, cp_o)
        ctx.has_hr = hr is not None
        if need:
            ctx.save_for_backward(*((x, h, ur, o, hr) if hr is not None else (x, h, ur, o)))
        return hn

    @staticmethod
    def backward(ctx, dhn):
        if ctx.has_hr:
            x, h, ur, o, hr = ctx.saved_tensors
        else:
            (x, h, ur, o), hr = ctx.saved_tensors, None
        cp_ur, cp_o = ctx.cps
        B, Hh, W, Cc = x.shape
        npix = B * Hh * W
        dhn = dense(dhn)
        L = H.lib()
        dpo = torch.empty_like(o)
        dpur = torch.empty_like(ur)
        dxh = torch.empty(B, Hh, W, 2 * Cc, device=x.device)
        taps, tapsd = Taps.get("conv", 3, 1), Taps.get("dgrad1", 3, 1)
        fused = _GRU_BWD_FUSED and Cc % 64 == 0
        if fused:
            H.check(L.ramnet_gru_bwd_a2(_p(dhn), _p(ur), _p(o), _p(h), _p(dpo), _p(dpur), _p(dxh, Cc), npix, Cc, ld(dhn), 2 * Cc, _st()), "gru_bwd_a2")
        else:
            dhd = torch.empty_like(o)
            H.check(L.ramnet_gru_bwd_a(_p(dhn), _p(ur), _p(o), _p(h), _p(dpo), _p(dpur), _p(dhd), npix, Cc, ld(dhn), _st()), "gru_bwd_a")
        ws, bws = cp_o.grad_ws(wino_ok=Cc % 32 == 0)
        if hr is not None:
            _wgrad_cell(cp_o, ws, [x, hr, dpo], x, taps, dpo, Cc, x1=hr, in_mode=H.IN_CAT, C1=Cc, dbias=bws)
        else:
            _wgrad_cell(cp_o, ws, [x, h, ur, dpo], x, taps, dpo, Cc, x1=h, xm=ur, xm_off=Cc, in_mode=H.IN_CAT_MUL, C1=Cc, dbias=bws)
        if fused:
            conv_launch(dpo, tapsd, cp_o.bwd(), dxh, 2 * Cc, epi=H.EPI_GRU_BWD, e0=ur, e1=h, o1=dpur)
        else:
            conv_launch(dpo, tapsd, cp_o.bwd(), dxh, 2 * Cc)
            H.check(L.ramnet_gru_bwd_b(_p(dxh), _p(ur), _p(h), _p(dpur), _p(dhd), npix, Cc, _st()), "gru_bwd_b")
        ws, bws = cp_ur.grad_ws(wino_ok=Cc % 32 == 0)
        _wgrad_cell(cp_ur, ws, [x, h, dpur], x, taps, dpur, 2 * Cc, x1=h, in_mode=H.IN_CAT, C1=Cc, dbias=bws)
        conv_launch(dpur, tapsd, cp_ur.bwd(), dxh, 2 * Cc, beta=1.0)
        return dxh[..., :Cc], dxh[..., Cc:], None, None, None, None, None, None, None, None, None, None


_TIME_BATCH = True


_TIME_BATCH_MAX_DECODES = 0


def set_time_batching(on, max_decodes=None):
    global _TIME_BATCH, _TIME_BATCH_MAX_DECODES
    _TIME_BATCH = bool(on)
    if max_decodes is not None:
        _TIME_BATCH_MAX_DECODES = int(max_decodes)


def time_batch_max_decodes():
    return _TIME_BATCH_MAX_DECODES


def time_batching():
    return _TIME_BATCH


_RELU_PREMASK = True


def set_relu_premask(on):
    global _RELU_PREMASK
    _RELU_PREMASK = bool(on)


def get_relu_premask():
    return _RELU_PREMASK


def premask_relu_feature(y):
    fn = getattr(y, "grad_fn", None)
    if not (_RELU_PREMASK and fn is not None and getattr(fn, "premask_ok", False)):
        return False
    fn.premasked = True
    return True


def _cat_batch_add(grads, base, shape, device, mask=None):
    n = len(grads)
    ok = (len(shape) == 4 and n <= 8 and shape[3] % 4 == 0 and all(g is not None and g.is_cuda and g.dim() == 4 and g.dtype == torch.float32 for g in grads)
          and (base is None or base.dtype == torch.float32))
    if ok:
        gs = [dense(g) for g in grads]
        ok = all(ld(g) == ld(gs[0]) and g.stride(1) == g.shape[2] * g.stride(2) and g.stride(0) == g.shape[1] * g.stride(1)
                 and tuple(g.shape) == (shape[0] // n,) + tuple(shape[1:]) for g in gs)
    if not ok:
        filled = [g if g is not None else torch.zeros((shape[0] // n,) + tuple(shape[1:]), device=device) for g in grads]
        out = torch.cat(filled, 0)
        out = out if base is None else out + base
        return out if mask is None else out * (mask > 0).to(out.dtype)
    out = torch.empty(shape, device=device)
    arr = (C.c_void_p * n)(*[g.data_ptr() for g in gs])
    b = None if base is None else base.contiguous()
    npix = shape[1] * shape[2] * (shape[0] // n)
    if mask is not None:
        assert tuple(mask.shape) == tuple(shape) and mask.is_contiguous() and mask.dtype == torch.float32
        H.check(H.lib().ramnet_cat_batch_add_masked(arr, n, npix, shape[3], ld(gs[0]), _p(b), _p(mask), _p(out), _st()), "ramnet_cat_batch_add_masked")
    else:
        H.check(H.lib().ramnet_cat_batch_add(arr, n, npix, shape[3], ld(gs[0]), _p(b), _p(out), _st()), "ramnet_cat_batch_add")
    return out


def arena_slots(n, shape, device):
    buf = torch.empty((n,) + tuple(shape), device=device, dtype=torch.float32)
    numel = buf[0].numel()
    st = buf.untyped_storage()
    slots = [torch.empty(0, device=device, dtype=torch.float32).set_(st, buf.storage_offset() + k * numel, tuple(shape)) for k in range(n)]
    return buf, slots


class TimeSplit(Function):

    @staticmethod
    def forward(ctx, x, n, premask=False):
        B = x.shape[0] // n
        ctx.meta = (n, tuple(x.shape), x.device)
        ctx.set_materialize_grads(False)
        ctx.premask = bool(premask) and x.is_contiguous()
        if ctx.premask:
            ctx.save_for_backward(x)
        return tuple(x[k * B:(k + 1) * B] for k in range(n))

    @staticmethod
    def backward(ctx, *grads):
        n, shape, dev = ctx.meta
        mask = ctx.saved_tensors[0] if ctx.premask else None
        if all(g is None for g in grads):
            return None, None, None
        return _cat_batch_add(list(grads), None, shape, dev, mask), None, None


class TimeFan(Function):

    @staticmethod
    def forward(ctx, x, n, premask=False):
        B = x.shape[0] // n
        ctx.meta = (n, tuple(x.shape), x.device)
        ctx.set_materialize_grads(False)
        ctx.premask = bool(premask) and x.is_contiguous()
        if ctx.premask:
            ctx.save_for_backward(x)
        return (x.view_as(x),) + tuple(x[k * B:(k + 1) * B] for k in range(n))

    @staticmethod
    def backward(ctx, g_all, *grads):
        n, shape, dev = ctx.meta
        mask = ctx.saved_tensors[0] if ctx.premask else None
        if all(g is None for g in grads):
            if mask is not None and g_all is not None:
                if g_all.is_cuda:
                    g_all = dense(g_all)
                    out = torch.empty_like(g_all)
                    H.check(H.lib().ramnet_relu_bwd(_p(g_all), _p(mask), _p(out), g_all.numel(), _st()), "ramnet_relu_bwd")
                    g_all = out
                else:
                    g_all = g_all * (mask > 0).to(g_all.dtype)
            return g_all, None, None
        return _cat_batch_add(list(grads), g_all, shape, dev, mask), None, None


class TimeJoin(Function):

    @staticmethod
    def forward(ctx, joined, *parts):
        B = parts[0].shape[0]
        step = parts[0].numel() * parts[0].element_size()
        for i, t in enumerate(parts):
            if t.data_ptr() != joined.data_ptr() + i * step or not t.is_contiguous():
                raise RuntimeError("TimeJoin: part %d is not slot %d of the joined buffer" % (i, i))
        ctx.meta = (len(parts), B)
        return joined.view(joined.shape)

    @staticmethod
    def backward(ctx, g):
        n, B = ctx.meta
        g = dense(g)
        return (None,) + tuple(g[i * B:(i + 1) * B] for i in range(n))


class LSTMCell(Function):

    @staticmethod
    def forward(ctx, x, h, c, w, b, cp, out_h=None, out_c=None, active=None):
        x, h, c = dense(x), dense(h), dense(c)
        act = active_mask(active, x.shape[0], x.device)
        if x.shape != h.shape or x.shape != c.shape:
            raise RuntimeError("Sizes of tensors must match except in dimension 1. Expected %s but got %s / %s (input vs "
                               "hidden / cell state; NHWC)" % (tuple(x.shape), tuple(h.shape), tuple(c.shape)))
        B, Hh, W, Cc = x.shape
        hn = torch.empty(B, Hh, W, Cc, device=x.device) if out_h is None else out_h
        cn = torch.empty_like(hn) if out_c is None else out_c
        for t in (out_h, out_c):
            if t is not None and (tuple(t.shape) != (B, Hh, W, Cc) or not t.is_contiguous() or t.dtype != torch.float32):
                raise RuntimeError("LSTMCell: `out_h` / `out_c` must be contiguous fp32 NHWC buffers of the state's shape")
        dirty = [t for t in (out_h, out_c) if t is not None]
        if dirty:
            ctx.mark_dirty(*dirty)
        need = any(ctx.needs_input_grad)
        gates = torch.empty(B, Hh, W, 4 * Cc, device=x.device) if need else None
        if act is None:
            conv_launch(x, Taps.get("conv", 3, 1), cp.fwd(), hn, Cc, x1=h, in_mode=H.IN_CAT, C1=Cc, bias=cp.bias(),
                        epi=H.EPI_LSTM, e1=c, o1=cn, o2=gates)
        else:
            conv_launch(x, Taps.get("conv", 3, 1), cp.fwd(), hn, Cc, x1=h, in_mode=H.IN_CAT, C1=Cc, bias=cp.bias(),
                        epi=H.EPI_LSTM, e0=h, e1=c, o1=cn, o2=gates, active=act)
        ctx.cp = cp
        ctx.active = act
        if need:
            ctx.save_for_backward(x, h, c, cn, gates)
        return hn, cn

    @staticmethod
    def backward(ctx, dhn, dcn):
        x, h, c, cn, gates = ctx.saved_tensors
        cp = ctx.cp
        B, Hh, W, Cc = x.shape
        npix = B * Hh * W
        dhn = None if dhn is None else dense(dhn).contiguous()
        dcn = None if dcn is None else dense(dcn).contiguous()
        dpre = torch.empty_like(gates)
        dc = torch.empty_like(cn)
        dxh = torch.empty(B, Hh, W, 2 * Cc, device=x.device)
        if ctx.active is None:
            H.check(H.lib().ramnet_lstm_bwd(_p(gates), _p(c), _p(cn), _p(dhn), _p(dcn), _p(dpre), _p(dc), npix, Cc, _st()), "lstm_bwd")
        else:
            H.check(H.lib().ramnet_lstm_bwd_masked(_p(gates), _p(c), _p(cn), _p(dhn), _p(dcn), _p(ctx.active), _p(dpre), _p(dc), _p(dxh),
                                                   npix, Hh * W, Cc, _st()), "lstm_bwd_masked")
        ws, bws = cp.grad_ws(wino_ok=x.shape[3] % 32 == 0)
        wgrad_side([x, h, dpre], x, Taps.get("conv", 3, 1), dpre, ws, 4 * Cc, x1=h, in_mode=H.IN_CAT, C1=Cc, dbias=bws)
        conv_launch(dpre, Taps.get("dgrad1", 3, 1), cp.bwd(), dxh, 2 * Cc, beta=0.0 if ctx.active is None else 1.0)
        return dxh[..., :Cc], dxh[..., Cc:], dc, None, None, None, None, None, None


class PredSigmoid(Function):

    @staticmethod
    def forward(ctx, x, w, b):
        x = dense(x)
        B, Hh, W, Cc = x.shape
        y = torch.empty(B, 1, Hh, W, device=x.device)
        H.check(H.lib().ramnet_pred_sigmoid_fwd(_p(x), ld(x), Cc, _p(w.detach()), _p(b.detach()), _p(y), B * Hh * W, _st()), "pred_fwd")
        ctx.save_for_backward(x, w, b, y)
        return y

    @staticmethod
    def backward(ctx, dy):
        x, w, b, y = ctx.saved_tensors
        B, Hh, W, Cc = x.shape
        dy = dy.contiguous()
        dx = torch.empty(B, Hh, W, Cc, device=x.device) if ctx.needs_input_grad[0] else None
        H.check(H.lib().ramnet_pred_sigmoid_bwd(_p(x), ld(x), Cc, _p(w.detach()), _p(y), _p(dy), _p(dx), Cc,
                                                _p(ensure_grad(w)), _p(ensure_grad(b)), B * Hh * W, _st()), "pred_bwd")
        return dx, None, None


_SI_FUSION = True


def set_si_fusion(on):
    global _SI_FUSION
    _SI_FUSION = bool(on)


def si_fusion():
    return _SI_FUSION


class PredSigmoidSI(Function):

    @staticmethod
    def forward(ctx, x, w, b, weight, n_lambda, mask_x, *targets):
        x = dense(x)
        B, Hh, W, Cc = x.shape
        n = len(targets)
        assert 1 <= n <= 8 and B % n == 0
        seg_pix = (B // n) * Hh * W
        tg = [t.contiguous() for t in targets]
        for t in tg:
            assert t.is_cuda and t.dtype == torch.float32 and t.numel() == seg_pix, "PredSigmoidSI: one [B/n, 1, H, W] fp32 target per segment"
        L = H.lib()
        y = torch.empty(B, 1, Hh, W, device=x.device)
        scratch = torch.zeros(L.ramnet_pred_si_scratch_doubles(seg_pix, n), device=x.device, dtype=torch.float64)
        stats = torch.empty(n, 4, device=x.device, dtype=torch.float64)
        loss = torch.empty(n, device=x.device)
        arr = (C.c_void_p * n)(*[t.data_ptr() for t in tg])
        H.check(L.ramnet_pred_sigmoid_si_fwd(_p(x), ld(x), Cc, _p(w.detach()), _p(b.detach()), _p(y), seg_pix, n, arr, weight, n_lambda,
                                             _p(scratch), _p(stats), _p(loss), _st()), "pred_si_fwd")
        ctx.save_for_backward(x, w, b, y, stats, scratch, *tg)
        ctx.meta = (weight, n_lambda, n, seg_pix, bool(mask_x))
        ctx.set_materialize_grads(False)
        return (y,) + tuple(loss[i] for i in range(n))

    @staticmethod
    def backward(ctx, dy, *dloss):
        x, w, b, y, stats, scratch = ctx.saved_tensors[:6]
        tg = ctx.saved_tensors[6:]
        weight, n_lambda, n, seg_pix, mask_x = ctx.meta
        B, Hh, W, Cc = x.shape
        dy = dy.contiguous() if dy is not None else None
        if all(g is None for g in dloss):
            gs = torch.zeros(n, device=x.device)
        else:
            gs = torch.stack([g.float().reshape(()) if g is not None else torch.zeros((), device=x.device) for g in dloss])
        dx = torch.empty(B, Hh, W, Cc, device=x.device) if ctx.needs_input_grad[0] else None
        arr = (C.c_void_p * n)(*[t.data_ptr() for t in tg])
        join = scratch.numel() == H.lib().ramnet_pred_si_scratch_doubles(seg_pix, n)
        H.check(H.lib().ramnet_pred_sigmoid_si_bwd(_p(x), ld(x), Cc, _p(w.detach()), _p(y), _p(dy), seg_pix, n, arr, _p(stats), _p(gs), weight,
                                                   n_lambda, _p(dx), Cc, _p(ensure_grad(w)), _p(ensure_grad(b)), _p(scratch) if join else None, int(mask_x), _st()), "pred_si_bwd")
        return (dx, None, None, None, None, None) + (None,) * n


class PredLinear(Function):

    @staticmethod
    def forward(ctx, x, w, b):
        x = dense(x)
        B, Hh, W, Cc = x.shape
        z = torch.empty(B, Hh, W, 1, device=x.device)
        H.check(H.lib().ramnet_pred_linear_fwd(_p(x), ld(x), Cc, _p(w.detach()), _p(b.detach()) if b is not None else None, _p(z),
                                               B * Hh * W, _st()), "pred_linear_fwd")
        ctx.save_for_backward(x, w, b)
        return z

    @staticmethod
    def backward(ctx, dz):
        x, w, b = ctx.saved_tensors
        B, Hh, W, Cc = x.shape
        dz = dz.contiguous()
        dx = torch.empty(B, Hh, W, Cc, device=x.device) if ctx.needs_input_grad[0] else None
        H.check(H.lib().ramnet_pred_linear_bwd(_p(x), ld(x), Cc, _p(w.detach()), _p(dz), _p(dx), Cc, _p(ensure_grad(w)),
                                               _p(ensure_grad(b)) if b is not None else None, B * Hh * W, _st()), "pred_linear_bwd")
        return dx, None, None


class SILoss(Function):

# ... 360 lines not shown
```

Before: 234.7 samples/s.

## Merge GRU backward dgrad convs into split-Cin Winograd launch for x-half

Restructures the ConvGRU backward data-gradient. The candidate-gate dgrad now computes only the h-half of the output channels. The update/reset dgrad is merged with the x-half of the candidate-gate dgrad into one Winograd F(2x4) launch over concatenated [dpur, dpo] inputs, using a per-column-block split of input-chunk count and beta. This removes redundant MACs on the half of the output that was previously overwritten or accumulated twice, and avoids a separate read-modify-write pass. In exchange it adds kernel parameters, a new split launch path, and extra packed-weight variants.

```diff
diff --git a/include/ramnet_hip.h b/include/ramnet_hip.h
--- a/include/ramnet_hip.h
+++ b/include/ramnet_hip.h
@@ -152,6 +152,7 @@
                                 void *stream);
 
 int ramnet_conv_launch(const ramnet_conv_desc *d, void *stream);
+int ramnet_conv_launch_split(const ramnet_conv_desc *d, int n_split, int c_lo, float beta_hi, void *stream);
 int ramnet_conv_launch_multi(const ramnet_conv_desc *descs, int n, void *stream);
 int ramnet_wgrad_launch(const ramnet_wgrad_desc *d, void *stream);
 
diff --git a/rpg_ramnet_amd/_hip.py b/rpg_ramnet_amd/_hip.py
--- a/rpg_ramnet_amd/_hip.py
+++ b/rpg_ramnet_amd/_hip.py
@@ -120,6 +120,7 @@
     "ramnet_unpack_wgrad_wino": (C.c_int, [_fp, _fp] + [C.c_int] * 5 + [_fp]),
     "ramnet_unpack_wgrad_wino2x4": (C.c_int, [_fp, _fp] + [C.c_int] * 5 + [_fp]),
     "ramnet_conv_launch": (C.c_int, [C.POINTER(ConvDesc), _fp]),
+    "ramnet_conv_launch_split": (C.c_int, [C.POINTER(ConvDesc), C.c_int, C.c_int, C.c_float, _fp]),
     "ramnet_conv_launch_multi": (C.c_int, [C.POINTER(ConvDesc), C.c_int, _fp]),
     "ramnet_wgrad_launch": (C.c_int, [C.POINTER(WgradDesc), _fp]),
     "ramnet_pred_sigmoid_fwd": (C.c_int, [_fp, C.c_int, C.c_int, _fp, _fp, _fp, C.c_size_t, _fp]),
diff --git a/rpg_ramnet_amd/csrc/common.hpp b/rpg_ramnet_amd/csrc/common.hpp
--- a/rpg_ramnet_amd/csrc/common.hpp
+++ b/rpg_ramnet_amd/csrc/common.hpp
@@ -18,6 +18,7 @@
 void note_kernel(const char *fmt, ...);
 int launch_wino(const ramnet_conv_desc &d, hipStream_t st);
 size_t wino24_splitk_floats(const ramnet_conv_desc &d);
+int check_conv_desc(const ramnet_conv_desc &d);
 int launch_wino6(const ramnet_conv_desc &d, hipStream_t st);
 int launch_wino6s(const ramnet_conv_desc &d, hipStream_t st);
 int launch_head(const ramnet_conv_desc &d, hipStream_t st);
diff --git a/rpg_ramnet_amd/csrc/conv_igemm.hip b/rpg_ramnet_amd/csrc/conv_igemm.hip
--- a/rpg_ramnet_amd/csrc/conv_igemm.hip
+++ b/rpg_ramnet_amd/csrc/conv_igemm.hip
@@ -191,7 +191,7 @@
     return 0;
 }
 
-static int check_desc(const ramnet_conv_desc &d) {
+int check_conv_desc(const ramnet_conv_desc &d) {
     RAMNET_CHECK_ARG(d.x0 && d.w && d.out);
     RAMNET_CHECK_ARG(d.ntaps >= 1 && d.ntaps <= 25 && (d.stride == 1 || d.stride == 2));
     RAMNET_CHECK_ARG(d.B > 0 && d.Ho > 0 && d.Wo > 0 && d.Hin > 0 && d.Win > 0 && d.Cout > 0);
@@ -227,7 +227,7 @@
 static int launch_classes(const ramnet_conv_desc *ds, int n, hipStream_t st) {
     const ramnet_conv_desc &d = ds[0];
     for (int i = 0; i < n; ++i) {
-        const int rc = check_desc(ds[i]);
+        const int rc = check_conv_desc(ds[i]);
         if (rc) return rc;
         RAMNET_CHECK_ARG(ds[i].x0 == d.x0 && ds[i].w == d.w && ds[i].out == d.out && ds[i].stride == d.stride &&
                          ds[i].Cout == d.Cout && ds[i].epi == d.epi && ds[i].osy == d.osy && ds[i].osx == d.osx &&
@@ -297,23 +297,23 @@
 extern "C" int ramnet_conv_launch(const ramnet_conv_desc *dp, void *stream) {
     RAMNET_CHECK_ARG(dp != nullptr);
     if (dp->algo == RAMNET_ALGO_WINOGRAD) {
-        const int rc = check_desc(*dp);
+        const int rc = check_conv_desc(*dp);
         return rc ? rc : launch_wino(*dp, (hipStream_t)stream);
     }
     if (dp->algo == RAMNET_ALGO_WINOGRAD_2X4) {
-        const int rc = check_desc(*dp);
+        const int rc = check_conv_desc(*dp);
         return rc ? rc : launch_wino6(*dp, (hipStream_t)stream);
     }
     if (dp->algo == RAMNET_ALGO_WINOGRAD_2X4_SPLIT) {
-        const int rc = check_desc(*dp);
+        const int rc = check_conv_desc(*dp);
         return rc ? rc : launch_wino6s(*dp, (hipStream_t)stream);
     }
     if (dp->algo == RAMNET_ALGO_WINOGRAD24 || dp->algo == RAMNET_ALGO_WINOGRAD24_2X3) {
-        const int rc = check_desc(*dp);
+        const int rc = check_conv_desc(*dp);
         return rc ? rc : launch_wino24(*dp, (hipStream_t)stream);
     }
     if (dp->algo == RAMNET_ALGO_HEAD) {
-        const int rc = check_desc(*dp);
+        const int rc = check_conv_desc(*dp);
         return rc ? rc : launch_head(*dp, (hipStream_t)stream);
     }
     RAMNET_CHECK_ARG(dp->algo == RAMNET_ALGO_DIRECT && dp->in_mode != RAMNET_IN_S2D && dp->out_s2d == 0);
diff --git a/rpg_ramnet_amd/csrc/conv_plan.hpp b/rpg_ramnet_amd/csrc/conv_plan.hpp
--- a/rpg_ramnet_amd/csrc/conv_plan.hpp
+++ b/rpg_ramnet_amd/csrc/conv_plan.hpp
@@ -104,8 +104,14 @@
     size_t exchange;
 };
 
-inline int wino6_plan(const ramnet_conv_desc &d, int chunk, Wino6Plan &out, bool quiet = false) {
+struct Wino6Split {
+    int n_split, c_lo;
+    float beta_hi;
+};
+
+inline int wino6_plan(const ramnet_conv_desc &d, int chunk, Wino6Plan &out, bool quiet = false, const Wino6Split *sp = nullptr) {
     const bool split = chunk == WKS;
+    if (sp) RAMNET_PLAN_CHECK(!split && d.epi != RAMNET_EPI_LSTM && sp->n_split >= 0 && sp->n_split % W6_BN == 0 && sp->n_split <= d.Cout);
     RAMNET_PLAN_CHECK(d.ntaps == 9 && d.stride == 1 && !d.frame);
     const bool lstm = d.epi == RAMNET_EPI_LSTM;
     if (lstm) RAMNET_PLAN_CHECK(!split && wino6_lstm_ok(d) && (!d.active || d.e0));
@@ -117,7 +123,7 @@
     if (d.in_mode == RAMNET_IN_CAT || d.in_mode == RAMNET_IN_CAT_MUL) RAMNET_PLAN_CHECK(d.C0 % chunk == 0);
     RAMNET_PLAN_CHECK(conv_vec4(d, false) && d.osy == 1 && d.osx == 1 && d.ooy == 0 && d.oox == 0);
     if (d.out_s2d) RAMNET_PLAN_CHECK(out_s2d_ok(d));
-    if (d.epi == RAMNET_EPI_GRU_BWD) RAMNET_PLAN_CHECK(d.Cout % 128 == 0);
+    if (d.epi == RAMNET_EPI_GRU_BWD) RAMNET_PLAN_CHECK(sp ? sp->n_split == 0 : d.Cout % 128 == 0);
     int dy0, dx0;
     RAMNET_PLAN_CHECK(taps_3x3(d.dy, d.dx, false, dy0, dx0));
     if (int rc = check_offsets32(d, lstm && d.o2, quiet)) return rc;
@@ -125,6 +131,13 @@
     q = WinoParams{};
     fill_in_src(d, q.src);
     q.nchunks = cdiv(q.src.Cin, chunk), q.nblk = cdiv(ncol, W6_BN);
+    q.n_split = 0, q.nchunks_lo = q.nchunks, q.beta_hi = d.beta;
+    q.gru_col0 = sp ? 0 : d.Cout / 2;
+    if (sp && sp->n_split > 0) {
+        RAMNET_PLAN_CHECK((d.epi == RAMNET_EPI_LINEAR || d.epi == RAMNET_EPI_RELU) && !d.out_s2d && d.in_mode != RAMNET_IN_S2D);
+        RAMNET_PLAN_CHECK(sp->c_lo > 0 && sp->c_lo % chunk == 0 && sp->c_lo <= q.src.Cin);
+        q.n_split = sp->n_split, q.nchunks_lo = sp->c_lo / chunk, q.beta_hi = sp->beta_hi;
+    }
     wino6_tile(d.Ho, d.Wo, out.txg);
     q.tiles_x = cdiv(d.Wo, 4 * out.txg), q.tiles_y = cdiv(d.Ho, 2 * (32 / out.txg));
     q.dy0 = dy0, q.dx0 = dx0;
diff --git a/rpg_ramnet_amd/csrc/conv_wino6.hip b/rpg_ramnet_amd/csrc/conv_wino6.hip
--- a/rpg_ramnet_amd/csrc/conv_wino6.hip
+++ b/rpg_ramnet_amd/csrc/conv_wino6.hip
@@ -81,11 +81,11 @@
 #pragma unroll
             for (int r = 0; r < 16; ++r) acc[i][f][r] = 0.f;
 
-    const int nch = q.nchunks;
+    const int nch = n0 < q.n_split ? q.nchunks : q.nchunks_lo;
     const int clast = (nch - 1) * WK;
     WinoPatch<MODE, 3> pr;
     pr.template init<G::PH, G::PW, G::PWS, G::PLANE, true>(q.src, b, iy0, ix0, tid, clast, 2 * RP_FLOATS);
-    const auto wrs = wino_rsrc(p.w, (unsigned)((size_t)nch * q.nblk * W6_U_FLOATS * sizeof(float)));
+    const auto wrs = wino_rsrc(p.w, (unsigned)((size_t)q.nchunks * q.nblk * W6_U_FLOATS * sizeof(float)));
     const unsigned wvo = (unsigned)((wave * 3072 + fh * 256 + lane * 4) * 4);
     const int wblk = nblk_i * W6_U_FLOATS * 4, wchunk = q.nblk * W6_U_FLOATS * 4;
     auto wload = [&](int chunk, int i) {
@@ -292,14 +292,15 @@
     }
     auto run = [&](auto kind) {
         constexpr int K = decltype(kind)::value;
-        const bool addold = K == 0 && p.beta != 0.f && (epi == RAMNET_EPI_RELU || epi == RAMNET_EPI_LINEAR);
+        const float beta = n0 < q.n_split ? q.beta_hi : p.beta;
+        const bool addold = K == 0 && beta != 0.f && (epi == RAMNET_EPI_RELU || epi == RAMNET_EPI_LINEAR);
         const bool relu = epi == RAMNET_EPI_RELU;
         const auto r_e0 = (K >= 1 && K <= 3) ? rsrc_of(p.e0, p.lde0) : r_out;
         const auto r_e1 = (K == 2 || K == 3 || K == 5) ? rsrc_of(p.e1, p.lde1) : r_out;
         const auto r_o1 = (K == 2 || K == 3 || K == 5) ? rsrc_of(p.o1, p.ldo1) : r_out;
         const unsigned o_out = off0_of(p.ldo, true), s_out = step_of(p.ldo);
         const unsigned o_e0 = off0_of(p.lde0, K >= 1 && K <= 3), s_e0 = step_of(p.lde0);
-        const unsigned o_e1 = off0_of(p.lde1, ((K == 2 || K == 3) && p.e1 != nullptr) || (K == 5 && nq >= p.Cout / 2), (K == 3 || K == 5) ? -(p.Cout / 2) : 0), s_e1 = step_of(p.lde1);
+        const unsigned o_e1 = off0_of(p.lde1, ((K == 2 || K == 3) && p.e1 != nullptr) || (K == 5 && nq >= p.Cout / 2), K == 3 ? -q.gru_col0 : K == 5 ? -(p.Cout / 2) : 0), s_e1 = step_of(p.lde1);
         const unsigned o_o1 = off0_of(p.ldo1, ((K == 2 || K == 3) && p.o1 != nullptr) || (K == 5 && nq >= p.Cout / 2), K == 5 ? -(p.Cout / 2) : 0), s_o1 = step_of(p.ldo1);
 #pragma unroll
         for (int half = 0; half < 2; ++half) {
@@ -328,7 +329,7 @@
                                        fmaf(sg, t2[i].z, fmaf(sg, t1[i].z, t0[i].z)), fmaf(sg, t2[i].w, fmaf(sg, t1[i].w, t0[i].w)));
                 v = f4add(v, bias4);
                 if (K == 0) {
-                    if (addold) v = make_float4(v.x + p.beta * ea[i].x, v.y + p.beta * ea[i].y, v.z + p.beta * ea[i].z, v.w + p.beta * ea[i].w);
+                    if (addold) v = make_float4(v.x + beta * ea[i].x, v.y + beta * ea[i].y, v.z + beta * ea[i].z, v.w + beta * ea[i].w);
                     if (relu) v = make_float4(fmaxf(v.x, 0.f), fmaxf(v.y, 0.f), fmaxf(v.z, 0.f), fmaxf(v.w, 0.f));
                 } else if (K == 4) {
                     v = make_float4(sigmoidf_(v.x), sigmoidf_(v.y), sigmoidf_(v.z), sigmoidf_(v.w));
@@ -386,7 +387,7 @@
     }
     if (epi == RAMNET_EPI_GRU_BLEND) run(std::integral_constant<int, 2>{});
     else if (epi == RAMNET_EPI_RES_RELU) run(std::integral_constant<int, 1>{});
-    else if (epi == RAMNET_EPI_GRU_BWD && n0 >= p.Cout / 2) run(std::integral_constant<int, 3>{});
+    else if (epi == RAMNET_EPI_GRU_BWD && n0 >= q.gru_col0) run(std::integral_constant<int, 3>{});
     else if (epi == RAMNET_EPI_SIGMOID) run(std::integral_constant<int, 4>{});
     else if (epi == RAMNET_EPI_SIGMOID_HR) run(std::integral_constant<int, 5>{});
     else run(std::integral_constant<int, 0>{});
@@ -453,9 +454,9 @@
     return wgs >= g_w6_min_wgs ? 1 : 0;
 }
 
-int launch_wino6(const ramnet_conv_desc &d, hipStream_t st) {
+static int launch_wino6_plan(const ramnet_conv_desc &d, hipStream_t st, const Wino6Split *sp) {
     Wino6Plan pl;
-    if (int rc = wino6_plan(d, WK, pl)) return rc;
+    if (int rc = wino6_plan(d, WK, pl, false, sp)) return rc;
     const bool lstm = d.epi == RAMNET_EPI_LSTM;
     if (lstm) note_kernel(d.active ? "conv_wino_r6_kernel<%d,%d,masked,lstm>" : "conv_wino_r6_kernel<%d,%d,lstm>", pl.txg, d.in_mode);
     else note_kernel(d.active ? "conv_wino_r6_kernel<%d,%d,masked>" : "conv_wino_r6_kernel<%d,%d>", pl.txg, d.in_mode);
@@ -493,9 +494,18 @@
     return 0;
 }
 
+int launch_wino6(const ramnet_conv_desc &d, hipStream_t st) { return launch_wino6_plan(d, st, nullptr); }
+
 }
 
 using namespace ramnet;
+
+extern "C" int ramnet_conv_launch_split(const ramnet_conv_desc *d, int n_split, int c_lo, float beta_hi, void *stream) {
+    RAMNET_CHECK_ARG(d != nullptr && d->algo == RAMNET_ALGO_WINOGRAD_2X4);
+    if (int rc = check_conv_desc(*d)) return rc;
+    const Wino6Split sp = {n_split, c_lo, beta_hi};
+    return launch_wino6_plan(*d, (hipStream_t)stream, &sp);
+}
 
 #ifdef RAMNET_PROBE
 extern "C" int ramnet_probe6_read(unsigned long long *dst, size_t n) {
diff --git a/rpg_ramnet_amd/csrc/conv_wino_common.hpp b/rpg_ramnet_amd/csrc/conv_wino_common.hpp
--- a/rpg_ramnet_amd/csrc/conv_wino_common.hpp
+++ b/rpg_ramnet_amd/csrc/conv_wino_common.hpp
@@ -17,6 +17,9 @@
     int ksplit;
     float *ws;
     int *cnt;
+    int n_split, nchunks_lo;
+    float beta_hi;
+    int gru_col0;
     float inv_nbl, inv_tx, inv_ty;
 };
 
diff --git a/rpg_ramnet_amd/ops.py b/rpg_ramnet_amd/ops.py
--- a/rpg_ramnet_amd/ops.py
+++ b/rpg_ramnet_amd/ops.py
@@ -73,6 +73,14 @@
 def set_gru_bwd_fused(on):
     global _GRU_BWD_FUSED
     _GRU_BWD_FUSED = bool(on)
+
+
+_GRU_BWD_MERGED = True
+
+
+def set_gru_bwd_merged(on):
+    global _GRU_BWD_MERGED
+    _GRU_BWD_MERGED = bool(on)
 
 
 _GRU_HR = _os.environ.get("RAMNET_GRU_HR", "1") != "0"
@@ -223,6 +231,12 @@
     d = _conv_desc(x0, taps, w, out, Cout, **kw)
     if active is not None:
         d.active = _p(active)
+    split = kw.get("split")
+    if split is not None:
+        if d.algo != H.ALGO_WINOGRAD_2X4:
+            raise RuntimeError("conv_launch(split=...): the launch does not run the exact F(2x4,3x3) kernel (algo %d)" % d.algo)
+        H.check(H.lib().ramnet_conv_launch_split(C.byref(d), split[0], split[1], split[2], _st()), "ramnet_conv_launch_split")
+        return
     H.check(H.lib().ramnet_conv_launch(C.byref(d), _st()), "ramnet_conv_launch")
 
 
@@ -278,7 +292,7 @@
 
 def _conv_desc(x0, taps, w, out, Cout, *, stride=1, x1=None, xm=None, xm_off=0, in_mode=H.IN_PLAIN,
                C0=None, C1=0, Hin=None, Win=None, bias=None, epi=H.EPI_LINEAR, beta=0.0, e0=None, e1=None,
-               o1=None, o2=None, Ho=None, Wo=None, os=(1, 1, 0, 0), out_off=0, frame=0, out_s2d=0, wino24=False, ws_owner=None):
+               o1=None, o2=None, Ho=None, Wo=None, os=(1, 1, 0, 0), out_off=0, frame=0, out_s2d=0, wino24=False, ws_owner=None, split=None):
     is_ref = isinstance(w, PackRef)
     al = out.data_ptr() | (4 * out_off)
     for t in (e0, e1, o1, o2, bias):
@@ -287,7 +301,7 @@
     key = (id(taps), id(w.cp) if is_ref else 0, w.transposed if is_ref else -1, id(ws_owner), Cout, stride, in_mode, C0, C1, Hin, Win, epi, beta, Ho,
            Wo, os, out_off, frame, out_s2d, wino24, xm_off, tuple(x0.shape), x0.stride(2), _sd(x1), _sd(xm), out.shape[1], out.shape[2],
            out.stride(2), _sd(e0), _sd(e1), _sd(o1), _sd(o2), bias is None, al & 15, _WINOGRAD, _WINO_2X4, _SPLIT_OPERANDS, _HEAD, _S2D_SPARSE, _S2D_2X4,
-           _FOLD_2X3, _DESC_EPOCH, x0.device.index)
+           _FOLD_2X3, _DESC_EPOCH, x0.device.index, split)
     hit = _DESC_CACHE.get(key) if _DESC_CACHE_ON else None
     if hit is not None and (not is_ref or hit[3]() is w.cp) and (ws_owner is None or hit[4]() is ws_owner):
         tmpl, kind, nsplit = hit[0], hit[1], hit[2]
@@ -305,7 +319,7 @@
     meta = []
     d = _conv_desc_build(x0, taps, w, out, Cout, meta, stride=stride, x1=x1, xm=xm, xm_off=xm_off, in_mode=in_mode, C0=C0, C1=C1, Hin=Hin, Win=Win,
                          bias=bias, epi=epi, beta=beta, e0=e0, e1=e1, o1=o1, o2=o2, Ho=Ho, Wo=Wo, os=os, out_off=out_off, frame=frame,
-                         out_s2d=out_s2d, wino24=wino24, ws_owner=ws_owner)
+                         out_s2d=out_s2d, wino24=wino24, ws_owner=ws_owner, split=split)
     import weakref
     if len(_DESC_CACHE) > 4096:
         _DESC_CACHE.clear()
@@ -316,7 +330,7 @@
 
 def _conv_desc_build(x0, taps, w, out, Cout, meta, *, stride=1, x1=None, xm=None, xm_off=0, in_mode=H.IN_PLAIN,
                      C0=None, C1=0, Hin=None, Win=None, bias=None, epi=H.EPI_LINEAR, beta=0.0, e0=None, e1=None,
-                     o1=None, o2=None, Ho=None, Wo=None, os=(1, 1, 0, 0), out_off=0, frame=0, out_s2d=0, wino24=False, ws_owner=None):
+                     o1=None, o2=None, Ho=None, Wo=None, os=(1, 1, 0, 0), out_off=0, frame=0, out_s2d=0, wino24=False, ws_owner=None, split=None):
     B = x0.shape[0]
     kind, nsplit = None, 0
     d = H.ConvDesc()
@@ -354,12 +368,15 @@
     d.ldo, d.ldo1, d.ldo2 = ld(out), (ld(o1) if o1 is not None else 0), (ld(o2) if o2 is not None else 0)
     if wino24:
         d.algo = H.ALGO_WINOGRAD24
+    if split is not None and epi == H.EPI_GRU_BWD:
+        d.epi = H.EPI_LINEAR
     if ref is not None and _WINO_2X4 != "off" and H.lib().ramnet_conv_wino_variant(C.byref(d), int(_WINO_2X4 == "force")):
         d.algo, d.s2d_5x5 = H.ALGO_WINOGRAD_2X4, 0
         kind = "2x4g" if epi == H.EPI_LSTM else "2x4"
-        if _SPLIT_OPERANDS and H.lib().ramnet_conv_wino_split_ok(C.byref(d), int(_WINO_2X4 == "force")):
+        if split is None and _SPLIT_OPERANDS and H.lib().ramnet_conv_wino_split_ok(C.byref(d), int(_WINO_2X4 == "force")):
             d.algo, kind = H.ALGO_WINOGRAD_2X4_SPLIT, "2x4s"
         d.w = _p(ref.cp.pack(ref.transposed, kind))
+    d.epi = epi
     if wino24 and cp is not None and _FOLD_2X3 != "off" and H.lib().ramnet_fold_wino_variant(C.byref(d), int(_FOLD_2X3 == "force")):
         kind = "f23d" if in_mode == H.IN_PARITY4 else "f23"
         d.algo = H.ALGO_WINOGRAD24_2X3
@@ -1523,6 +1540,25 @@
     return active if (active.dtype == torch.int32 and active.is_contiguous()) else (active != 0).to(torch.int32).contiguous()
 
 
+class _GRUBwdHalf(ConvParam):
+
+    def __init__(self, wo):
+        super().__init__([wo], [None])
+        self.Cin = wo.shape[1] // 2
+        self.CinWs = self.Cin
+
+    def _cat_w(self):
+        w = self.weights[0].detach()
+        return w[:, w.shape[1] // 2:].contiguous()
+
+
+def _gru_bwd_params(cp_ur, cp_o):
+    hit = cp_ur.__dict__.get("_gru_bwd")
+    if hit is None or hit[0] is not cp_o:
+        hit = cp_ur._gru_bwd = (cp_o, ConvParam(cp_ur.weights + cp_o.weights, [None] * (len(cp_ur.weights) + 1)), _GRUBwdHalf(cp_o.weights[0]), {})
+    return hit[1:]
+
+
 class GRUCell(Function):
 
     @staticmethod
@@ -1586,14 +1622,32 @@
             _wgrad_cell(cp_o, ws, [x, hr, dpo], x, taps, dpo, Cc, x1=hr, in_mode=H.IN_CAT, C1=Cc, dbias=bws)
         else:
             _wgrad_cell(cp_o, ws, [x, h, ur, dpo], x, taps, dpo, Cc, x1=h, xm=ur, xm_off=Cc, in_mode=H.IN_CAT_MUL, C1=Cc, dbias=bws)
-        if fused:
+        merged = False
+        if _GRU_BWD_MERGED and Cc % 64 == 0 and not _SPLIT_OPERANDS:
+            cp_cat, cp_half, ok = _gru_bwd_params(cp_ur, cp_o)
+            a2 = dict(out_off=Cc, split=(0, 0, 0.0))
+            if fused:
+                a2.update(epi=H.EPI_GRU_BWD, e0=ur[..., Cc:], e1=h, o1=dpur[..., Cc:])
+            a3 = dict(x1=dpo, in_mode=H.IN_CAT, C1=Cc, beta=1.0, split=(Cc, 2 * Cc, 0.0))
+            key = (tuple(x.shape), fused, _WINOGRAD, _WINO_2X4, _DESC_EPOCH)
+            merged = ok.get(key)
+            if merged is None:
+                merged = ok[key] = (_conv_desc(dpo, tapsd, cp_half.bwd(), dxh, Cc, **a2).algo == H.ALGO_WINOGRAD_2X4 and
+                                    _conv_desc(dpur, tapsd, cp_cat.bwd(), dxh, 2 * Cc, **a3).algo == H.ALGO_WINOGRAD_2X4)
+        if merged:
+            conv_launch(dpo, tapsd, cp_half.bwd(), dxh, Cc, **a2)
+        elif fused:
             conv_launch(dpo, tapsd, cp_o.bwd(), dxh, 2 * Cc, epi=H.EPI_GRU_BWD, e0=ur, e1=h, o1=dpur)
         else:
             conv_launch(dpo, tapsd, cp_o.bwd(), dxh, 2 * Cc)
+        if not fused:
             H.check(L.ramnet_gru_bwd_b(_p(dxh), _p(ur), _p(h), _p(dpur), _p(dhd), npix, Cc, _st()), "gru_bwd_b")
         ws, bws = cp_ur.grad_ws(wino_ok=Cc % 32 == 0)
         _wgrad_cell(cp_ur, ws, [x, h, dpur], x, taps, dpur, 2 * Cc, x1=h, in_mode=H.IN_CAT, C1=Cc, dbias=bws)
-        conv_launch(dpur, tapsd, cp_ur.bwd(), dxh, 2 * Cc, beta=1.0)
+        if merged:
+            conv_launch(dpur, tapsd, cp_cat.bwd(), dxh, 2 * Cc, **a3)
+        else:
+            conv_launch(dpur, tapsd, cp_ur.bwd(), dxh, 2 * Cc, beta=1.0)
         return dxh[..., :Cc], dxh[..., Cc:], None, None, None, None, None, None, None, None, None, None
 
 
```

Result: no change. 234.5 samples/s, median of 2 (-0.1%).
